# NVIDIA/nvalchemi-toolkit-ops

Measured on AMD Instinct MI355X. Metric: atom-steps/sec (nlist+D3+PME) on 100k-atom PBC box, higher is better.
Workload: dtype f64 (PME) + f32 (D3)

## Files before the change

include/nvalchemiops_hip.h:

```cpp
#ifndef NVALCHEMIOPS_HIP_H
#define NVALCHEMIOPS_HIP_H

#include <stddef.h>
#include <stdint.h>

#ifdef __cplusplus
extern "C" {
#endif

#define MI_OK 0
#define MI_EINVAL (-1)
#define MI_EHIP (-2)
#define MI_EWORKSPACE (-3)
#define MI_ECOMM (-4)

#define MI_F32 0
#define MI_F64 1

int mi_version(void);
const char* mi_last_error(void);
int mi_timing_enable(int on);
int mi_timing_select(const char* name );
int mi_timing_report(char* buf , int cap);
int mi_timing_report_stats(char* buf , int cap);
int mi_calibrate_copy(const void* src, void* dst, size_t bytes, void* stream);
int mi_calibrate_fill(void* dst, size_t bytes, float value, void* stream);
int mi_calibrate_read(const void* src, size_t bytes, float* sink , void* stream);

#define MI_NL_MODE_MATRIX 0
#define MI_NL_MODE_COUNT 1
#define MI_NL_MODE_CSR 2

#define MI_NL_HALF_FILL 1
#define MI_NL_NAIVE_EXPR 2
#define MI_NL_REUSE_GRID 4
#define MI_NL_NO_SHIFTS 8
#define MI_NL_NO_PAD 16

size_t mi_nl_workspace_bytes(int n_atoms, int n_systems, int dtype);

int mi_nl_neighbors(const void* positions,
                    int n_atoms,
                    const void* cell,
                    const uint8_t* pbc,
                    const int32_t* batch_idx,
                    int n_systems, double cutoff, int dtype, int mode, int flags,
                    int32_t* neighbor_matrix,
                    int32_t* neighbor_matrix_shifts,
                    int32_t* num_neighbors,
                    int max_neighbors, int fill_value,
                    const int32_t* neighbor_ptr,
                    int32_t* list_ij,
                    int32_t* list_shifts,
                    long long n_pairs,
                    const void* bin_origin,
                    void* workspace, size_t workspace_bytes, void* stream);

size_t mi_nl_packed_bytes(int n_atoms, int max_neighbors);
int mi_nl_neighbors_packed(const void* positions, int n_atoms, const void* cell, const uint8_t* pbc, const int32_t* batch_idx, int n_systems,
                           double cutoff, int dtype, int flags, int32_t* neighbor_matrix, int32_t* neighbor_matrix_shifts,
                           int32_t* num_neighbors, int max_neighbors, int fill_value, const void* bin_origin, void* workspace,
                           size_t workspace_bytes, void* packed_out, size_t packed_bytes, void* stream);

typedef struct mi_nl_cn_request {
  const int32_t* numbers;
  const float* covalent_radii;
  int nz;
  float k1;
} mi_nl_cn_request;
size_t mi_nl_cn_bytes(int n_atoms);
int mi_nl_neighbors_packed_cn(const void* positions, int n_atoms, const void* cell, const uint8_t* pbc, const int32_t* batch_idx, int n_systems,
                              double cutoff, int dtype, int flags, int32_t* neighbor_matrix, int32_t* neighbor_matrix_shifts,
                              int32_t* num_neighbors, int max_neighbors, int fill_value, const void* bin_origin, void* workspace,
                              size_t workspace_bytes, void* packed_out, size_t packed_bytes, const mi_nl_cn_request* request ,
                              void* cn_out, size_t cn_bytes, void* stream);

int mi_nl_neighbors_dual(const void* positions, int n_atoms, const void* cell, const uint8_t* pbc, const int32_t* batch_idx, int n_systems,
                         double cutoff_short, double cutoff_long, int dtype, int flags,
                         int32_t* neighbor_matrix_short, int32_t* neighbor_matrix_shifts_short, int32_t* num_neighbors_short,
                         int max_neighbors_short,
                         int32_t* neighbor_matrix_long, int32_t* neighbor_matrix_shifts_long, int32_t* num_neighbors_long,
                         int max_neighbors_long, int fill_value, const void* bin_origin, void* workspace, size_t workspace_bytes,
                         void* stream);

int mi_nl_matrix_to_coo(const int32_t* neighbor_matrix, const int32_t* neighbor_matrix_shifts,
                        const int32_t* neighbor_ptr, int n_atoms, int max_neighbors, int fill_value,
                        int32_t* list_ij, int32_t* list_shifts, long long n_pairs, void* stream);

int mi_nl_build_cell_cache(const void* positions, int n_atoms, const void* cell, const uint8_t* pbc,
                           const int32_t* batch_idx, int n_systems, double cutoff, int dtype,
                           int max_total_cells, int32_t* cells_per_dimension, int32_t* atom_periodic_shifts,
                           int32_t* atom_to_cell_mapping, int32_t* atoms_per_cell_count,
                           int32_t* cell_atom_start_indices, int32_t* cell_atom_list, void* workspace,
                           size_t workspace_bytes, void* stream);

int mi_nl_estimate_sizes(const void* cell, const uint8_t* pbc, int n_systems, double cutoff, int max_nbins,
                         int dtype, int32_t* number_of_cells ,
                         int32_t* neighbor_search_radius , void* stream);

int mi_nl_bounding_cells(const void* positions, const int32_t* batch_idx, int n_atoms, int n_systems, int dtype, void* cell_out,
                         void* origin_out, void* scratch, void* stream);

int mi_nl_cells_changed(const void* positions, const void* cell , const int32_t* atom_to_cell_mapping,
                        const int32_t* cells_per_dimension , const uint8_t* pbc , int n_atoms, int dtype,
                        uint8_t* flag, void* stream);
int mi_nl_moved_beyond_skin(const void* reference_positions, const void* current_positions, double threshold, int n_atoms, int dtype,
                            uint8_t* flag, void* stream);

typedef struct {
  const float* rcov;
  const float* r4r2;
  const float* c6ab;
  const float* cn_ref;
  int nz;
  float a1, a2, s6, s8, k1, k3, s5_on, s5_off;
} mi_d3_params;

size_t mi_d3_workspace_bytes(int n_atoms, int n_systems, int nz);
size_t mi_d3_workspace_bytes_packed(int n_atoms, int n_systems, int nz, int max_neighbors);
size_t mi_d3_workspace_bytes_entries(int n_atoms, int n_systems, int nz, long long n_entries);

int mi_d3(const void* positions, const int32_t* numbers, int n_atoms, int dtype,
          const int32_t* idx_j,
          const int32_t* unit_shifts,
          const int32_t* neighbor_ptr,
          int max_neighbors,
          long long n_list_entries,
          int fill_value,
          const void* cell,
          const int32_t* batch_idx,
          int n_systems, const mi_d3_params* params , int compute_virial,
          float* energy , float* forces , float* coord_num ,
          float* virial , void* workspace, size_t workspace_bytes, void* stream);

int mi_d3_packed(const void* positions, const int32_t* numbers, int n_atoms, int dtype, const int32_t* neighbor_matrix,
                 const int32_t* neighbor_matrix_shifts, int max_neighbors, int fill_value, const void* cell, const int32_t* batch_idx,
                 int n_systems, const mi_d3_params* params, int compute_virial, float* energy, float* forces, float* coord_num, float* virial,
                 void* workspace, size_t workspace_bytes, const void* packed_list, size_t packed_bytes ,
                 void* stream);

int mi_d3_packed_cn(const void* positions, const int32_t* numbers, int n_atoms, int dtype, const int32_t* neighbor_matrix,
                    const int32_t* neighbor_matrix_shifts, int max_neighbors, int fill_value, const void* cell, const int32_t* batch_idx,
                    int n_systems, const mi_d3_params* params, int compute_virial, float* energy, float* forces, float* coord_num, float* virial,
                    void* workspace, size_t workspace_bytes, const void* packed_list, size_t packed_bytes, const void* cn_block, size_t cn_bytes,
                    int verify_stride, int verify_phase, void* stream);

typedef struct {
  float rs6, rs8, alpha, beta;
  const float* r0ab;
} mi_d3_zero_params;

int mi_d3_zero(const void* positions, const int32_t* numbers, int n_atoms, int dtype, const int32_t* idx_j, const int32_t* unit_shifts,
               const int32_t* neighbor_ptr, int max_neighbors, long long n_list_entries, int fill_value, const void* cell,
               const int32_t* batch_idx, int n_systems, const mi_d3_params* params , const mi_d3_zero_params* zero ,
               int compute_virial, float* energy, float* forces, float* coord_num, float* virial, void* workspace, size_t workspace_bytes,
               void* stream);

int mi_d3_zero_packed_cn(const void* positions, const int32_t* numbers, int n_atoms, int dtype, const int32_t* neighbor_matrix,
                         const int32_t* neighbor_matrix_shifts, int max_neighbors, int fill_value, const void* cell, const int32_t* batch_idx,
                         int n_systems, const mi_d3_params* params, const mi_d3_zero_params* zero, int compute_virial, float* energy,
                         float* forces, float* coord_num, float* virial, void* workspace, size_t workspace_bytes, const void* packed_list,
                         size_t packed_bytes, const void* cn_block, size_t cn_bytes, int verify_stride, int verify_phase, void* stream);

size_t mi_d3_atm_workspace_bytes(int n_atoms, int n_systems, int nz);
size_t mi_d3_atm_visits_offset(int n_atoms, int n_systems, int nz);
int mi_d3_atm_tile(void);
int mi_d3_atm(const void* positions, const int32_t* numbers, int n_atoms, int dtype,
              const int32_t* idx_j, const int32_t* unit_shifts, const int32_t* neighbor_ptr ,
              int max_neighbors, int fill_value, const void* cell, const int32_t* batch_idx, int n_systems,
              const mi_d3_params* params , float s9, float alpha, float three_body_cutoff, int compute_virial,
              float* energy , float* forces , float* virial ,
              void* workspace, size_t workspace_bytes, void* stream);

int mi_d3_zero_atm(const void* positions, const int32_t* numbers, int n_atoms, int dtype,
                   const int32_t* idx_j, const int32_t* unit_shifts, const int32_t* neighbor_ptr ,
                   int max_neighbors, int fill_value, const void* cell, const int32_t* batch_idx, int n_systems,
                   const mi_d3_params* params , float s9, float alpha, float three_body_cutoff, float rs9,
                   const float* r0ab , int compute_virial, float* energy, float* forces, float* virial,
                   void* workspace, size_t workspace_bytes, void* stream);

typedef struct {
  const float* rcov;
  const float* en;
  const float* r4r2;
  const float* zeff;
  const float* gam;
  const int32_t* n_ref;
  const int32_t* ngw;
  const float* cn_ref;
  const float* q_ref;
  const float* c6_ref;
  int nz;
  float a1, a2, s6, s8, k_cn, k4, k5, k6, wf, ga, gc;
  float cn_cutoff;
} mi_d4_params;
size_t mi_d4_workspace_bytes(int n_atoms, int n_systems, int nz);
int mi_d4_species_slots(void);
int mi_d4_fold_blocks(void);
int mi_d4(const void* positions, const int32_t* numbers, int n_atoms, int dtype, const int32_t* idx_j, const int32_t* unit_shifts,
          const int32_t* neighbor_ptr , int max_neighbors, long long n_list_entries, int fill_value,
          const void* cell, const int32_t* batch_idx, int n_systems, const mi_d4_params* params ,
          const float* charges , int compute_virial, float* energy , float* forces ,
          float* coord_num , float* charge_grad , float* virial ,
          void* workspace, size_t workspace_bytes, void* stream);

size_t mi_d4_atm_workspace_bytes(int n_atoms, int n_systems, int nz);
size_t mi_d4_atm_visits_offset(int n_atoms, int n_systems, int nz);
int mi_d4_atm_tile(void);
int mi_d4_atm(const void* positions, const int32_t* numbers, int n_atoms, int dtype, const int32_t* idx_j, const int32_t* unit_shifts,
              const int32_t* neighbor_ptr , int max_neighbors, int fill_value, const void* cell,
              const int32_t* batch_idx, int n_systems, const mi_d4_params* params , float s9, float alpha,
              float three_body_cutoff, int compute_virial, float* energy , float* forces ,
              float* virial , void* workspace, size_t workspace_bytes, void* stream);

#define MI_EW_FORCES 1
#define MI_EW_CHARGE_GRAD 2
size_t mi_ewald_symmetry_scratch_bytes(void);
size_t mi_ewald_real_scratch_bytes(int n_atoms, int dtype);
int mi_ewald_real(const void* positions, const void* charges, const void* cell, const void* alpha ,
                  const int32_t* batch_idx, int n_atoms, int dtype, const int32_t* idx_j,
                  const int32_t* unit_shifts, const int32_t* neighbor_ptr, int max_neighbors, int mask_value,
                  int flags, double* energies , void* forces ,
                  double* charge_grads , void* scratch , size_t scratch_bytes, void* stream);
int mi_ewald_real_listed(const void* positions, const void* charges, const void* cell, const void* alpha, const int32_t* batch_idx, int n_atoms,
                         int dtype, const int32_t* idx_j, const int32_t* unit_shifts, const int32_t* neighbor_ptr, int max_neighbors,
                         int mask_value, int flags, double* energies, void* forces, double* charge_grads, void* scratch, size_t scratch_bytes,
                         const int32_t* search_num_neighbors, int verify_stride, int verify_phase, void* stream);
int mi_ewald_real_virial(const void* positions, const void* charges, const void* cell, const void* alpha, const int32_t* batch_idx, int n_atoms,
                         int n_systems, int dtype, const int32_t* idx_j, const int32_t* unit_shifts, const int32_t* neighbor_ptr, int max_neighbors,
                         int mask_value, int flags, double* energies, void* forces, double* charge_grads, void* scratch, size_t scratch_bytes,
                         const int32_t* search_num_neighbors, int verify_stride, int verify_phase, double* row_virial, double* virial_partial,
                         void* stream);
int mi_ewald_virial_blocks(void);

#define MI_GC_FORCES 1
#define MI_GC_CHARGE_GRAD 2
#define MI_GC_SIGMA_GRAD 4
#define MI_GC_VIRIAL 8
#define MI_GC_CELL_GRAD 16
size_t mi_gaussian_charges_scratch_bytes(int n_atoms, int dtype);
int mi_gaussian_charges_blocks(void);
int mi_gaussian_charges_row_words(void);
int mi_gaussian_charges_system_sums(const void* charges, const void* sigma, const double* weights, const int32_t* batch_idx, int n_atoms,
                                    int n_systems, int dtype, double* partial, void* stream);
int mi_gaussian_charges(const void* positions, const void* charges, const void* sigma, const void* cell ,
                        const int32_t* batch_idx, const double* weights, int n_atoms, int n_systems, int dtype, const int32_t* idx_j,
                        const int32_t* unit_shifts, const int32_t* neighbor_ptr, int max_neighbors, int mask_value, int flags, double* energies,
                        void* forces, double* charge_grads, double* sigma_grads, double* system_partial, void* scratch, size_t scratch_bytes,
                        void* stream);

#define MI_DP_FORCES 1
#define MI_DP_CHARGE_GRAD 2
#define MI_DP_DIPOLE_GRAD 4
#define MI_DP_VIRIAL 8
size_t mi_ewald_dipole_real_scratch_bytes(int n_atoms, int dtype);
int mi_ewald_dipole_blocks(void);
int mi_ewald_dipole_real(const void* positions, const void* charges, const void* dipoles, const void* cell ,
                         const void* alpha , const int32_t* batch_idx, const double* weights, int n_atoms, int n_systems, int dtype,
                         const int32_t* idx_j, const int32_t* unit_shifts, const int32_t* neighbor_ptr, int max_neighbors, int mask_value, int flags,
                         double* energies, void* forces, double* charge_grads, double* dipole_grads, double* virial_partial, void* scratch,
                         size_t scratch_bytes, void* stream);
int mi_ewald_dipole_structure_factors(const void* positions, const void* charges, const void* dipoles, const double* weights, const void* k_vectors,
                                      const int32_t* system_ptr, int n_atoms, int n_systems, int n_k, int dtype, double* table, void* stream);
int mi_ewald_dipole_recip_gather(const void* positions, const void* charges, const void* dipoles, const void* k_vectors, const void* cell,
                                 const void* alpha, const int32_t* batch_idx, const double* table, const double* table_g, const double* weights,
                                 int n_atoms, int n_systems, int n_k, int dtype, double* energies, void* forces, double* charge_grads,
                                 double* dipole_grads, void* stream);
int mi_ewald_dipole_recip_virial(const double* table, const void* k_vectors, const void* cell, const void* alpha, int n_systems, int n_k, int dtype,
                                 double* virial, void* stream);

#define MI_QD_FORCES 1
#define MI_QD_CHARGE_GRAD 2
#define MI_QD_DIPOLE_GRAD 4
#define MI_QD_VIRIAL 8
#define MI_QD_QUADRUPOLE_GRAD 16
size_t mi_ewald_quadrupole_real_scratch_bytes(int n_atoms, int dtype);
int mi_ewald_quadrupole_blocks(void);
int mi_ewald_quadrupole_real(const void* positions, const void* charges, const void* dipoles, const void* quadrupoles,
                             const void* cell , const void* alpha , const int32_t* batch_idx,
                             const double* weights, int n_atoms, int n_systems, int dtype, const int32_t* idx_j, const int32_t* unit_shifts,
                             const int32_t* neighbor_ptr, int max_neighbors, int mask_value, int flags, double* energies, void* forces,
                             double* charge_grads, double* dipole_grads, double* quadrupole_grads, double* virial_partial, void* scratch,
                             size_t scratch_bytes, void* stream);
int mi_ewald_quadrupole_structure_factors(const void* positions, const void* charges, const void* dipoles, const void* quadrupoles,
                                          const double* weights, const void* k_vectors, const int32_t* system_ptr, int n_atoms, int n_systems,
                                          int n_k, int dtype, double* table, double* table_v, void* stream);
int mi_ewald_quadrupole_recip_gather(const void* positions, const void* charges, const void* dipoles, const void* quadrupoles,
                                     const void* k_vectors, const void* cell, const void* alpha, const int32_t* batch_idx, const double* table,
                                     const double* table_g, const double* weights, int n_atoms, int n_systems, int n_k, int dtype,
                                     double* energies, void* forces, double* charge_grads, double* dipole_grads, double* quadrupole_grads,
                                     void* stream);
int mi_ewald_quadrupole_recip_virial(const double* table, const double* table_v, const void* k_vectors, const void* cell, const void* alpha,
                                     int n_systems, int n_k, int dtype, double* virial, void* stream);

#define MI_DP_POLAR_GRAD 16
size_t mi_thole_dipole_scratch_bytes(int n_atoms, int dtype);
int mi_thole_dipole_blocks(void);
int mi_thole_dipole(const void* positions, const void* charges, const void* dipoles, const void* cell ,
                    const void* polarizability , double thole_a, const int32_t* batch_idx, const double* weights, int n_atoms,
                    int n_systems, int dtype, const int32_t* idx_j, const int32_t* unit_shifts, const int32_t* neighbor_ptr, int max_neighbors,
                    int mask_value, int flags, double* energies, void* forces, double* charge_grads, double* dipole_grads,
                    double* polarizability_grads, double* virial_partial, void* scratch, size_t scratch_bytes, void* stream);

size_t mi_coulomb_dipole_scratch_bytes(int n_atoms, int dtype);
int mi_coulomb_dipole_blocks(void);
int mi_coulomb_dipole(const void* positions, const void* charges, const void* dipoles, const void* cell ,
                      const int32_t* batch_idx, const double* weights, int n_atoms, int n_systems, int dtype, const int32_t* idx_j,
                      const int32_t* unit_shifts, const int32_t* neighbor_ptr, int max_neighbors, int mask_value, int flags, double* energies,
                      void* forces, double* charge_grads, double* dipole_grads, double* virial_partial, void* scratch, size_t scratch_bytes,
                      void* stream);
size_t mi_coulomb_quadrupole_scratch_bytes(int n_atoms, int dtype);
int mi_coulomb_quadrupole_blocks(void);
int mi_coulomb_quadrupole(const void* positions, const void* charges, const void* dipoles, const void* quadrupoles,
                          const void* cell , const int32_t* batch_idx, const double* weights, int n_atoms,
                          int n_systems, int dtype, const int32_t* idx_j, const int32_t* unit_shifts, const int32_t* neighbor_ptr,
                          int max_neighbors, int mask_value, int flags, double* energies, void* forces, double* charge_grads,
                          double* dipole_grads, double* quadrupole_grads, double* virial_partial, void* scratch, size_t scratch_bytes,
                          void* stream);

int mi_qeq_blocks(void);
int mi_qeq_state_words(void);
int mi_qeq_pair_coefficients(const void* positions, const void* sigma, const double* hardness, const void* cell ,
                             const void* alpha , const int32_t* batch_idx, int n_atoms, int n_systems, int dtype,
                             const int32_t* idx_j, const int32_t* unit_shifts, const int32_t* neighbor_ptr, int max_neighbors, int mask_value,
                             double* coefficients, int32_t* neighbors, double* diagonal, void* stream);
int mi_qeq_apply(const double* coefficients, const int32_t* neighbors, const double* diagonal, const double* x, const double* y_in,
                 const int32_t* batch_idx, int n_atoms, int n_systems, const int32_t* neighbor_ptr, int max_neighbors, double* y, double* partial,
                 void* stream);
int mi_qeq_cg_update(const double* y, const double* partial_y, const double* counts, const int32_t* batch_idx, int n_atoms, int n_systems, int mode,
                     double* q, double* r, const double* p, const double* state_in, double* state_out, double* partial_rr, void* stream);
int mi_qeq_cg_direction(const double* partial_rr, const int32_t* batch_idx, int n_atoms, int n_systems, int mode, double tolerance, const double* r,
                        double* p, const double* state_in, double* state_out, void* stream);

int mi_induced_blocks(void);
int mi_induced_state_words(void);
int mi_induced_tensor_words(void);
int mi_induced_unroll_depth(void);
int mi_induced_pair_tensors(const void* positions, const void* polarizability, const void* cell , const void* alpha ,
                            const int32_t* batch_idx, int n_atoms, int n_systems, int dtype, const int32_t* idx_j, const int32_t* unit_shifts,
                            const int32_t* neighbor_ptr, int max_neighbors, int mask_value, long long n_slots, double* tensors, int32_t* neighbors,
                            double* diagonal, double* preconditioner, void* stream);
int mi_thole_induced_pair_tensors(const void* positions, const void* polarizability, const void* cell ,
                                  const void* alpha , const int32_t* batch_idx, int n_atoms, int n_systems, int dtype,
                                  const int32_t* idx_j, const int32_t* unit_shifts, const int32_t* neighbor_ptr, int max_neighbors, int mask_value,
                                  long long n_slots, double* tensors, int32_t* neighbors, double* diagonal, double* preconditioner,
                                  double thole_a, void* stream);
int mi_cluster_induced_pair_tensors(const void* positions, const void* polarizability, int n_atoms, int dtype, const int32_t* idx_j,
                                    const int32_t* neighbor_ptr, int max_neighbors, int mask_value, long long n_slots, double* tensors,
                                    int32_t* neighbors, double* diagonal, double* preconditioner, double thole_a, void* stream);
int mi_induced_apply(const double* tensors, const int32_t* neighbors, const double* diagonal, const double* x, const double* y_in,
                     const int32_t* batch_idx, int n_atoms, int n_systems, const int32_t* neighbor_ptr, int max_neighbors, long long n_slots,
                     double* y, double* partial, void* stream);
int mi_induced_dot(const double* x, const double* y, const int32_t* batch_idx, int n_atoms, int n_systems, double* partial, void* stream);
int mi_induced_cg_update(const double* y, const double* partial_y, const double* preconditioner, const int32_t* batch_idx, int n_atoms,
                         int n_systems, int mode, double* x, double* r, const double* p, const double* state_in,
                         double* state_out, double* partial_rr, void* stream);
int mi_induced_cg_direction(const double* partial_rr, const double* preconditioner, const int32_t* batch_idx, int n_atoms, int n_systems,
                            int mode, double tolerance, const double* r, double* p, const double* state_in, double* state_out,
                            void* stream);

int mi_ewald_recip_virial(const double* structure_factors, const void* k_vectors, const void* cell, const void* alpha, int n_systems, int n_k,
                          int dtype, double* partial, void* stream);
int mi_ewald_recip_virial_blocks(void);
int mi_ewald_structure_factors(const void* positions, const void* weights , const void* k_vectors, const void* cell,
                               const void* alpha, const int32_t* system_ptr, int n_atoms, int n_systems, int n_k,
                               int max_atoms_per_system, int dtype, double* structure_factors ,
                               double* total_charge , void* stream);
int mi_ewald_recip_gather(const void* positions, const void* charges, const void* k_vectors, const void* alpha, const int32_t* batch_idx,
                          const double* structure_factors, const double* total_charge, int n_atoms, int n_k, int dtype,
                          double* potential , double* kforce , double* energies ,
                          void* forces , double* charge_grads , void* stream);

int mi_ewald_recip_gather_kk(const void* positions, const void* k_vectors, const int32_t* batch_idx, const double* structure_factors,
                             const double* weights , int n_atoms, int n_k, int dtype, double* out , void* stream);

size_t mi_ewald_real_bwd_scratch_bytes(int n_systems);
int mi_ewald_real_bwd(const void* positions, const void* charges, const void* cell, const void* alpha, const int32_t* batch_idx,
                      int n_atoms, int n_systems, int dtype, const int32_t* idx_j, const int32_t* unit_shifts, const int32_t* neighbor_ptr,
                      int max_neighbors, int mask_value, const void* grad_energies ,
                      void* grad_positions , void* grad_charges ,
                      double* grad_cell, double* grad_alpha, void* symmetry_scratch ,
                      size_t scratch_bytes ,
                      void* stream);

int mi_ewald_real_forces_bwd(const void* positions, const void* charges, const void* cell, const void* alpha, const int32_t* batch_idx,
                             int n_atoms, int n_systems, int dtype, const int32_t* idx_j, const int32_t* unit_shifts,
                             const int32_t* neighbor_ptr, int max_neighbors, int mask_value, const void* grad_forces ,
                             const void* grad_charge_grads , double* grad_positions ,
                             double* grad_charges , double* grad_cell , double* grad_alpha ,
                             void* scratch , size_t scratch_bytes, void* stream);

int mi_coulomb(const double* positions, const double* charges, const double* cell , const int32_t* batch_idx,
               int n_atoms, const int32_t* idx_j, const int32_t* unit_shifts, const int32_t* neighbor_ptr, int max_neighbors,
               int fill_value, double cutoff, double alpha, double energy_prefactor, double* energies ,
               double* forces , void* stream);
int mi_coulomb_bwd(const double* positions, const double* charges, const double* cell, const int32_t* batch_idx, int n_atoms,
                   int n_systems, const int32_t* idx_j, const int32_t* unit_shifts, const int32_t* neighbor_ptr, int max_neighbors,
                   int fill_value, double cutoff, double alpha, double energy_prefactor, const double* grad_energies ,
                   double* grad_positions , double* grad_charges , double* grad_cell ,
                   void* stream);

int mi_coulomb_forces_bwd(const double* positions, const double* charges, const double* cell, const int32_t* batch_idx, int n_atoms,
                          int n_systems, const int32_t* idx_j, const int32_t* unit_shifts, const int32_t* neighbor_ptr, int max_neighbors,
                          int fill_value, double cutoff, double alpha, const double* grad_forces ,
                          double* grad_positions , double* grad_charges , double* grad_cell ,
                          void* stream);

#define MI_SPLINE_REFERENCE_ORDERS 0x100
int mi_cell_geometry(const void* cell, int n_systems, int dtype, void* cell_inv_t, void* reciprocal_cell, void* volume, void* stream);
int mi_pme_prepare(const void* cell, const void* charges, const int32_t* batch_idx, int n_atoms, int n_systems, int dtype,
                   void* cell_inv_t, void* reciprocal_cell, void* volume, void* total_charge , void* stream);
int mi_spline_spread_is_tiled(int n_systems, int nx, int ny, int nz, int order);
int mi_spline_spread_prefers_tiles(int n_atoms, int n_systems, int nx, int ny, int nz, int order);
int mi_spline_spread(const void* positions, const void* values, const int32_t* batch_idx,
                     const void* cell_inv_t , int n_atoms, int n_systems, int nx, int ny,
                     int nz, int order, int batched, int dtype, void* mesh ,
                     void* workspace , size_t workspace_bytes, void* stream);
size_t mi_spline_spread_workspace_bytes(int n_atoms, int n_systems, int nx, int ny, int nz);
size_t mi_spline_spread_workspace_bytes_for(int n_atoms, int n_systems, int nx, int ny, int nz, int order, int dtype);
long long mi_spline_spread_order_offset(int n_atoms, int n_systems, int nx, int ny, int nz, int order);
int mi_spline_gather(const void* positions, const void* mesh, const int32_t* batch_idx, const void* cell_inv_t,
                     int n_atoms, int n_systems, int nx, int ny, int nz, int order, int dtype,
                     void* out , void* stream);
int mi_spline_gather_vec3(const void* positions, const void* charges, const void* mesh_vec3 ,
                          const int32_t* batch_idx, const void* cell_inv_t, int n_atoms, int n_systems, int nx,
                          int ny, int nz, int order, int dtype, void* out , void* stream);

int mi_spline_gather_grad(const void* positions, const void* mesh, const int32_t* batch_idx, const void* cell_inv_t, int n_atoms,
                          int n_systems, int nx, int ny, int nz, int order, int dtype, void* out , void* stream);

int mi_spline_gather_hess_dot(const void* positions, const void* mesh, const int32_t* batch_idx, const void* cell_inv_t,
                              const void* vec , int n_atoms, int n_systems, int nx, int ny, int nz, int order, int dtype,
                              void* out , void* stream);
int mi_spline_spread_grad(const void* positions, const void* vec , const int32_t* batch_idx, const void* cell_inv_t,
                          int n_atoms, int n_systems, int nx, int ny, int nz, int order, int dtype, void* mesh ,
                          void* stream);

size_t mi_spline_spread_channels_workspace_bytes_for(int n_atoms, int n_systems, int nx, int ny, int nz, int order, int n_channels, int dtype);
int mi_spline_spread_channels(const void* positions, const void* values , const int32_t* batch_idx, const void* cell_inv_t,
                              int n_atoms, int n_systems, int n_channels, int nx, int ny, int nz, int order, int batched, int dtype,
                              void* mesh , void* workspace, size_t workspace_bytes, void* stream);
int mi_spline_gather_channels(const void* positions, const void* mesh , const int32_t* batch_idx,
                              const void* cell_inv_t, int n_atoms, int n_systems, int n_channels, int nx, int ny, int nz, int order, int dtype,
                              void* out , void* stream);
int mi_spline_gather_channels_frac_grad(const void* positions, const void* mesh , const void* coef ,
                                        const int32_t* batch_idx, const void* cell_inv_t, int n_atoms, int n_systems, int n_channels, int nx,
                                        int ny, int nz, int order, int dtype, void* out , void* stream);

int mi_sph_harm(const double* positions , int n, int l_max, double* out, void* stream);
int mi_sph_harm_grad(const double* positions , int n, int l_max, double* out, void* stream);
int mi_gto_density(const double* positions , int n, double sigma, int l_max, double* out, void* stream);
int mi_gto_fourier(const double* k_vectors , int n, double sigma, int l_max, double* out_real, double* out_imag, void* stream);

int mi_fft_plan_create(int nx, int ny, int nz, int batch, int dtype, int inverse, void** plan_out);
size_t mi_fft_plan_work_bytes(const void* plan);
int mi_fft_plan_exec(void* plan, void* in, void* out, void* stream);
int mi_fft_plan_destroy(void* plan);

int mi_fft_library_versions(int* compiled, int* loaded);

#define MI_DFT_MAX_N 1024
int mi_dft3d(void* in, void* out, int nx, int ny, int nz, int batch, int dtype, int inverse, void* stream);

int mi_pme_green_sf(const void* k_squared , const void* alpha , const void* volume ,
                    int n_systems, int nx, int ny, int nz, int sf_exponent, int dtype, void* green ,
                    void* sf_sq , void* stream);
int mi_pme_convolve(const void* spec , const void* recip_cell ,
                    const void* alpha , const void* volume , int n_systems, int nx, int ny, int nz,
                    int sf_exponent, int with_field, int dtype,
                    const void* k_vectors , const void* k_squared ,
                    int k_batched , void* out , void* stream);
int mi_pme_solve_supported(int n_systems, int nx, int ny, int nz, int dtype);
int mi_pme_solve_preferred(int n_systems, int nx, int ny, int nz, int dtype);
size_t mi_pme_solve_scratch_bytes(int n_systems, int nx, int ny, int nz, int n_channels , int dtype);
int mi_pme_solve(const void* mesh, const void* recip_cell , const void* alpha ,
                 const void* volume , int n_systems, int nx, int ny, int nz, int order ,
                 int with_field, int dtype, void* scratch, size_t scratch_bytes, void* real_out, void* stream);
int mi_pme_solve_keep(const void* mesh, const void* recip_cell, const void* alpha, const void* volume, int n_systems, int nx, int ny, int nz,
                      int order, int with_field, int dtype, void* scratch, size_t scratch_bytes, void* real_out, void* spectrum_out,
                      void* stream);
int mi_fft_lds_supported(int batch, int nx, int ny, int nz, int dtype);
size_t mi_fft_lds_scratch_bytes(int batch, int nx, int ny, int nz, int dtype);
int mi_fft_lds(const void* in, void* out, int batch, int nx, int ny, int nz, int dtype, int inverse, void* scratch, size_t scratch_bytes,
               const void* tables , void* stream);
size_t mi_fft_lds_tables_bytes(int nx, int ny, int nz, int dtype);
int mi_fft_lds_tables(int nx, int ny, int nz, int dtype, void* tables, void* stream);
int mi_pme_solve_tabled(const void* mesh, const void* recip_cell, const void* alpha, const void* volume, int n_systems, int nx, int ny, int nz,
                        int order, int with_field, int dtype, void* scratch, size_t scratch_bytes, void* real_out, void* spectrum_out,
                        const void* tables, void* stream);
int mi_pme_convolve_bwd(const void* spec, const void* weight_spec, int n_channels, const void* recip_cell, const void* alpha, const void* volume,
                        int n_systems, int nx, int ny, int nz, int order, int dtype, void* conv_out, double* partial, void* stream);
int mi_pme_convolve_bwd_blocks(void);
int mi_pme_virial(const void* spec, const void* recip_cell, const void* alpha, const void* volume, int n_systems, int nx, int ny, int nz, int order,
                  int dtype, const void* k_vectors, const void* k_squared, int k_batched, const void* total_charge, double* partial, void* stream);
int mi_pme_virial_blocks(void);

int mi_pme_dipole_spread(const void* positions, const void* charges, const void* dipoles, const double* weights, const int32_t* batch_idx,
                         const void* cell_inv_t, int n_atoms, int n_systems, int nx, int ny, int nz, int order, int dtype, void* meshes, void* stream);
int mi_pme_dipole_gather(const void* positions, const void* charges, const void* dipoles, const double* weights, const int32_t* batch_idx,
                         const void* cell_inv_t, const void* mesh_a, const void* mesh_b, const void* alpha , int n_atoms, int n_systems,
                         int nx, int ny, int nz, int order, int dtype, int accumulate, double* energies, void* forces, double* charge_grads,
                         double* dipole_grads, void* stream);
int mi_pme_dipole_virial(const void* spec_q, const void* spec_mu, const void* recip_cell, const void* alpha, const void* volume, int n_systems, int nx,
                         int ny, int nz, int order, int dtype, double* partial, void* stream);
int mi_pme_dipole_virial_blocks(void);

int mi_pme_quadrupole_spread(const void* positions, const void* charges, const void* dipoles, const void* quadrupoles, const double* weights,
                             const int32_t* batch_idx, const void* cell_inv_t, int n_atoms, int n_systems, int nx, int ny, int nz, int order, int dtype,
                             void* meshes, void* stream);
int mi_pme_quadrupole_gather(const void* positions, const void* charges, const void* dipoles, const void* quadrupoles, const double* weights,
                             const int32_t* batch_idx, const void* cell_inv_t, const void* mesh_a, const void* mesh_b, const void* alpha ,
                             int n_atoms, int n_systems, int nx, int ny, int nz, int order, int dtype, int accumulate, double* energies, void* forces,
                             double* charge_grads, double* dipole_grads, double* quadrupole_grads, void* stream);
int mi_pme_quadrupole_virial(const void* spec_l, const void* spec_t, const void* recip_cell, const void* alpha, const void* volume, int n_systems,
                             int nx, int ny, int nz, int order, int dtype, double* partial, void* stream);
int mi_pme_quadrupole_virial_blocks(void);

int mi_pme_gather_finish(const void* positions, const void* charges, const int32_t* batch_idx, const void* cell_inv_t,
                         const void* meshes , const void* alpha, const void* volume,
                         const void* total_charge , int n_atoms, int n_systems, int nx, int ny, int nz,
                         int order, int with_field, int dtype, void* energies ,
                         void* forces , void* charge_grads ,
                         const double* add_energies, const void* add_forces, const double* add_charge_grads,
                         const void* spread_workspace ,
                         void* stream);
int mi_pme_corrections(const void* raw, const void* charges, const int32_t* batch_idx, const void* volume,
                       const void* alpha, const void* total_charge, int n_atoms, int dtype, void* energies,
                       void* charge_grads , void* stream);
int mi_segment_sum(const void* values, const int32_t* batch_idx, int n_atoms, int dtype, void* out , void* stream);

int mi_frame_rotate(const void* positions, const void* local_dipoles, const void* local_quadrupoles, const int32_t* frame_atoms,
                    const int32_t* frame_kinds, const void* cell, const int32_t* batch_idx, int n_atoms, int n_systems, int dtype, void* dipoles,
                    void* quadrupoles, void* stream);
int mi_frame_adjoint(const void* positions, const void* local_dipoles, const void* local_quadrupoles, const int32_t* frame_atoms,
                     const int32_t* frame_kinds, const void* cell, const int32_t* batch_idx, const void* dipole_grads,
                     const void* quadrupole_grads, int n_atoms, int n_systems, int dtype, double* records, double* local_dipole_grads,
                     double* local_quadrupole_grads, double* virial_rows, void* stream);
int mi_frame_gather(const double* records, const int32_t* inverse_ptr, const int32_t* inverse_slots, long long n_entries,
                    const double* virial_rows, const int32_t* batch_idx, int n_atoms, int n_systems, int dtype, double sign, void* out,
                    double* virial_partial, void* stream);
int mi_frame_blocks(void);
int mi_frame_block_threads(void);

#define MI_COMM_ID_BYTES 128
int mi_comm_library_version(int* version );
int mi_comm_unique_id(void* id_out , size_t bytes);
int mi_comm_init(const void* id , size_t bytes, int n_ranks, int rank, void** comm_out);
int mi_comm_size(const void* comm, int* n_ranks , int* rank );
int mi_comm_allgather_f32(void* comm, const float* send, float* recv , size_t count_per_rank, void* stream);
int mi_comm_allgather_f64(void* comm, const double* send, double* recv, size_t count_per_rank, void* stream);
int mi_comm_destroy(void* comm);

#ifdef __cplusplus
}
#endif
#endif
```

nvalchemi-toolkit-ops_amd/csrc/nlist.hip:

```cpp
#include <stdlib.h>

#include "binsort.h"
#include "common.h"

namespace {

#define NL_PRUNE_R 8
#ifndef NL_TILE
#define NL_TILE 1024
#endif
#ifndef NL_TILE_F64
#define NL_TILE_F64 768
#endif
#ifndef NL_TILED_WAVES
#define NL_TILED_WAVES 0
#endif
#ifndef NL_CCHUNK
#define NL_CCHUNK 64
#endif
#define NL_MAXROWS 96
#define NL_MIXED 0x7fffffff
#define NL_TILED_GRID 1536
static int nl_tiled_grid() {
  static const int g = [] { const char* e = getenv("NVALCHEMIOPS_NL_TILED_GRID"); const int v = e ? atoi(e) : 0; return v > 0 ? v : NL_TILED_GRID; }();
  return g;
}
template <class T> struct NlSys {
  T cell[9];
  T inv[9];
  T origin[3];
  int cpd[3];
  int R[3];
  int pbc[3];
  int nrange[3];
  int cell_off;
  int ncells;
  int tiled;
  int prune;
  signed char dxlim[NL_PRUNE_R + 1][NL_PRUNE_R + 1];
};
struct NlGlobal {
  int total_cells; int any_wrap; int use_tiled; int pad1;
  int work[4];
  int done[4];
};

struct NlLayout {
  size_t sys, glob, natoms, keys_in, keys_out, vals_in, vals_out, wrap, swrap, spos, srk, cell_start, bins, total;
  long long cell_cap;
};

inline long long nl_cell_cap(int N, int B) { return 4ll * N + 8ll * B; }

inline int nl_key_bits(long long cap) {
  int bits = 1;
  while ((1ll << bits) <= cap && bits < 31) ++bits;
  return bits;
}

NlLayout nl_layout(int N, int B, int dtype) {
  NlLayout L;
  size_t o = 0;
  const size_t sysz = dtype == MI_F32 ? sizeof(NlSys<float>) : sizeof(NlSys<double>);
  const size_t esz = dtype == MI_F32 ? 4 : 8;
  L.cell_cap = nl_cell_cap(N, B);
  auto take = [&](size_t bytes) { size_t at = o; o += mi_align(bytes); return at; };
  L.sys = take(sysz * (size_t)B);
  L.glob = take(sizeof(NlGlobal));
  L.natoms = take(sizeof(int) * (size_t)B);
  L.keys_in = take(sizeof(int) * (size_t)N);
  L.keys_out = take(sizeof(int) * (size_t)N);
  L.vals_in = take(sizeof(int) * (size_t)N);
  L.vals_out = take(sizeof(int) * (size_t)N);
  L.wrap = take(8 * (size_t)N);
  L.swrap = take(8 * (size_t)N);
  L.spos = take(4 * esz * (size_t)N);
  L.srk = take(sizeof(float) * (size_t)N);
  L.cell_start = take(sizeof(int) * (size_t)(L.cell_cap + 2));
  L.bins = take(sizeof(int) * bs_scratch_ints(L.cell_cap + 2));
  L.total = o;
  return L;
}

__device__ __forceinline__ float4 pack4(float x, float y, float z, int idx) { return make_float4(x, y, z, __int_as_float(idx)); }
__device__ __forceinline__ double4 pack4(double x, double y, double z, int idx) { return make_double4(x, y, z, (double)idx); }
__device__ __forceinline__ int idx_of(const float4& v) { return __float_as_int(v.w); }
__device__ __forceinline__ int idx_of(const double4& v) { return (int)v.w; }

__global__ void nl_count_atoms_kernel(const int* __restrict__ batch_idx, int N, int* __restrict__ natoms) {
  const int i = blockIdx.x * blockDim.x + threadIdx.x;
  const bool in = i < N;
  const int s = in ? batch_idx[i] : -1;
  const int s0 = __shfl(s, 0, MI_WAVE);
  const unsigned long long same = __ballot(in && s == s0);
  if ((threadIdx.x & (MI_WAVE - 1)) == 0 && s0 >= 0) atomicAdd(&natoms[s0], __popcll(same));
  if (in && s != s0) atomicAdd(&natoms[s], 1);
}

template <class T>
__device__ void nl_describe_system(const T* __restrict__ cell, const uint8_t* __restrict__ pbc, const int* __restrict__ natoms, int N, T cutoff,
                                   const T* __restrict__ origin, int s, NlSys<T>& S) {
  for (int k = 0; k < 9; ++k) S.cell[k] = cell[9 * (size_t)s + k];
  for (int k = 0; k < 3; ++k) S.origin[k] = origin ? origin[3 * (size_t)s + k] : T(0);
  inverse3(S.cell, S.inv);
  const T* a = S.cell;
  double det = (double)a[0] * ((double)a[4] * a[8] - (double)a[5] * a[7]) - (double)a[1] * ((double)a[3] * a[8] - (double)a[5] * a[6]) +
               (double)a[2] * ((double)a[3] * a[7] - (double)a[4] * a[6]);
  double vol = fabs(det);
  int ns = natoms ? natoms[s] : N;
  double rc = (double)cutoff;
  double apc = vol > 0 ? (double)ns / vol * rc * rc * rc : 0.0;
#ifndef NL_K2_APC
#define NL_K2_APC 64.0
#endif
  int k = apc < NL_K2_APC ? 1 : (apc < 512.0 ? 2 : 3);
  long long cap = 4ll * ns + 8;
  double face[3];
  for (int d = 0; d < 3; ++d) {
    T col[3] = {S.inv[d], S.inv[3 + d], S.inv[6 + d]};
    T ln = sqrt(col[0] * col[0] + col[1] * col[1] + col[2] * col[2]);
    face[d] = 1.0 / (double)ln;
    S.pbc[d] = pbc[3 * (size_t)s + d] ? 1 : 0;
    double want = face[d] * k / (rc * (1.0 + 2e-6));
    S.cpd[d] = want >= 1048576.0 ? 1048576 : (want >= 1.0 ? (int)want : 1);
    S.nrange[d] = S.pbc[d] ? (int)ceil(ln * cutoff) : 0;
  }
  long long tot = (long long)S.cpd[0] * S.cpd[1] * S.cpd[2];
  while (tot > cap) {
    for (int d = 0; d < 3; ++d) S.cpd[d] = S.cpd[d] / 2 > 1 ? S.cpd[d] / 2 : 1;
    tot = (long long)S.cpd[0] * S.cpd[1] * S.cpd[2];
  }
  for (int d = 0; d < 3; ++d) {
    if (S.cpd[d] == 1 && !S.pbc[d]) S.R[d] = 0;
    else S.R[d] = (int)ceil(rc * S.cpd[d] / face[d] * (1.0 + 1e-6));
  }
  S.ncells = (int)tot;
  S.cell_off = 0;
  S.tiled = ((k >= 2 || apc >= 32.0) && (2 * S.R[1] + 1) * (2 * S.R[2] + 1) <= NL_MAXROWS && (!S.pbc[0] || S.R[0] <= S.cpd[0])) ? 1 : 0;
  const bool ortho = a[1] == T(0) && a[2] == T(0) && a[3] == T(0) && a[5] == T(0) && a[6] == T(0) && a[7] == T(0);
  S.prune = (ortho && S.R[0] <= NL_PRUNE_R && S.R[1] <= NL_PRUNE_R && S.R[2] <= NL_PRUNE_R) ? 1 : 0;
}

template <class T>
__global__ __launch_bounds__(256) void nl_setup_kernel(const T* __restrict__ cell, const uint8_t* __restrict__ pbc, const int* __restrict__ natoms, int N,
                                int B, T cutoff, const T* __restrict__ origin, NlSys<T>* __restrict__ sys, NlGlobal* __restrict__ glob,
                                int table_blocks, int4* __restrict__ zero, long long zero_words, int* __restrict__ pk_flag,
                                int* __restrict__ cn_hdr, float cn_scale) {
  constexpr int NE = (NL_PRUNE_R + 1) * (NL_PRUNE_R + 1);
  if (pk_flag && blockIdx.x == 0 && threadIdx.x == 0) *pk_flag = 0;
  if (cn_hdr && blockIdx.x == 0) {
    if (threadIdx.x == 0) { cn_hdr[0] = 0; cn_hdr[1] = 0; cn_hdr[2] = __float_as_int((float)cutoff); cn_hdr[3] = __float_as_int(cn_scale); }
    if (threadIdx.x < MI_CN_SLOTS) reinterpret_cast<unsigned long long*>(cn_hdr)[MI_CN_SLOT_OFFSET_U64 + threadIdx.x] = 0ull;
  }
  if ((int)blockIdx.x > table_blocks) {
    const long long zb = (long long)blockIdx.x - table_blocks - 1, nzb = (long long)gridDim.x - table_blocks - 1;
    for (long long k = zb * blockDim.x + threadIdx.x; k < zero_words; k += nzb * blockDim.x) zero[k] = make_int4(0, 0, 0, 0);
    return;
  }
  if (blockIdx.x > 0) {
    const int t = ((int)blockIdx.x - 1) * blockDim.x + threadIdx.x;
    if (t >= B * NE) return;
    const int s = t / NE, az = (t - s * NE) / (NL_PRUNE_R + 1), ay = t - s * NE - az * (NL_PRUNE_R + 1);
    NlSys<T> S;
    nl_describe_system<T>(cell, pbc, natoms, N, cutoff, origin, s, S);
    if (!S.prune) return;
    const double rc = (double)cutoff;
    double w[3];
    for (int d = 0; d < 3; ++d) {
      const double ln = fabs((double)S.inv[4 * d]);
      w[d] = (S.pbc[d] && ln > 0.0) ? (1.0 / ln) / S.cpd[d] : 0.0;
    }
    const double gz = (az > 1 ? az - 1 : 0) * w[2], gy = (ay > 1 ? ay - 1 : 0) * w[1];
    const double rem = rc * rc - gz * gz - gy * gy;
    int lim;
    if (rem < -1e-6 * rc * rc) lim = -1;
    else if (w[0] > 0.0) { lim = (int)(sqrt(rem > 0.0 ? rem : 0.0) / w[0] * (1.0 + 1e-6)) + 1; if (lim > S.R[0]) lim = S.R[0]; }
    else lim = S.R[0];
    sys[s].dxlim[az][ay] = (signed char)lim;
    return;
  }
  for (int s = threadIdx.x; s < B; s += blockDim.x) {
    NlSys<T> S;
    nl_describe_system<T>(cell, pbc, natoms, N, cutoff, origin, s, S);
    NlSys<T>* dst = sys + s;
    for (int k = 0; k < 9; ++k) { dst->cell[k] = S.cell[k]; dst->inv[k] = S.inv[k]; }
    for (int k = 0; k < 3; ++k) { dst->origin[k] = S.origin[k]; dst->cpd[k] = S.cpd[k]; dst->R[k] = S.R[k]; dst->pbc[k] = S.pbc[k]; dst->nrange[k] = S.nrange[k]; }
    dst->cell_off = 0; dst->ncells = S.ncells; dst->tiled = S.tiled; dst->prune = S.prune;
  }
  __syncthreads();
  __shared__ int wave_tot[4];
  __shared__ int carry_sh, tiled_sh;
  if (threadIdx.x == 0) { carry_sh = 0; tiled_sh = 1; }
  __syncthreads();
  const int lane = threadIdx.x & (MI_WAVE - 1), wave = threadIdx.x / MI_WAVE;
  for (int s0 = 0; s0 < B; s0 += blockDim.x) {
    const int s = s0 + threadIdx.x;
    const int x = s < B ? sys[s].ncells : 0;
    if (s < B && !sys[s].tiled) tiled_sh = 0;
    int inc = x;
#pragma unroll
    for (int o = 1; o < MI_WAVE; o <<= 1) { const int up = __shfl_up(inc, o, MI_WAVE); if (lane >= o) inc += up; }
    if (lane == MI_WAVE - 1) wave_tot[wave] = inc;
    __syncthreads();
    int woff = carry_sh;
    for (int w = 0; w < 4; ++w) woff += (w < wave) ? wave_tot[w] : 0;
    if (s < B) sys[s].cell_off = woff + inc - x;
    __syncthreads();
    if (threadIdx.x == blockDim.x - 1) carry_sh = woff + inc;
    __syncthreads();
  }
  if (threadIdx.x == 0) {
    glob->total_cells = carry_sh;
    glob->any_wrap = 0;
    glob->use_tiled = tiled_sh;
    for (int k = 0; k < 4; ++k) { glob->work[k] = 0; glob->done[k] = 0; }
  }
}

template <class T>
__global__ void nl_assign_kernel(const T* __restrict__ pos, const int* __restrict__ batch_idx, int N, const NlSys<T>* __restrict__ sys,
                                 int* __restrict__ keys, int* __restrict__ count, short4* __restrict__ wrap, NlGlobal* __restrict__ glob) {
  int i = blockIdx.x * blockDim.x + threadIdx.x;
  const bool in = i < N;
  int key = 0;
  if (in) {
    const int s = batch_idx ? batch_idx[i] : 0;
    const NlSys<T>& S = sys[s];
    T p[3] = {pos[3 * (size_t)i] - S.origin[0], pos[3 * (size_t)i + 1] - S.origin[1], pos[3 * (size_t)i + 2] - S.origin[2]}, frac[3];
    rowvec_mat3(p, S.inv, frac);
    int c[3], w[3];
#pragma unroll
    for (int d = 0; d < 3; ++d) {
      int v = (int)floor(frac[d] * (T)S.cpd[d]);
      if (S.pbc[d]) floor_divmod(v, S.cpd[d], w[d], c[d]);
      else { w[d] = 0; c[d] = v < 0 ? 0 : (v >= S.cpd[d] ? S.cpd[d] - 1 : v); }
    }
    key = S.cell_off + c[0] + S.cpd[0] * (c[1] + S.cpd[1] * c[2]);
    keys[i] = key;
    wrap[i] = make_short4((short)w[0], (short)w[1], (short)w[2], 0);
    if (w[0] | w[1] | w[2]) glob->any_wrap = 1;
  }
  bs_wave_add<false>(count, key, in);
}

struct NlCnBuild { const int* numbers; const float* rcov; int nz; float K; float* srk; unsigned long long* slots; const void* cell; int n_cell; const int* batch_idx; };
template <class T>
__global__ void nl_rank_gather_kernel(const T* __restrict__ pos, const int* __restrict__ ids, const int* __restrict__ keys,
                                      const int* __restrict__ cell_start, const short4* __restrict__ wrap, int N,
                                      typename Vec4<T>::type* __restrict__ spos, short4* __restrict__ swrap, int* __restrict__ keys_sorted,
                                      NlCnBuild C) {
  int p = blockIdx.x * blockDim.x + threadIdx.x;
  unsigned long long h = 0;
  if (p < N) {
    const int i = ids[p];
    const int key = keys[i];
    const int b = cell_start[key], e = cell_start[key + 1];
    int rank = 0;
    for (int q = b; q < e; ++q) rank += ids[q] < i ? 1 : 0;
    const int dst = b + rank;
    const T x = pos[3 * (size_t)i], y = pos[3 * (size_t)i + 1], z = pos[3 * (size_t)i + 2];
    spos[dst] = pack4(x, y, z, i);
    swrap[dst] = wrap[i];
    keys_sorted[dst] = key;
    if (C.srk) {
      const float rk = mi_cn_rk(C.numbers[i], C.nz, C.rcov, C.K);
      C.srk[dst] = rk;
      h = mi_cn_atom_hash<T>(i, C.batch_idx ? C.batch_idx[i] : 0, x, y, z, rk);
    }
  }
  if (C.srk) {
    if (p < C.n_cell) h += mi_cn_cell_hash<T>(p, reinterpret_cast<const T*>(C.cell)[p]);
    if (p == 0) h += mi_cn_scale_hash(C.K);
    mi_cn_slot_add(C.slots, p / MI_WAVE, h);
  }
}

struct NlInt3 { int a, b, c; };

template <bool NT = true>
__device__ __forceinline__ void wave_fill(int* __restrict__ dst, long long begin, long long end, int value, int lane) {
  long long n = end - begin;
  if (n <= 0) return;
  int* p = dst + begin;
  int head = (int)(((16 - ((uintptr_t)p & 15)) & 15) >> 2);
  if (head > n) head = (int)n;
  if (lane < head) p[lane] = value;
  long long body = (n - head) >> 2;
  int4* p4 = reinterpret_cast<int4*>(p + head);
  typedef int nl_i4 __attribute__((ext_vector_type(4)));
  const nl_i4 w4 = {value, value, value, value};
  for (long long t = lane; t < body; t += MI_WAVE) {
    if constexpr (NT) __builtin_nontemporal_store(w4, reinterpret_cast<nl_i4*>(p4 + t));
    else *reinterpret_cast<nl_i4*>(p4 + t) = w4;
  }
  long long done = head + (body << 2);
  if (done + lane < n) p[done + lane] = value;
}

__device__ __noinline__ void nl_prefix_runs(int* run_pre, int n, int lane) {
  int carry = 0;
  if (lane == 0) run_pre[0] = 0;
  for (int r0 = 0; r0 < n; r0 += MI_WAVE) {
    const int r = r0 + lane;
    int inc = r < n ? run_pre[r + 1] : 0;
#pragma unroll
    for (int o = 1; o < MI_WAVE; o <<= 1) { const int up = __shfl_up(inc, o, MI_WAVE); if (lane >= o) inc += up; }
    if (r < n) run_pre[r + 1] = carry + inc;
    carry += __shfl(inc, MI_WAVE - 1, MI_WAVE);
  }
}

__device__ __forceinline__ long long nl_uniform64(long long v) {
  const unsigned lo = __builtin_amdgcn_readfirstlane((unsigned)v), hi = __builtin_amdgcn_readfirstlane((unsigned)((unsigned long long)v >> 32));
  return (long long)(((unsigned long long)hi << 32) | lo);
}

__device__ __forceinline__ float nl_uni(float x) { return __int_as_float(__builtin_amdgcn_readfirstlane(__float_as_int(x))); }
__device__ __forceinline__ double nl_uni(double x) { return __longlong_as_double(nl_uniform64(__double_as_longlong(x))); }

template <class T> struct NlSecond { T rc2; int* nm; int* nsh; int* num; int M; };
struct NlPacked { unsigned* words; int* flag; };
struct NlCn { const float* rk; float* cn; int* flag; float K; };
__device__ __forceinline__ float nl_cn_term(float d2, float rki, float rkj, float K) {
  const float rinv = __builtin_amdgcn_rsqf(d2);
  const float t = fmaf(-(rki + rkj), rinv, K);
  return __builtin_amdgcn_rcpf(1.0f + __builtin_amdgcn_exp2f(t));
}
#define NL_PK_PAD 0xffffffffu
#ifndef NL_PREZERO_SHIFTS
#define NL_PREZERO_SHIFTS 1
#endif
#ifndef NL_PREZERO_NT
#define NL_PREZERO_NT 1
#endif
#define NL_PK_ZERO_SHIFT 0x54000000u
__device__ __forceinline__ unsigned nl_pk_code(int Sx, int Sy, int Sz, bool& bad) {
  const unsigned cx = (unsigned)(Sx + 1), cy = (unsigned)(Sy + 1), cz = (unsigned)(Sz + 1);
  bad = (cx > 2u) | (cy > 2u) | (cz > 2u);
  return ((cx & 3u) << 26) | ((cy & 3u) << 28) | (cz << 30);
}

template <class T>
__device__ __forceinline__ bool nl_pair_hit(T pix, T piy, T piz, int i, T cjx, T cjy, T cjz, int j, int Sx, int Sy, int Sz, const T* cart,
                                            T rc2, bool naive, bool half, int nr0, int nr1, int nr2, T* d2_out = nullptr) {
  T dr0, dr1, dr2;
  bool ok = true;
  if (!naive) {
    dr0 = (cjx - pix) + cart[0];
    dr1 = (cjy - piy) + cart[1];
    dr2 = (cjz - piz) + cart[2];
  } else {
    const bool upper = Sx > 0 || (Sx == 0 && Sy > 0) || (Sx == 0 && Sy == 0 && Sz >= 0);
    if (upper) { dr0 = (cart[0] + cjx) - pix; dr1 = (cart[1] + cjy) - piy; dr2 = (cart[2] + cjz) - piz; }
    else { dr0 = ((-cart[0]) + pix) - cjx; dr1 = ((-cart[1]) + piy) - cjy; dr2 = ((-cart[2]) + piz) - cjz; }
    ok = (Sx <= nr0 && -Sx <= nr0) && (Sy <= nr1 && -Sy <= nr1) && (Sz <= nr2 && -Sz <= nr2);
  }
  const T d2 = dr0 * dr0 + dr1 * dr1 + dr2 * dr2;
  if (d2_out) *d2_out = d2;
  const bool zeroS = (Sx | Sy | Sz) == 0;
  bool hit = ok && (d2 < rc2) && !(j == i && zeroS);
  if (half && hit) {
    const bool pos_shift = Sx > 0 || (Sx == 0 && Sy > 0) || (Sx == 0 && Sy == 0 && Sz > 0);
    hit = pos_shift || (zeroS && j > i);
  }
  return hit;
}

template <class T, int MODE, bool FAST, bool DUAL = false, bool CNF = false>
#if NL_TILED_WAVES > 0
__global__ __launch_bounds__(256) __attribute__((amdgpu_waves_per_eu(NL_TILED_WAVES, NL_TILED_WAVES))) void nl_query_tiled_kernel(
#else
__global__ __launch_bounds__(256) __attribute__((amdgpu_waves_per_eu((CNF && sizeof(T) == 4) ? 5 : 1, (CNF && sizeof(T) == 4) ? 5 : 8))) void nl_query_tiled_kernel(
#endif
    const typename Vec4<T>::type* __restrict__ spos, const short4* __restrict__ swrap, const int* __restrict__ cell_start,
    const NlSys<T>* __restrict__ sys, const NlGlobal* __restrict__ glob, int B, T rc2, int flags, int* __restrict__ nm,
    int* __restrict__ nsh, int* __restrict__ num, int M, int fill_value, const int* __restrict__ ptr, int* __restrict__ list_ij,
    int* __restrict__ list_sh, long long P, NlSecond<T> D, NlPacked K, NlCn CN = NlCn{nullptr, nullptr, nullptr, 0.0f}) {
  static_assert(!DUAL || (MODE == MI_NL_MODE_MATRIX && !FAST), "the dual-cutoff sweep is instantiated for the general matrix kernel only");
  static_assert(!CNF || (MODE == MI_NL_MODE_MATRIX && FAST && !DUAL), "coordination numbers ride with the plain full-list matrix search");
  constexpr int TILE = sizeof(T) == 8 ? NL_TILE_F64 : NL_TILE;
  if (!glob->use_tiled) return;
  if (!DUAL && FAST != ((flags & (MI_NL_HALF_FILL | MI_NL_NAIVE_EXPR)) == 0)) return;
  __shared__ float trk[CNF ? TILE : 1], cen_rk[CNF ? NL_CCHUNK : 1];
  __shared__ double ccn[CNF ? NL_CCHUNK : 1];
  __shared__ int ccnt2[DUAL ? NL_CCHUNK : 1];
  __shared__ T tx[TILE], ty[TILE], tz[TILE];
  __shared__ int tj[TILE];
  __shared__ short tsx[CNF ? 1 : TILE], tsy[CNF ? 1 : TILE], tsz[CNF ? 1 : TILE];
  __shared__ int tsp[CNF ? TILE : 1];
  __shared__ int run_beg[3 * NL_MAXROWS], run_pre[3 * NL_MAXROWS + 1], run_cs[3 * NL_MAXROWS];
  __shared__ int ccnt[NL_CCHUNK];
  __shared__ T cen_x[NL_CCHUNK], cen_y[NL_CCHUNK], cen_z[NL_CCHUNK];
  __shared__ int cen_i[NL_CCHUNK];
  __shared__ short4 cen_w[NL_CCHUNK];
  __shared__ int grp_run[TILE / MI_WAVE];
  __shared__ int grp_shift[TILE / MI_WAVE];
  __shared__ int u_store[CNF ? 1 : 9 * NL_MAXROWS];
  static_assert(sizeof(T) * TILE >= sizeof(int) * 9 * NL_MAXROWS, "the run table must fit the x array of a tile");
  int* const u_beg = CNF ? reinterpret_cast<int*>(tx) : u_store;
  int* const u_len = u_beg + 3 * NL_MAXROWS;
  int* const u_cs = u_beg + 6 * NL_MAXROWS;
  const int tid = threadIdx.x, lane = tid & (MI_WAVE - 1), wave = tid / MI_WAVE;
  const int total_cells = glob->total_cells;
  const bool anyw = glob->any_wrap != 0;
  const bool half = (flags & MI_NL_HALF_FILL) != 0, naive = (flags & MI_NL_NAIVE_EXPR) != 0;
  const unsigned long long lt = (1ull << lane) - 1ull;
  __shared__ int next_cell;
  NlGlobal* gw = const_cast<NlGlobal*>(glob);
  for (;;) {
    __syncthreads();
    if (tid == 0) next_cell = atomicAdd(&gw->work[MODE], 1);
    __syncthreads();
    const int c = next_cell;
    if (c >= total_cells) break;
    const int c_beg = cell_start[c], n_c = cell_start[c + 1] - c_beg;
    if (n_c == 0) continue;
    int s = 0;
    {
      int lo = 0, hi = B - 1;
      while (lo < hi) { const int mid = (lo + hi + 1) >> 1; if (sys[mid].cell_off <= c) lo = mid; else hi = mid - 1; }
      s = lo;
    }
    const NlSys<T>* S = sys + s;
    const int nx = S->cpd[0], ny = S->cpd[1], nz = S->cpd[2];
    const int Rx = S->R[0], Ry = S->R[1], Rz = S->R[2];
    const bool pbx = S->pbc[0] != 0, pby = S->pbc[1] != 0, pbz = S->pbc[2] != 0;
    const int coff = S->cell_off;
    const int nr0 = S->nrange[0], nr1 = S->nrange[1], nr2 = S->nrange[2];
    T cm[9];
#pragma unroll
    for (int k = 0; k < 9; ++k) cm[k] = S->cell[k];
    const int local = c - coff;
    const int cx = local % nx, cyz = local / nx, cy = cyz % ny, cz = cyz / ny;
    const int nyr = 2 * Ry + 1, nrows = (2 * Rz + 1) * nyr;
    __syncthreads();
    if (tid < nrows) {
      const int dzr = tid / nyr, dz = dzr - Rz, dy = tid - dzr * nyr - Ry;
      const int tzc = cz + dz, tyc = cy + dy;
      bool ok = (pbz || (tzc >= 0 && tzc < nz)) && (pby || (tyc >= 0 && tyc < ny));
      int csz = 0, wz = tzc, csy = 0, wy = tyc;
      if (ok) {
        while (wz < 0) { wz += nz; --csz; }
        while (wz >= nz) { wz -= nz; ++csz; }
        while (wy < 0) { wy += ny; --csy; }
        while (wy >= ny) { wy -= ny; ++csy; }
      }
      int dxm = Rx;
      if (S->prune) { dxm = S->dxlim[dz < 0 ? -dz : dz][dy < 0 ? -dy : dy]; ok = ok && dxm >= 0; }
      int xlo = cx - dxm, xhi = cx + dxm;
      if (!pbx) { xlo = xlo < 0 ? 0 : xlo; xhi = xhi > nx - 1 ? nx - 1 : xhi; }
      const int rowbase = coff + nx * (wy + ny * wz);
      for (int g = 0; g < 3; ++g) {
        const int img0 = (g - 1) * nx;
        const int xa = (xlo > img0 ? xlo : img0), xb = (xhi < img0 + nx - 1 ? xhi : img0 + nx - 1);
        int b = 0, len = 0;
        if (ok && xa <= xb && (pbx || g == 1)) { b = cell_start[rowbase + xa - img0]; len = cell_start[rowbase + xb - img0 + 1] - b; }
        u_beg[3 * tid + g] = b;
        u_len[3 * tid + g] = len;
        u_cs[3 * tid + g] = ((g - 1) & 0x3ff) | ((csy & 0x3ff) << 10) | ((csz & 0x3ff) << 20);
      }
    }
    __syncthreads();
    for (int r = tid; r < 3 * nrows; r += 256) {
      const int key = u_cs[r];
      int rank = 0;
      for (int q = 0; q < 3 * nrows; ++q) {
        const int kq = u_cs[q];
        rank += ((unsigned)kq < (unsigned)key) || (kq == key && q < r);
      }
      run_beg[rank] = u_beg[r];
      run_pre[rank + 1] = u_len[r];
      run_cs[rank] = key;
    }
    __syncthreads();
    if (wave == 0) nl_prefix_runs(run_pre, 3 * nrows, lane);
    __syncthreads();
    const int nruns = 3 * nrows, total = run_pre[nruns];
    for (int cbase = 0; cbase < n_c; cbase += NL_CCHUNK) {
      const int cend = (cbase + NL_CCHUNK < n_c) ? cbase + NL_CCHUNK : n_c;
      if (tid < NL_CCHUNK) {
        ccnt[tid] = 0;
        if (DUAL) ccnt2[tid] = 0;
        if (cbase + tid < cend) {
          const auto cr = spos[c_beg + cbase + tid];
          cen_x[tid] = cr.x; cen_y[tid] = cr.y; cen_z[tid] = cr.z;
          cen_i[tid] = idx_of(cr);
          cen_w[tid] = anyw ? swrap[c_beg + cbase + tid] : make_short4(0, 0, 0, 0);
          if (CNF) { cen_rk[tid] = CN.rk[c_beg + cbase + tid]; ccn[tid] = 0.0; }
        }
      }
      for (int tile0 = 0; tile0 < total; tile0 += TILE) {
        const int tile_n = (total - tile0 < TILE) ? total - tile0 : TILE;
        __syncthreads();
        if (tid < TILE / MI_WAVE && tile0 + tid * MI_WAVE < total) {
          const int v = tile0 + tid * MI_WAVE;
          int lo = 0, hi = nruns - 1;
          while (lo < hi) { const int mid = (lo + hi + 1) >> 1; if (run_pre[mid] <= v) lo = mid; else hi = mid - 1; }
          grp_run[tid] = lo;
        }
        __syncthreads();
        for (int t = tid; t < tile_n; t += 256) {
          const int v = tile0 + t;
          int lo = grp_run[t / MI_WAVE];
          while (lo + 1 < nruns && run_pre[lo + 1] <= v) ++lo;
          const int q = run_beg[lo] + (v - run_pre[lo]);
          const auto rec = spos[q];
          tx[t] = rec.x; ty[t] = rec.y; tz[t] = rec.z;
          tj[t] = idx_of(rec);
          if (CNF) trk[t] = CN.rk[q];
          const int cs = run_cs[lo];
          int sx = (cs << 22) >> 22, sy = (cs << 12) >> 22, sz = (cs << 2) >> 22;
          if (anyw) {
            const short4 wj = swrap[q];
            if (pbx) sx -= wj.x;
            if (pby) sy -= wj.y;
            if (pbz) sz -= wj.z;
          }
          if (CNF) tsp[t] = (sx & 0x3ff) | ((sy & 0x3ff) << 10) | ((sz & 0x3ff) << 20);
          else { tsx[t] = (short)sx; tsy[t] = (short)sy; tsz[t] = (short)sz; }
          const int cs0 = __builtin_amdgcn_readfirstlane(cs);
          const bool same = __all(cs == cs0) && !anyw;
          if (lane == 0) grp_shift[t / MI_WAVE] = same ? cs0 : NL_MIXED;
        }
        __syncthreads();
        constexpr int NC = 2;
        for (int ci0 = cbase + wave; ci0 < cend; ci0 += 4 * NC) {
          T ccx[NC], ccy[NC], ccz[NC];
          int ii[NC], cap_row[NC], cnt[NC], cnt2[NC];
          float rki[NC], cnp[NC];
          long long out_base[NC];
          short4 wi[NC];
          const int nc = (cend - ci0 + 3) / 4 < NC ? (cend - ci0 + 3) / 4 : NC;
#pragma unroll
          for (int u = 0; u < NC; ++u) {
            const bool live = u < nc;
            const int ci = live ? ci0 + 4 * u : ci0;
            ccx[u] = live ? cen_x[ci - cbase] : (T)NAN; ccy[u] = cen_y[ci - cbase]; ccz[u] = cen_z[ci - cbase];
            if (CNF) { ccx[u] = nl_uni(ccx[u]); ccy[u] = nl_uni(ccy[u]); ccz[u] = nl_uni(ccz[u]); }
            ii[u] = __builtin_amdgcn_readfirstlane(cen_i[ci - cbase]);
            wi[u] = cen_w[ci - cbase];
            if (MODE == MI_NL_MODE_CSR) { out_base[u] = ptr[ii[u]]; cap_row[u] = ptr[ii[u] + 1] - ptr[ii[u]]; }
            else { out_base[u] = (long long)ii[u] * M; cap_row[u] = M; }
            cnt[u] = ccnt[ci - cbase];
            cnt2[u] = DUAL ? ccnt2[ci - cbase] : 0;
            if (CNF) { rki[u] = nl_uni(cen_rk[ci - cbase]); cnp[u] = 0.0f; }
          }
          const bool ortho = S->prune != 0;
          int* row_j[NC];
          NlInt3* row_s[NC];
          unsigned* row_p[NC];
#pragma unroll
          for (int u = 0; u < NC; ++u) {
            const long long ob = nl_uniform64(out_base[u]);
            row_p[u] = (MODE == MI_NL_MODE_MATRIX && !DUAL && K.words) ? K.words + ob : nullptr;
            if (MODE == MI_NL_MODE_MATRIX) { row_j[u] = nm + ob; row_s[u] = nsh ? reinterpret_cast<NlInt3*>(nsh) + ob : nullptr; }
            else if (MODE == MI_NL_MODE_CSR) { row_j[u] = list_ij + P + ob; row_s[u] = list_sh ? reinterpret_cast<NlInt3*>(list_sh) + ob : nullptr; }
            else { row_j[u] = nullptr; row_s[u] = nullptr; }
          }
          constexpr bool PREZERO = NL_PREZERO_SHIFTS && MODE == MI_NL_MODE_MATRIX && !DUAL;
          const bool prezero = PREZERO && nsh && !(flags & MI_NL_NO_PAD);
          if (PREZERO && prezero && tile0 == 0) {
#pragma unroll
            for (int u = 0; u < NC; ++u)
              if (u < nc) wave_fill<NL_PREZERO_NT != 0>(nsh, out_base[u] * 3, (out_base[u] + M) * 3, 0, lane);
            asm volatile("s_waitcnt vmcnt(0)" ::: "memory");
          }
          auto emit_m = [&](int u, unsigned long long mask, bool hit, int j, int Sx, int Sy, int Sz, unsigned code, bool zero_shift = false) {
            if (MODE == MI_NL_MODE_COUNT) { cnt[u] += __popcll(mask); return; }
            if (mask) {
              const unsigned slot = __builtin_amdgcn_mbcnt_hi((unsigned)(mask >> 32), __builtin_amdgcn_mbcnt_lo((unsigned)mask, (unsigned)cnt[u]));
              if (hit && slot < (unsigned)cap_row[u]) {
                *reinterpret_cast<int*>(reinterpret_cast<char*>(row_j[u]) + slot * 4u) = j;
                if (row_s[u] && !(PREZERO && prezero && zero_shift))
                  *reinterpret_cast<NlInt3*>(reinterpret_cast<char*>(row_s[u]) + __umul24(slot, 12u)) = NlInt3{Sx, Sy, Sz};
                if (MODE == MI_NL_MODE_MATRIX && !DUAL && row_p[u]) *reinterpret_cast<unsigned*>(reinterpret_cast<char*>(row_p[u]) + slot * 4u) = (unsigned)j | code;
              }
              cnt[u] += __popcll(mask);
            }
          };
          auto emit = [&](int u, bool hit, int j, int Sx, int Sy, int Sz, unsigned code) { emit_m(u, __builtin_amdgcn_ballot_w64(hit), hit, j, Sx, Sy, Sz, code); };
          struct Cand { int j, tt, zg; T x, y, z; };
          auto fetch = [&](int t0) {
            Cand c;
            const int t = t0 + lane;
            const bool in = t < tile_n;
            c.tt = in ? t : 0;
            c.j = tj[c.tt];
            c.x = in ? tx[c.tt] : (T)NAN;
            c.y = ty[c.tt]; c.z = tz[c.tt];
            c.zg = grp_shift[(t0 < tile_n ? t0 : 0) / MI_WAVE];
            return c;
          };
          Cand nxt = fetch(0);
          for (int t0 = 0; t0 < tile_n; t0 += MI_WAVE) {
            const Cand cur = nxt;
            nxt = fetch(t0 + MI_WAVE);
            const int j = cur.j, tt = cur.tt;
            const float rkj = CNF ? trk[tt] : 0.0f;
            const T cjx = cur.x, cjy = cur.y, cjz = cur.z;
            const int gs = __builtin_amdgcn_readfirstlane(cur.zg);
            if (FAST && gs == 0) {
#pragma unroll
              for (int u = 0; u < NC; ++u) {
                const T dr0 = cjx - ccx[u], dr1 = cjy - ccy[u], dr2 = cjz - ccz[u];
                const T d2 = dr0 * dr0 + dr1 * dr1 + dr2 * dr2;
                const bool in = d2 < rc2, other = j != ii[u];
                if (CNF) cnp[u] += (in & other & ((float)d2 >= 1e-24f)) ? nl_cn_term((float)d2, rki[u], rkj, CN.K) : 0.0f;
                emit_m(u, __builtin_amdgcn_ballot_w64(in) & __builtin_amdgcn_ballot_w64(other), in & other, j, 0, 0, 0, NL_PK_ZERO_SHIFT, true);
              }
            } else if (FAST && gs != NL_MIXED) {
              const int Sx = (gs << 22) >> 22, Sy = (gs << 12) >> 22, Sz = (gs << 2) >> 22;
              T cart[3];
              if (ortho) { cart[0] = cm[0] * (T)Sx; cart[1] = cm[4] * (T)Sy; cart[2] = cm[8] * (T)Sz; }
              else { const T fs[3] = {(T)Sx, (T)Sy, (T)Sz}; rowvec_mat3(fs, cm, cart); }
              bool bad;
              const unsigned code = nl_pk_code(Sx, Sy, Sz, bad);
#pragma unroll
              for (int u = 0; u < NC; ++u) {
                const T dr0 = (cjx - ccx[u]) + cart[0], dr1 = (cjy - ccy[u]) + cart[1], dr2 = (cjz - ccz[u]) + cart[2];
                const T d2 = dr0 * dr0 + dr1 * dr1 + dr2 * dr2;
                const bool h = d2 < rc2;
                if (CNF) cnp[u] += (h & ((float)d2 >= 1e-24f)) ? nl_cn_term((float)d2, rki[u], rkj, CN.K) : 0.0f;
                if (MODE == MI_NL_MODE_MATRIX && bad && row_p[u] && h) *K.flag = 1;
                emit(u, h, j, Sx, Sy, Sz, code);
              }
            } else {
              int Sx0, Sy0, Sz0;
              if (CNF) { const int w = tsp[tt]; Sx0 = (w << 22) >> 22; Sy0 = (w << 12) >> 22; Sz0 = (w << 2) >> 22; }
              else { Sx0 = tsx[tt]; Sy0 = tsy[tt]; Sz0 = tsz[tt]; }
#pragma unroll
              for (int u = 0; u < NC; ++u) {
                int Sx = Sx0, Sy = Sy0, Sz = Sz0;
                if (anyw) { if (pbx) Sx += wi[u].x; if (pby) Sy += wi[u].y; if (pbz) Sz += wi[u].z; }
                T cart[3];
                if (ortho) { cart[0] = cm[0] * (T)Sx; cart[1] = cm[4] * (T)Sy; cart[2] = cm[8] * (T)Sz; }
                else { const T fs[3] = {(T)Sx, (T)Sy, (T)Sz}; rowvec_mat3(fs, cm, cart); }
                bool h;
                if (FAST) {
                  const T dr0 = (cjx - ccx[u]) + cart[0], dr1 = (cjy - ccy[u]) + cart[1], dr2 = (cjz - ccz[u]) + cart[2];
                  const T d2 = dr0 * dr0 + dr1 * dr1 + dr2 * dr2;
                  h = (d2 < rc2) & !((j == ii[u]) & ((Sx | Sy | Sz) == 0));
                  if (CNF) cnp[u] += (h & ((float)d2 >= 1e-24f)) ? nl_cn_term((float)d2, rki[u], rkj, CN.K) : 0.0f;
                } else {
                  T d2;
                  h = nl_pair_hit<T>(ccx[u], ccy[u], ccz[u], ii[u], cjx, cjy, cjz, j, Sx, Sy, Sz, cart, rc2, naive, half, nr0, nr1, nr2, &d2);
                  if (DUAL) {
                    const bool h2 = h && (d2 < D.rc2);
                    const unsigned long long m2 = __ballot(h2);
                    if (m2) {
                      const int slot = cnt2[u] + __popcll(m2 & lt);
                      if (h2 && slot < D.M) {
                        const long long o = (long long)ii[u] * D.M + slot;
                        D.nm[o] = j;
                        if (D.nsh) reinterpret_cast<NlInt3*>(D.nsh)[o] = NlInt3{Sx, Sy, Sz};
                      }
                      cnt2[u] += __popcll(m2);
                    }
                  }
                }
                bool bad;
                const unsigned code = nl_pk_code(Sx, Sy, Sz, bad);
                if (MODE == MI_NL_MODE_MATRIX && !DUAL && bad && row_p[u] && h) *K.flag = 1;
                emit(u, h, j, Sx, Sy, Sz, code);
              }
            }
          }
          if (CNF) {
#pragma unroll
            for (int u = 0; u < NC; ++u) {
              const double part = wave_sum((double)cnp[u]);
              if (lane == 0 && u < nc) ccn[ci0 + 4 * u - cbase] += part;
            }
          }
          if (lane == 0) {
#pragma unroll
            for (int u = 0; u < NC; ++u) if (u < nc) { ccnt[ci0 + 4 * u - cbase] = cnt[u]; if (DUAL) ccnt2[ci0 + 4 * u - cbase] = cnt2[u]; }
          }
        }
      }
      __syncthreads();
      for (int ci = cbase + wave; ci < cend; ci += 4) {
        const int i = __builtin_amdgcn_readfirstlane(cen_i[ci - cbase]);
        const int cnt = ccnt[ci - cbase];
        if (MODE != MI_NL_MODE_CSR) { if (lane == 0) num[i] = cnt; }
        if (CNF && lane == 0) {
          CN.cn[i] = (float)ccn[ci - cbase];
          if (cnt > M) *CN.flag = 1;
        }
        if (MODE == MI_NL_MODE_CSR) {
          const long long rb = ptr[i];
          const int room = ptr[i + 1] - ptr[i];
          wave_fill(list_ij, rb, rb + (cnt < room ? cnt : room), i, lane);
        }
        if (MODE == MI_NL_MODE_MATRIX && !(flags & MI_NL_NO_PAD)) {
          const long long out_base = (long long)i * M;
          const int used = cnt < M ? cnt : M;
          wave_fill(nm, out_base + used, out_base + M, fill_value, lane);
          if (nsh && !(NL_PREZERO_SHIFTS && !DUAL)) wave_fill(nsh, (out_base + used) * 3, (out_base + M) * 3, 0, lane);
          if (!DUAL && K.words) wave_fill(reinterpret_cast<int*>(K.words), out_base + used, out_base + M, (int)NL_PK_PAD, lane);
        }
        if (DUAL) {
          const int c2 = ccnt2[ci - cbase];
          if (lane == 0) D.num[i] = c2;
          if (!(flags & MI_NL_NO_PAD)) {
            const long long ob = (long long)i * D.M;
            const int used = c2 < D.M ? c2 : D.M;
            wave_fill(D.nm, ob + used, ob + D.M, fill_value, lane);
            if (D.nsh) wave_fill(D.nsh, (ob + used) * 3, (ob + D.M) * 3, 0, lane);
          }
        }
      }
      __syncthreads();
    }
  }
  if (tid == 0 && atomicAdd(&gw->done[MODE], 1) == (int)gridDim.x - 1) {
    gw->work[MODE] = 0;
    gw->done[MODE] = 0;
  }
}

template <class T, int MODE, bool DUAL = false, bool CNF = false>
__global__ __launch_bounds__(256) void nl_query_kernel(
    const typename Vec4<T>::type* __restrict__ spos, const short4* __restrict__ swrap, const int* __restrict__ keys_sorted,
    const int* __restrict__ cell_start, const int* __restrict__ batch_idx, const NlSys<T>* __restrict__ sys,
    const NlGlobal* __restrict__ glob, int N, T rc2, int flags, int* __restrict__ nm, int* __restrict__ nsh, int* __restrict__ num,
    int M, int fill_value, const int* __restrict__ ptr, int* __restrict__ list_ij, int* __restrict__ list_sh, long long P, NlSecond<T> D,
    NlPacked K, NlCn CN = NlCn{nullptr, nullptr, nullptr, 0.0f}) {
  static_assert(!DUAL || MODE == MI_NL_MODE_MATRIX, "the dual-cutoff sweep fills two padded matrices");
  static_assert(!CNF || (MODE == MI_NL_MODE_MATRIX && !DUAL), "coordination numbers ride with the plain matrix search");
  if (glob->use_tiled) return;
  const int lane = threadIdx.x & (MI_WAVE - 1);
  const int p = __builtin_amdgcn_readfirstlane(blockIdx.x * (blockDim.x / MI_WAVE) + (threadIdx.x / MI_WAVE));
  if (p >= N) return;
  const auto ci = spos[p];
  const int i = __builtin_amdgcn_readfirstlane(idx_of(ci));
  const T pix = ci.x, piy = ci.y, piz = ci.z;
  const int s = batch_idx ? __builtin_amdgcn_readfirstlane(batch_idx[i]) : 0;
  const NlSys<T>* S = sys + s;
  const int nx = S->cpd[0], ny = S->cpd[1], nz = S->cpd[2];
  const int Rx = S->R[0], Ry = S->R[1], Rz = S->R[2];
  const bool pbx = S->pbc[0] != 0, pby = S->pbc[1] != 0, pbz = S->pbc[2] != 0;
  const int coff = S->cell_off;
  T cm[9];
#pragma unroll
  for (int k = 0; k < 9; ++k) cm[k] = S->cell[k];
  const int local = __builtin_amdgcn_readfirstlane(keys_sorted[p]) - coff;
  const int cx = local % nx, cyz = local / nx, cy = cyz % ny, cz = cyz / ny;
  const bool anyw = glob->any_wrap != 0;
  short4 wi = make_short4(0, 0, 0, 0);
  if (anyw) wi = swrap[p];
  const bool half = (flags & MI_NL_HALF_FILL) != 0;
  const bool naive = (flags & MI_NL_NAIVE_EXPR) != 0;
  const int nr0 = S->nrange[0], nr1 = S->nrange[1], nr2 = S->nrange[2];
  const unsigned long long lt = (1ull << lane) - 1ull;
  long long out_base;
  int cap_row;
  if (MODE == MI_NL_MODE_CSR) { out_base = ptr[i]; cap_row = ptr[i + 1] - ptr[i]; }
  else { out_base = (long long)i * M; cap_row = M; }
  int cnt = 0, cnt2 = 0;
  const float rki = CNF ? __int_as_float(__builtin_amdgcn_readfirstlane(__float_as_int(CN.rk[p]))) : 0.0f;
  double cnacc = 0.0;

  const bool prune = S->prune != 0;

  auto scan_run = [&](int beg, int end, int sx, int csy, int csz) {
    T cart_u[3];
    {
      const T fsu[3] = {(T)sx, (T)csy, (T)csz};
      rowvec_mat3(fsu, cm, cart_u);
    }
    for (int q0 = beg; q0 < end; q0 += MI_WAVE) {
      const int q = q0 + lane;
      bool hit = false, hit2 = false;
      int j = 0, Sx = sx, Sy = csy, Sz = csz;
      if (q < end) {
        const auto cj = spos[q];
        j = idx_of(cj);
        if (anyw) {
          const short4 wj = swrap[q];
          if (pbx) Sx += (int)wi.x - (int)wj.x;
          if (pby) Sy += (int)wi.y - (int)wj.y;
          if (pbz) Sz += (int)wi.z - (int)wj.z;
        }
        T cart[3] = {cart_u[0], cart_u[1], cart_u[2]};
        if (anyw) {
          const T fs[3] = {(T)Sx, (T)Sy, (T)Sz};
          rowvec_mat3(fs, cm, cart);
        }
        T d2;
        hit = nl_pair_hit<T>(pix, piy, piz, i, cj.x, cj.y, cj.z, j, Sx, Sy, Sz, cart, rc2, naive, half, nr0, nr1, nr2, &d2);
        hit2 = DUAL && hit && (d2 < D.rc2);
        if (CNF) cnacc += (hit && (float)d2 >= 1e-24f) ? (double)nl_cn_term((float)d2, rki, CN.rk[q], CN.K) : 0.0;
      }
      if (DUAL) {
        const unsigned long long m2 = __ballot(hit2);
        if (m2) {
          const int slot = cnt2 + __popcll(m2 & lt);
          if (hit2 && slot < D.M) {
            const long long o = (long long)i * D.M + slot;
            D.nm[o] = j;
            if (D.nsh) reinterpret_cast<NlInt3*>(D.nsh)[o] = NlInt3{Sx, Sy, Sz};
          }
          cnt2 += __popcll(m2);
        }
      }
      const unsigned long long mask = __ballot(hit);
      if (mask) {
        const int slot = cnt + __popcll(mask & lt);
        if (MODE == MI_NL_MODE_MATRIX) {
          if (hit && slot < cap_row) {
            nm[out_base + slot] = j;
            if (nsh) reinterpret_cast<NlInt3*>(nsh)[out_base + slot] = NlInt3{Sx, Sy, Sz};
            if (K.words) {
              bool bad;
              const unsigned code = nl_pk_code(Sx, Sy, Sz, bad);
              if (bad) *K.flag = 1;
              K.words[out_base + slot] = (unsigned)j | code;
            }
          }
        } else if (MODE == MI_NL_MODE_CSR) {
          if (hit && slot < cap_row) {
            list_ij[P + out_base + slot] = j;
            if (list_sh) reinterpret_cast<NlInt3*>(list_sh)[out_base + slot] = NlInt3{Sx, Sy, Sz};
          }
        }
        cnt += __popcll(mask);
      }
    }
  };

  if (!pbx || Rx <= nx) {
    const int nyr = 2 * Ry + 1, nrows = (2 * Rz + 1) * nyr;
    for (int rbase = 0; rbase < nrows; rbase += MI_WAVE) {
      const int row = rbase + lane;
      int rb[3] = {0, 0, 0}, re[3] = {0, 0, 0}, cs = 0;
      if (row < nrows) {
        const int dzr = row / nyr, dz = dzr - Rz, dy = row - dzr * nyr - Ry;
        const int tz = cz + dz, ty = cy + dy;
        bool ok = (pbz || (tz >= 0 && tz < nz)) && (pby || (ty >= 0 && ty < ny));
        int csz = 0, wz = tz, csy = 0, wy = ty;
        if (ok) {
          while (wz < 0) { wz += nz; --csz; }
          while (wz >= nz) { wz -= nz; ++csz; }
          while (wy < 0) { wy += ny; --csy; }
          while (wy >= ny) { wy -= ny; ++csy; }
        }
        int dxm = Rx;
        if (prune) { dxm = S->dxlim[dz < 0 ? -dz : dz][dy < 0 ? -dy : dy]; ok = ok && dxm >= 0; }
        if (ok) {
          int xlo = cx - dxm, xhi = cx + dxm;
          if (!pbx) { xlo = xlo < 0 ? 0 : xlo; xhi = xhi > nx - 1 ? nx - 1 : xhi; }
          const int rowbase = coff + nx * (wy + ny * wz);
#pragma unroll
          for (int g = 0; g < 3; ++g) {
            const int img0 = (g - 1) * nx;
            const int xa = (xlo > img0 ? xlo : img0), xb = (xhi < img0 + nx - 1 ? xhi : img0 + nx - 1);
            if (xa <= xb && (pbx || g == 1)) { rb[g] = cell_start[rowbase + xa - img0]; re[g] = cell_start[rowbase + xb - img0 + 1]; }
          }
          cs = (csy & 0xffff) | (csz << 16);
        }
      }
      const int rmax = nrows - rbase < MI_WAVE ? nrows - rbase : MI_WAVE;
      for (int r = 0; r < rmax; ++r) {
        const int csr = __builtin_amdgcn_readlane(cs, r);
        const int csy = (int)(short)(csr & 0xffff), csz = csr >> 16;
#pragma unroll
        for (int g = 0; g < 3; ++g) {
          const int beg = __builtin_amdgcn_readlane(rb[g], r), end = __builtin_amdgcn_readlane(re[g], r);
          if (beg < end) scan_run(beg, end, g - 1, csy, csz);
        }
      }
    }
  } else {
    for (int dz = -Rz; dz <= Rz; ++dz) {
      const int tz = cz + dz;
      if (!pbz && (tz < 0 || tz >= nz)) continue;
      int csz = 0, wz = tz;
      while (wz < 0) { wz += nz; --csz; }
      while (wz >= nz) { wz -= nz; ++csz; }
      for (int dy = -Ry; dy <= Ry; ++dy) {
        const int ty = cy + dy;
        if (!pby && (ty < 0 || ty >= ny)) continue;
        int csy = 0, wy = ty;
        while (wy < 0) { wy += ny; --csy; }
        while (wy >= ny) { wy -= ny; ++csy; }
        int dxm = Rx;
        if (prune) {
          dxm = S->dxlim[dz < 0 ? -dz : dz][dy < 0 ? -dy : dy];
          if (dxm < 0) continue;
        }
        int xlo = cx - dxm, xhi = cx + dxm, sx_lo = 0, sx_hi = 0;
        for (int t = xlo; t < 0; t += nx) --sx_lo;
        for (int t = xhi; t >= nx; t -= nx) ++sx_hi;
        const int rowbase = coff + nx * (wy + ny * wz);
        for (int sx = sx_lo; sx <= sx_hi; ++sx) {
          const int img0 = sx * nx;
          const int xa = (xlo > img0 ? xlo : img0) - img0;
          const int xb = (xhi < img0 + nx - 1 ? xhi : img0 + nx - 1) - img0;
          scan_run(cell_start[rowbase + xa], cell_start[rowbase + xb + 1], sx, csy, csz);
        }
      }
    }
  }
  if (MODE != MI_NL_MODE_CSR) {
    if (lane == 0) num[i] = cnt;
  } else {
    wave_fill(list_ij, out_base, out_base + (cnt < cap_row ? cnt : cap_row), i, lane);
  }
  if (CNF) {
    cnacc = wave_sum(cnacc);
    if (lane == 0) {
      CN.cn[i] = (float)cnacc;
      if (cnt > M || half) *CN.flag = 1;
    }
  }
  if (MODE == MI_NL_MODE_MATRIX && !(flags & MI_NL_NO_PAD)) {
    const int used = cnt < M ? cnt : M;
    wave_fill(nm, out_base + used, out_base + M, fill_value, lane);
    if (nsh) wave_fill(nsh, (out_base + used) * 3, (out_base + M) * 3, 0, lane);
    if (K.words) wave_fill(reinterpret_cast<int*>(K.words), out_base + used, out_base + M, (int)NL_PK_PAD, lane);
  }
  if (DUAL) {
    if (lane == 0) D.num[i] = cnt2;
    if (!(flags & MI_NL_NO_PAD)) {
      const long long ob = (long long)i * D.M;
      const int used = cnt2 < D.M ? cnt2 : D.M;
      wave_fill(D.nm, ob + used, ob + D.M, fill_value, lane);
      if (D.nsh) wave_fill(D.nsh, (ob + used) * 3, (ob + D.M) * 3, 0, lane);
    }
  }
}

__global__ __launch_bounds__(256) void nl_matrix_to_coo_kernel(const int* __restrict__ nm, const int* __restrict__ nsh,
                                                               const int* __restrict__ ptr, int N, int M, int fill_value,
                                                               int* __restrict__ ij, int* __restrict__ sh, long long P) {
  const int lane = threadIdx.x & (MI_WAVE - 1);
  const int i = __builtin_amdgcn_readfirstlane(blockIdx.x * (blockDim.x / MI_WAVE) + (threadIdx.x / MI_WAVE));
  if (i >= N) return;
  const long long base = ptr[i];
  const int room = ptr[i + 1] - ptr[i];
  const unsigned long long lt = (1ull << lane) - 1ull;
  int cnt = 0;
  for (int t0 = 0; t0 < M; t0 += MI_WAVE) {
    const int t = t0 + lane;
    int j = fill_value;
    if (t < M) j = nm[(long long)i * M + t];
    const bool keep = (t < M) && (j != fill_value);
    const unsigned long long mask = __ballot(keep);
    const int slot = cnt + __popcll(mask & lt);
    if (keep && slot < room) {
      ij[base + slot] = i;
      ij[P + base + slot] = j;
      if (sh) {
        const int* sp = nsh + ((long long)i * M + t) * 3;
        int* dp = sh + (base + slot) * 3;
        dp[0] = sp[0]; dp[1] = sp[1]; dp[2] = sp[2];
      }
    }
    cnt += __popcll(mask);
  }
}

template <class T>
__device__ void ref_cells_per_dim(const T* cell9, const uint8_t* pbc3, T cutoff, int cpd[3], int* radius) {
  T inv[9];
  inverse3(cell9, inv);
  for (int d = 0; d < 3; ++d) {
    T col[3] = {inv[d], inv[3 + d], inv[6 + d]};
    T face = T(1) / sqrt(col[0] * col[0] + col[1] * col[1] + col[2] * col[2]);
    int c = (int)(face / cutoff);
    cpd[d] = c > 1 ? c : 1;
    if (radius) radius[d] = (cpd[d] == 1 && !pbc3[d]) ? 0 : (int)ceil(cutoff * (T)cpd[d] / face);
  }
}
template <class T>
__global__ void nl_estimate_sizes_kernel(const T* __restrict__ cell, const uint8_t* __restrict__ pbc, int B, T cutoff, int max_nbins,
                                         int* __restrict__ ncells, int* __restrict__ radius) {
  int s = blockIdx.x * blockDim.x + threadIdx.x;
  if (s >= B) return;
  int cpd[3];
  ref_cells_per_dim(cell + 9 * (size_t)s, pbc + 3 * (size_t)s, cutoff, cpd, radius + 3 * (size_t)s);
  long long tot = (long long)cpd[0] * cpd[1] * cpd[2];
  while (tot > max_nbins) {
    for (int d = 0; d < 3; ++d) cpd[d] = cpd[d] / 2 > 1 ? cpd[d] / 2 : 1;
    tot = (long long)cpd[0] * cpd[1] * cpd[2];
  }
  ncells[s] = (int)tot;
}

template <class T>
__global__ void nl_cache_binsize_kernel(const T* __restrict__ cell, const uint8_t* __restrict__ pbc, int B, T cutoff, int max_total_cells,
                                        int batched, int* __restrict__ cpd_out, int* __restrict__ cell_off ) {
  for (int s = threadIdx.x; s < B; s += blockDim.x) {
    int cpd[3];
    ref_cells_per_dim<T>(cell + 9 * (size_t)s, pbc + 3 * (size_t)s, cutoff, cpd, nullptr);
    long long tot = (long long)cpd[0] * cpd[1] * cpd[2];
    const long long mult = batched ? B : 1;
    while (tot * mult > max_total_cells) {
      for (int d = 0; d < 3; ++d) cpd[d] = cpd[d] / 2 > 1 ? cpd[d] / 2 : 1;
      tot = (long long)cpd[0] * cpd[1] * cpd[2];
    }
    for (int d = 0; d < 3; ++d) cpd_out[3 * (size_t)s + d] = cpd[d];
  }
  __syncthreads();
  if (threadIdx.x == 0) {
    int off = 0;
    for (int s = 0; s < B; ++s) { cell_off[s] = off; off += cpd_out[3 * s] * cpd_out[3 * s + 1] * cpd_out[3 * s + 2]; }
    cell_off[B] = off;
  }
}
template <class T>
__global__ void nl_cache_assign_kernel(const T* __restrict__ pos, const T* __restrict__ cell, const uint8_t* __restrict__ pbc,
                                       const int* __restrict__ batch_idx, int N, const int* __restrict__ cpd, const int* __restrict__ cell_off,
                                       int* __restrict__ keys, int* __restrict__ counts, int* __restrict__ atom_shift, int* __restrict__ atom_cell) {
  int i = blockIdx.x * blockDim.x + threadIdx.x;
  const bool in = i < N;
  int key = 0;
  if (in) {
    const int s = batch_idx ? batch_idx[i] : 0;
    T inv[9];
    inverse3(cell + 9 * (size_t)s, inv);
    T p[3] = {pos[3 * (size_t)i], pos[3 * (size_t)i + 1], pos[3 * (size_t)i + 2]}, frac[3];
    rowvec_mat3(p, inv, frac);
    int c[3];
    for (int d = 0; d < 3; ++d) {
      const int n = cpd[3 * s + d];
      int v = (int)floor(frac[d] * (T)n), w = 0;
      if (pbc[3 * s + d]) floor_divmod(v, n, w, c[d]);
      else c[d] = v < 0 ? 0 : (v >= n ? n - 1 : v);
      atom_shift[3 * (size_t)i + d] = w;
      atom_cell[3 * (size_t)i + d] = c[d];
    }
    key = cell_off[s] + c[0] + cpd[3 * s] * (c[1] + cpd[3 * s + 1] * c[2]);
    keys[i] = key;
  }
  bs_wave_add<false>(counts, key, in);
}
__global__ void nl_cache_add_offsets_kernel(int* __restrict__ starts, const int* __restrict__ block_off, int C) {
  const int c = blockIdx.x * blockDim.x + threadIdx.x;
  if (c < C) starts[c] += block_off[c / BS_CHUNK];
}
__global__ void nl_cache_scatter_kernel(const int* __restrict__ keys, int N, int* __restrict__ cursor, int* __restrict__ ids) {
  const int i = blockIdx.x * blockDim.x + threadIdx.x;
  const bool in = i < N;
  const int slot = bs_wave_add<true>(cursor, in ? keys[i] : 0, in);
  if (in) ids[slot] = i;
}
__global__ void nl_cache_rank_kernel(const int* __restrict__ ids, const int* __restrict__ keys, const int* __restrict__ cursor_end,
                                     const int* __restrict__ counts, int N, int* __restrict__ cell_atoms) {
  const int p = blockIdx.x * blockDim.x + threadIdx.x;
  if (p >= N) return;
  const int i = ids[p], key = keys[i];
  const int e = cursor_end[key], b = e - counts[key];
  int rank = 0;
  for (int q = b; q < e; ++q) rank += ids[q] < i ? 1 : 0;
  cell_atoms[b + rank] = i;
}
__global__ void nl_cache_rewind_kernel(int* __restrict__ starts, const int* __restrict__ counts, int C) {
  const int c = blockIdx.x * blockDim.x + threadIdx.x;
  if (c < C) starts[c] -= counts[c];
}

__device__ __forceinline__ unsigned long long nl_key(double v) {
  const unsigned long long b = (unsigned long long)__double_as_longlong(v);
  return (b >> 63) ? ~b : (b | 0x8000000000000000ull);
}
__device__ __forceinline__ double nl_unkey(unsigned long long k) {
  const unsigned long long b = (k >> 63) ? (k & 0x7fffffffffffffffull) : ~k;
  return __longlong_as_double((long long)b);
}
template <class T>
__global__ void nl_bbox_kernel(const T* __restrict__ pos, const int* __restrict__ batch_idx, int N, unsigned long long* __restrict__ box ) {
  const int i = blockIdx.x * blockDim.x + threadIdx.x;
  const bool in = i < N;
  const int s = in ? (batch_idx ? batch_idx[i] : 0) : -1;
  double v[3] = {0, 0, 0};
  if (in) { v[0] = pos[3 * (size_t)i]; v[1] = pos[3 * (size_t)i + 1]; v[2] = pos[3 * (size_t)i + 2]; }
  const int s0 = __shfl(s, 0, MI_WAVE);
  if (__all(!in || s == s0) && s0 >= 0) {
#pragma unroll
    for (int d = 0; d < 3; ++d) {
      double lo = in ? v[d] : INFINITY, hi = in ? v[d] : -INFINITY;
      for (int o = MI_WAVE / 2; o; o >>= 1) { lo = fmin(lo, __shfl_xor(lo, o, MI_WAVE)); hi = fmax(hi, __shfl_xor(hi, o, MI_WAVE)); }
      if ((threadIdx.x & (MI_WAVE - 1)) == 0) { atomicMin(&box[6 * (size_t)s0 + d], nl_key(lo)); atomicMax(&box[6 * (size_t)s0 + 3 + d], nl_key(hi)); }
    }
  } else if (in) {
#pragma unroll
    for (int d = 0; d < 3; ++d) { atomicMin(&box[6 * (size_t)s + d], nl_key(v[d])); atomicMax(&box[6 * (size_t)s + 3 + d], nl_key(v[d])); }
  }
}
template <class T>
__global__ void nl_bbox_finish_kernel(const unsigned long long* __restrict__ box, int B, T* __restrict__ cell, T* __restrict__ origin) {
  const int s = blockIdx.x * blockDim.x + threadIdx.x;
  if (s >= B) return;
  for (int k = 0; k < 9; ++k) cell[9 * (size_t)s + k] = T(0);
  for (int d = 0; d < 3; ++d) {
    const unsigned long long klo = box[6 * (size_t)s + d], khi = box[6 * (size_t)s + 3 + d];
    const bool empty = klo == ~0ull;
    const double lo = empty ? 0.0 : nl_unkey(klo), hi = empty ? 0.0 : nl_unkey(khi);
    const T span = (T)lo == (T)lo ? (T)(hi - lo) : T(0);
    cell[9 * (size_t)s + 4 * d] = (span > T(1) ? span : T(1)) * (T)1.001;
    origin[3 * (size_t)s + d] = (T)lo;
  }
}

template <class T>
__global__ void nl_cells_changed_kernel(const T* __restrict__ pos, const T* __restrict__ cell, const int* __restrict__ atom_cell,
                                        const int* __restrict__ cpd, const uint8_t* __restrict__ pbc, int N, uint8_t* __restrict__ flag) {
  const int i = blockIdx.x * blockDim.x + threadIdx.x;
  if (i >= N) return;
  T inv[9];
  inverse3(cell, inv);
  const T p[3] = {pos[3 * (size_t)i], pos[3 * (size_t)i + 1], pos[3 * (size_t)i + 2]};
  T frac[3];
  rowvec_mat3(p, inv, frac);
  bool changed = false;
#pragma unroll
  for (int d = 0; d < 3; ++d) {
    const int n = cpd[d];
    int c = (int)floor(frac[d] * (T)n);
    if (pbc[d]) { c = c % n; if (c < 0) c += n; }
    else c = c < 0 ? 0 : (c >= n ? n - 1 : c);
    changed = changed || (c != atom_cell[3 * (size_t)i + d]);
  }
  if (changed) *flag = 1;
}
template <class T>
__global__ void nl_moved_kernel(const T* __restrict__ ref, const T* __restrict__ cur, T threshold, int N, uint8_t* __restrict__ flag) {
  const int i = blockIdx.x * blockDim.x + threadIdx.x;
  if (i >= N) return;
  const T dx = cur[3 * (size_t)i] - ref[3 * (size_t)i], dy = cur[3 * (size_t)i + 1] - ref[3 * (size_t)i + 1], dz = cur[3 * (size_t)i + 2] - ref[3 * (size_t)i + 2];
  if (sqrt(dx * dx + dy * dy + dz * dz) > threshold) *flag = 1;
}

template <class T>
int nl_neighbors_impl(const T* pos, int N, const T* cell, const uint8_t* pbc, const int* batch_idx, int B, double cutoff, int mode, int flags,
                      int* nm, int* nsh, int* num, int M, int fill_value, const int* ptr, int* list_ij, int* list_sh, long long P,
                      const T* origin, char* ws, const NlLayout& L, hipStream_t st, const NlSecond<T>* second = nullptr,
                      NlPacked K = NlPacked{nullptr, nullptr}, const mi_nl_cn_request* cnreq = nullptr, void* cn_block = nullptr) {
  auto* sys = reinterpret_cast<NlSys<T>*>(ws + L.sys);
  auto* glob = reinterpret_cast<NlGlobal*>(ws + L.glob);
  int* natoms = reinterpret_cast<int*>(ws + L.natoms);
  int* keys_in = reinterpret_cast<int*>(ws + L.keys_in);
  int* keys_out = reinterpret_cast<int*>(ws + L.keys_out);
  int* vals_in = reinterpret_cast<int*>(ws + L.vals_in);
  int* vals_out = reinterpret_cast<int*>(ws + L.vals_out);
  auto* wrap = reinterpret_cast<short4*>(ws + L.wrap);
  auto* swrap = reinterpret_cast<short4*>(ws + L.swrap);
  auto* spos = reinterpret_cast<typename Vec4<T>::type*>(ws + L.spos);
  int* cell_start = reinterpret_cast<int*>(ws + L.cell_start);
  const T rc = (T)cutoff;
  NlCn CN{nullptr, nullptr, nullptr, 0.0f};
  NlCnBuild CB{nullptr, nullptr, 0, 0.0f, nullptr, nullptr, nullptr, 0, nullptr};
  if (cnreq && cn_block) {
    const float K1 = mi_cn_scale(cnreq->k1);
    int* hdr = reinterpret_cast<int*>(cn_block);
    CN = NlCn{reinterpret_cast<const float*>(ws + L.srk), reinterpret_cast<float*>((char*)cn_block + MI_CN_HEADER_BYTES), hdr, K1};
    CB = NlCnBuild{cnreq->numbers, cnreq->covalent_radii, cnreq->nz, K1, reinterpret_cast<float*>(ws + L.srk),
                   reinterpret_cast<unsigned long long*>(cn_block) + MI_CN_SLOT_OFFSET_U64, cell, 9 * B, batch_idx};
    MI_REQUIRE(!(flags & MI_NL_REUSE_GRID), "a search that sums coordination numbers bins its atoms itself (no MI_NL_REUSE_GRID)");
  }
  const T rc2 = (flags & MI_NL_NAIVE_EXPR) ? (T)(cutoff * cutoff) : rc * rc;

  if (!(flags & MI_NL_REUSE_GRID)) {
    mi_timing_begin("nl_build(setup+assign+binsort+gather)", (void*)st);
    const int* nat = nullptr;
    if (batch_idx && B > 1) {
      MI_HIP_CHECK(hipMemsetAsync(natoms, 0, sizeof(int) * (size_t)B, st));
      nl_count_atoms_kernel<<<mi_blocks(N, 256), 256, 0, st>>>(batch_idx, N, natoms);
      MI_LAUNCH_CHECK();
      nat = natoms;
    }
    const BsScratch bins = bs_carve(reinterpret_cast<int*>(ws + L.bins), L.cell_cap + 2);
    const long long zero_words = (2 * bins.cap + 3) / 4;
    const int zero_blocks = (int)(zero_words / 2048 < 1 ? 1 : (zero_words / 2048 > 255 ? 255 : zero_words / 2048));
    const int table_blocks = mi_blocks((long long)B * (NL_PRUNE_R + 1) * (NL_PRUNE_R + 1), 256);
    nl_setup_kernel<T><<<1 + table_blocks + zero_blocks, 256, 0, st>>>(cell, pbc, nat, N, B, rc, origin, sys, glob, table_blocks,
                                                                       reinterpret_cast<int4*>(bins.count), zero_words, K.words ? K.flag : nullptr,
                                                                       CN.flag, CN.K);
    MI_LAUNCH_CHECK();
    nl_assign_kernel<T><<<mi_blocks(N, 256), 256, 0, st>>>(pos, batch_idx, N, sys, keys_in, bins.count, wrap, glob);
    MI_LAUNCH_CHECK();
    MI_HIP_CHECK(bs_sort(bins, keys_in, N, &glob->total_cells, vals_out, cell_start, st));
    nl_rank_gather_kernel<T><<<mi_blocks(CB.srk && 9 * B > N ? 9 * B : N, 256), 256, 0, st>>>(pos, vals_out, keys_in, cell_start, wrap, N, spos, swrap, keys_out, CB);
    MI_LAUNCH_CHECK();
    mi_timing_end((void*)st);
  }
  const int blocks = mi_blocks(N, 4);
  const NlSecond<T> none{T(0), nullptr, nullptr, nullptr, 0};
  const NlPacked nopk{nullptr, nullptr};
  if (K.words && (flags & MI_NL_REUSE_GRID)) MI_HIP_CHECK(hipMemsetAsync(K.flag, 0, sizeof(int), st));
  if (second) {
    MI_TIMED("nl_query_dual", st,
             (nl_query_kernel<T, MI_NL_MODE_MATRIX, true><<<blocks, 256, 0, st>>>(spos, swrap, keys_out, cell_start, batch_idx, sys, glob, N, rc2, flags, nm, nsh,
                                                                                 num, M, fill_value, ptr, list_ij, list_sh, P, *second, nopk),
              nl_query_tiled_kernel<T, MI_NL_MODE_MATRIX, false, true><<<nl_tiled_grid(), 256, 0, st>>>(spos, swrap, cell_start, sys, glob, B, rc2, flags, nm, nsh,
                                                                                                       num, M, fill_value, ptr, list_ij, list_sh, P, *second, nopk)));
    MI_LAUNCH_CHECK();
    return MI_OK;
  }
#define MI_NLQ(MODE_)                                                                                                              \
  nl_query_kernel<T, MODE_><<<blocks, 256, 0, st>>>(spos, swrap, keys_out, cell_start, batch_idx, sys, glob, N, rc2, flags, nm, nsh, num, M, \
                                                    fill_value, ptr, list_ij, list_sh, P, none, K)
#define MI_NLT(MODE_)                                                                                                                    \
  do {                                                                                                                                   \
    if ((flags & (MI_NL_HALF_FILL | MI_NL_NAIVE_EXPR)) == 0)                                                                             \
      nl_query_tiled_kernel<T, MODE_, true><<<nl_tiled_grid(), 256, 0, st>>>(spos, swrap, cell_start, sys, glob, B, rc2, flags, nm, nsh, num, \
                                                                          M, fill_value, ptr, list_ij, list_sh, P, none, K);             \
    else                                                                                                                                 \
      nl_query_tiled_kernel<T, MODE_, false><<<nl_tiled_grid(), 256, 0, st>>>(spos, swrap, cell_start, sys, glob, B, rc2, flags, nm, nsh, num, \
                                                                           M, fill_value, ptr, list_ij, list_sh, P, none, K);            \
  } while (0)
  if (mode == MI_NL_MODE_MATRIX && CN.cn) {
    MI_TIMED(sizeof(T) == 4 ? "nl_query_matrix_f32" : "nl_query_matrix_f64", st,
             (nl_query_kernel<T, MI_NL_MODE_MATRIX, false, true><<<blocks, 256, 0, st>>>(spos, swrap, keys_out, cell_start, batch_idx, sys, glob, N, rc2, flags, nm,
                                                                                        nsh, num, M, fill_value, ptr, list_ij, list_sh, P, none, K, CN),
              nl_query_tiled_kernel<T, MI_NL_MODE_MATRIX, true, false, true><<<nl_tiled_grid(), 256, 0, st>>>(
                  spos, swrap, cell_start, sys, glob, B, rc2, flags, nm, nsh, num, M, fill_value, ptr, list_ij, list_sh, P, none, K, CN)));
  } else if (mode == MI_NL_MODE_MATRIX) MI_TIMED(sizeof(T) == 4 ? "nl_query_matrix_f32" : "nl_query_matrix_f64", st, MI_NLQ(MI_NL_MODE_MATRIX); MI_NLT(MI_NL_MODE_MATRIX));
  else if (mode == MI_NL_MODE_COUNT) MI_TIMED("nl_query_count", st, MI_NLQ(MI_NL_MODE_COUNT); MI_NLT(MI_NL_MODE_COUNT));
  else MI_TIMED("nl_query_csr", st, MI_NLQ(MI_NL_MODE_CSR); MI_NLT(MI_NL_MODE_CSR));
#undef MI_NLT
#undef MI_NLQ
  MI_LAUNCH_CHECK();
  return MI_OK;
}

template <class T>
int nl_cache_impl(const T* pos, int N, const T* cell, const uint8_t* pbc, const int* batch_idx, int B, double cutoff, int C, int* cpd,
                  int* atom_shift, int* atom_cell, int* counts, int* starts, int* cell_atoms, char* ws, const NlLayout& L, hipStream_t st) {
  int* keys_in = reinterpret_cast<int*>(ws + L.keys_in);
  int* ids = reinterpret_cast<int*>(ws + L.keys_out);
  int* cell_off = reinterpret_cast<int*>(ws + L.cell_start);
  int* block_sum = reinterpret_cast<int*>(ws + L.bins);
  const int nblocks = (C + BS_CHUNK - 1) / BS_CHUNK;
  MI_REQUIRE((size_t)(2 * nblocks + 8) <= bs_scratch_ints(L.cell_cap + 2), "max_total_cells too large for this workspace");
  int* block_off = block_sum + nblocks + 4;
  nl_cache_binsize_kernel<T><<<1, 256, 0, st>>>(cell, pbc, B, (T)cutoff, C, batch_idx != nullptr, cpd, cell_off);
  MI_LAUNCH_CHECK();
  MI_HIP_CHECK(hipMemsetAsync(counts, 0, sizeof(int) * (size_t)C, st));
  nl_cache_assign_kernel<T><<<mi_blocks(N, 256), 256, 0, st>>>(pos, cell, pbc, batch_idx, N, cpd, cell_off, keys_in, counts, atom_shift, atom_cell);
  MI_LAUNCH_CHECK();
  MI_HIP_CHECK(hipMemcpyAsync(starts, counts, sizeof(int) * (size_t)C, hipMemcpyDeviceToDevice, st));
  bs_scan_partial_kernel<<<nblocks, 256, 0, st>>>(starts, nullptr, C, block_sum);
  bs_scan_blocks_kernel<<<1, 256, 0, st>>>(block_sum, nblocks, block_off);
  nl_cache_add_offsets_kernel<<<mi_blocks(C, 256), 256, 0, st>>>(starts, block_off, C);
  nl_cache_scatter_kernel<<<mi_blocks(N, 256), 256, 0, st>>>(keys_in, N, starts, ids);
  nl_cache_rank_kernel<<<mi_blocks(N, 256), 256, 0, st>>>(ids, keys_in, starts, counts, N, cell_atoms);
  nl_cache_rewind_kernel<<<mi_blocks(C, 256), 256, 0, st>>>(starts, counts, C);
  MI_LAUNCH_CHECK();
  return MI_OK;
}

}

extern "C" {

size_t mi_nl_workspace_bytes(int n_atoms, int n_systems, int dtype) {
  if (n_atoms < 0 || n_systems < 1) return 0;
  return nl_layout(n_atoms, n_systems, dtype).total;
}

}
static int nl_neighbors_entry(const void* positions, int n_atoms, const void* cell, const uint8_t* pbc, const int32_t* batch_idx, int n_systems,
                    double cutoff, int dtype, int mode, int flags, int32_t* neighbor_matrix, int32_t* neighbor_matrix_shifts,
                    int32_t* num_neighbors, int max_neighbors, int fill_value, const int32_t* neighbor_ptr, int32_t* list_ij,
                    int32_t* list_shifts, long long n_pairs, const void* bin_origin, void* workspace, size_t workspace_bytes, void* stream, void* packed_out,
                    const mi_nl_cn_request* cnreq = nullptr, void* cn_block = nullptr) {
  MI_REQUIRE(dtype == MI_F32 || dtype == MI_F64, "dtype must be MI_F32 or MI_F64");
  MI_REQUIRE(n_atoms >= 0 && n_systems >= 1, "n_atoms >= 0 and n_systems >= 1");
  MI_REQUIRE(cutoff > 0, "cutoff must be positive");
  MI_REQUIRE(mode >= 0 && mode <= 2, "mode");
  if (n_atoms == 0) return MI_OK;
  MI_REQUIRE(positions && cell && pbc && workspace, "null pointer");
  if (mode == MI_NL_MODE_MATRIX) MI_REQUIRE(neighbor_matrix && num_neighbors && max_neighbors >= 0, "matrix outputs");
  if (mode == MI_NL_MODE_COUNT) MI_REQUIRE(num_neighbors != nullptr, "num_neighbors");
  if (mode == MI_NL_MODE_CSR) MI_REQUIRE(neighbor_ptr && list_ij, "csr outputs");
  if (flags & MI_NL_NO_SHIFTS) neighbor_matrix_shifts = nullptr;
  NlLayout L = nl_layout(n_atoms, n_systems, dtype);
  if (workspace_bytes < L.total) { mi_set_error("workspace too small: %zu < %zu", workspace_bytes, L.total); return MI_EWORKSPACE; }
  hipStream_t st = (hipStream_t)stream;
  NlPacked K{nullptr, nullptr};
  if (packed_out) {
    MI_REQUIRE(mode == MI_NL_MODE_MATRIX && neighbor_matrix_shifts && !(flags & (MI_NL_NO_PAD | MI_NL_HALF_FILL)) && n_atoms < (1 << 26),
               "packed companion: full (not half-filled) padded matrix with shifts, n_atoms < 2^26");
    K.flag = reinterpret_cast<int*>(packed_out);
    K.words = reinterpret_cast<unsigned*>(packed_out) + 64;
  }
  if (cnreq) MI_REQUIRE(packed_out && cn_block && cnreq->numbers && cnreq->covalent_radii && cnreq->nz >= 2, "coordination numbers: companion, output block, numbers and radii");
  if (dtype == MI_F32)
    return nl_neighbors_impl<float>((const float*)positions, n_atoms, (const float*)cell, pbc, batch_idx, n_systems, cutoff, mode, flags,
                                    neighbor_matrix, neighbor_matrix_shifts, num_neighbors, max_neighbors, fill_value, neighbor_ptr, list_ij,
                                    list_shifts, n_pairs, (const float*)bin_origin, (char*)workspace, L, st, nullptr, K, cnreq, cn_block);
  return nl_neighbors_impl<double>((const double*)positions, n_atoms, (const double*)cell, pbc, batch_idx, n_systems, cutoff, mode, flags,
                                   neighbor_matrix, neighbor_matrix_shifts, num_neighbors, max_neighbors, fill_value, neighbor_ptr, list_ij,
                                   list_shifts, n_pairs, (const double*)bin_origin, (char*)workspace, L, st, nullptr, K, cnreq, cn_block);
}

extern "C" {
int mi_nl_neighbors(const void* positions, int n_atoms, const void* cell, const uint8_t* pbc, const int32_t* batch_idx, int n_systems,
                    double cutoff, int dtype, int mode, int flags, int32_t* neighbor_matrix, int32_t* neighbor_matrix_shifts,
                    int32_t* num_neighbors, int max_neighbors, int fill_value, const int32_t* neighbor_ptr, int32_t* list_ij,
                    int32_t* list_shifts, long long n_pairs, const void* bin_origin, void* workspace, size_t workspace_bytes, void* stream) {
  return nl_neighbors_entry(positions, n_atoms, cell, pbc, batch_idx, n_systems, cutoff, dtype, mode, flags, neighbor_matrix, neighbor_matrix_shifts,
                            num_neighbors, max_neighbors, fill_value, neighbor_ptr, list_ij, list_shifts, n_pairs, bin_origin, workspace,
                            workspace_bytes, stream, nullptr);
}

size_t mi_nl_packed_bytes(int n_atoms, int max_neighbors) {
  if (n_atoms <= 0 || max_neighbors <= 0 || n_atoms >= (1 << 26)) return 0;
  return 256 + sizeof(unsigned) * (size_t)n_atoms * (size_t)max_neighbors;
}

int mi_nl_neighbors_packed(const void* positions, int n_atoms, const void* cell, const uint8_t* pbc, const int32_t* batch_idx, int n_systems,
                           double cutoff, int dtype, int flags, int32_t* neighbor_matrix, int32_t* neighbor_matrix_shifts,
                           int32_t* num_neighbors, int max_neighbors, int fill_value, const void* bin_origin, void* workspace,
                           size_t workspace_bytes, void* packed_out, size_t packed_bytes, void* stream) {
  MI_REQUIRE(packed_out != nullptr && packed_bytes >= mi_nl_packed_bytes(n_atoms, max_neighbors) && mi_nl_packed_bytes(n_atoms, max_neighbors) > 0,
             "packed_out: mi_nl_packed_bytes(n_atoms, max_neighbors) bytes");
  return nl_neighbors_entry(positions, n_atoms, cell, pbc, batch_idx, n_systems, cutoff, dtype, MI_NL_MODE_MATRIX, flags, neighbor_matrix,
                            neighbor_matrix_shifts, num_neighbors, max_neighbors, fill_value, nullptr, nullptr, nullptr, 0, bin_origin, workspace,
                            workspace_bytes, stream, packed_out);
}

size_t mi_nl_cn_bytes(int n_atoms) { return n_atoms > 0 ? MI_CN_HEADER_BYTES + sizeof(float) * (size_t)n_atoms : 0; }

int mi_nl_neighbors_packed_cn(const void* positions, int n_atoms, const void* cell, const uint8_t* pbc, const int32_t* batch_idx, int n_systems,
                              double cutoff, int dtype, int flags, int32_t* neighbor_matrix, int32_t* neighbor_matrix_shifts,
                              int32_t* num_neighbors, int max_neighbors, int fill_value, const void* bin_origin, void* workspace,
                              size_t workspace_bytes, void* packed_out, size_t packed_bytes, const mi_nl_cn_request* request, void* cn_out,
                              size_t cn_bytes, void* stream) {
  MI_REQUIRE(packed_out != nullptr && packed_bytes >= mi_nl_packed_bytes(n_atoms, max_neighbors) && mi_nl_packed_bytes(n_atoms, max_neighbors) > 0,
             "packed_out: mi_nl_packed_bytes(n_atoms, max_neighbors) bytes");
  MI_REQUIRE(request != nullptr && cn_out != nullptr && cn_bytes >= mi_nl_cn_bytes(n_atoms), "cn_out: mi_nl_cn_bytes(n_atoms) bytes and a request");
  return nl_neighbors_entry(positions, n_atoms, cell, pbc, batch_idx, n_systems, cutoff, dtype, MI_NL_MODE_MATRIX, flags, neighbor_matrix,
                            neighbor_matrix_shifts, num_neighbors, max_neighbors, fill_value, nullptr, nullptr, nullptr, 0, bin_origin, workspace,
                            workspace_bytes, stream, packed_out, request, cn_out);
}

int mi_nl_neighbors_dual(const void* positions, int n_atoms, const void* cell, const uint8_t* pbc, const int32_t* batch_idx, int n_systems,
                         double cutoff_short, double cutoff_long, int dtype, int flags, int32_t* neighbor_matrix_short,
                         int32_t* neighbor_matrix_shifts_short, int32_t* num_neighbors_short, int max_neighbors_short,
                         int32_t* neighbor_matrix_long, int32_t* neighbor_matrix_shifts_long, int32_t* num_neighbors_long, int max_neighbors_long,
                         int fill_value, const void* bin_origin, void* workspace, size_t workspace_bytes, void* stream) {
  MI_REQUIRE(dtype == MI_F32 || dtype == MI_F64, "dtype must be MI_F32 or MI_F64");
  MI_REQUIRE(n_atoms >= 0 && n_systems >= 1, "n_atoms >= 0 and n_systems >= 1");
  MI_REQUIRE(cutoff_short > 0 && cutoff_long >= cutoff_short, "0 < cutoff_short <= cutoff_long");
  if (n_atoms == 0) return MI_OK;
  MI_REQUIRE(positions && cell && pbc && workspace, "null pointer");
  MI_REQUIRE(neighbor_matrix_short && num_neighbors_short && max_neighbors_short >= 0 && neighbor_matrix_long && num_neighbors_long &&
                 max_neighbors_long >= 0, "matrix outputs");
  if (flags & MI_NL_NO_SHIFTS) neighbor_matrix_shifts_short = neighbor_matrix_shifts_long = nullptr;
  NlLayout L = nl_layout(n_atoms, n_systems, dtype);
  if (workspace_bytes < L.total) { mi_set_error("workspace too small: %zu < %zu", workspace_bytes, L.total); return MI_EWORKSPACE; }
  hipStream_t st = (hipStream_t)stream;
  if (dtype == MI_F32) {
    const float r1 = (float)cutoff_short;
    const NlSecond<float> sec{(flags & MI_NL_NAIVE_EXPR) ? (float)(cutoff_short * cutoff_short) : r1 * r1, neighbor_matrix_short,
                              neighbor_matrix_shifts_short, num_neighbors_short, max_neighbors_short};
    return nl_neighbors_impl<float>((const float*)positions, n_atoms, (const float*)cell, pbc, batch_idx, n_systems, cutoff_long, MI_NL_MODE_MATRIX,
                                    flags, neighbor_matrix_long, neighbor_matrix_shifts_long, num_neighbors_long, max_neighbors_long, fill_value,
                                    nullptr, nullptr, nullptr, 0, (const float*)bin_origin, (char*)workspace, L, st, &sec);
  }
  const double r1 = cutoff_short;
  const NlSecond<double> sec{(flags & MI_NL_NAIVE_EXPR) ? cutoff_short * cutoff_short : r1 * r1, neighbor_matrix_short, neighbor_matrix_shifts_short,
                             num_neighbors_short, max_neighbors_short};
  return nl_neighbors_impl<double>((const double*)positions, n_atoms, (const double*)cell, pbc, batch_idx, n_systems, cutoff_long, MI_NL_MODE_MATRIX,
                                   flags, neighbor_matrix_long, neighbor_matrix_shifts_long, num_neighbors_long, max_neighbors_long, fill_value,
                                   nullptr, nullptr, nullptr, 0, (const double*)bin_origin, (char*)workspace, L, st, &sec);
}

int mi_nl_matrix_to_coo(const int32_t* neighbor_matrix, const int32_t* neighbor_matrix_shifts, const int32_t* neighbor_ptr, int n_atoms,
                             int max_neighbors, int fill_value, int32_t* list_ij, int32_t* list_shifts, long long n_pairs, void* stream) {
  if (n_atoms == 0 || n_pairs == 0) return MI_OK;
  MI_REQUIRE(neighbor_matrix && neighbor_ptr && list_ij, "null pointer");
  nl_matrix_to_coo_kernel<<<mi_blocks(n_atoms, 4), 256, 0, (hipStream_t)stream>>>(neighbor_matrix, neighbor_matrix_shifts, neighbor_ptr, n_atoms,
                                                                                  max_neighbors, fill_value, list_ij,
                                                                                  neighbor_matrix_shifts ? list_shifts : nullptr, n_pairs);
  MI_LAUNCH_CHECK();
  return MI_OK;
}

int mi_nl_bounding_cells(const void* positions, const int32_t* batch_idx, int n_atoms, int n_systems, int dtype, void* cell_out,
                         void* origin_out, void* scratch, void* stream) {
  MI_REQUIRE(dtype == MI_F32 || dtype == MI_F64, "dtype");
  MI_REQUIRE(n_systems >= 1 && cell_out && origin_out && scratch, "null pointer");
  MI_REQUIRE(n_atoms == 0 || positions, "positions");
  hipStream_t st = (hipStream_t)stream;
  unsigned long long* box = (unsigned long long*)scratch;
  MI_HIP_CHECK(hipMemsetAsync(box, 0xff, sizeof(unsigned long long) * 6 * (size_t)n_systems, st));
  MI_HIP_CHECK(hipMemset2DAsync(box + 3, sizeof(unsigned long long) * 6, 0, sizeof(unsigned long long) * 3, (size_t)n_systems, st));
  if (n_atoms > 0) {
    if (dtype == MI_F32) nl_bbox_kernel<float><<<mi_blocks(n_atoms, 256), 256, 0, st>>>((const float*)positions, batch_idx, n_atoms, box);
    else nl_bbox_kernel<double><<<mi_blocks(n_atoms, 256), 256, 0, st>>>((const double*)positions, batch_idx, n_atoms, box);
    MI_LAUNCH_CHECK();
  }
  if (dtype == MI_F32) nl_bbox_finish_kernel<float><<<mi_blocks(n_systems, 256), 256, 0, st>>>(box, n_systems, (float*)cell_out, (float*)origin_out);
  else nl_bbox_finish_kernel<double><<<mi_blocks(n_systems, 256), 256, 0, st>>>(box, n_systems, (double*)cell_out, (double*)origin_out);
  MI_LAUNCH_CHECK();
  return MI_OK;
}

int mi_nl_cells_changed(const void* positions, const void* cell, const int32_t* atom_to_cell_mapping, const int32_t* cells_per_dimension,
                        const uint8_t* pbc, int n_atoms, int dtype, uint8_t* flag, void* stream) {
  MI_REQUIRE(dtype == MI_F32 || dtype == MI_F64, "dtype");
  if (n_atoms <= 0) return MI_OK;
  MI_REQUIRE(positions && cell && atom_to_cell_mapping && cells_per_dimension && pbc && flag, "null pointer");
  hipStream_t st = (hipStream_t)stream;
  if (dtype == MI_F32)
    nl_cells_changed_kernel<float><<<mi_blocks(n_atoms, 256), 256, 0, st>>>((const float*)positions, (const float*)cell, atom_to_cell_mapping,
                                                                           cells_per_dimension, pbc, n_atoms, flag);
  else
    nl_cells_changed_kernel<double><<<mi_blocks(n_atoms, 256), 256, 0, st>>>((const double*)positions, (const double*)cell, atom_to_cell_mapping,
                                                                            cells_per_dimension, pbc, n_atoms, flag);
  MI_LAUNCH_CHECK();
  return MI_OK;
}

int mi_nl_moved_beyond_skin(const void* reference_positions, const void* current_positions, double threshold, int n_atoms, int dtype,
                            uint8_t* flag, void* stream) {
  MI_REQUIRE(dtype == MI_F32 || dtype == MI_F64, "dtype");
  if (n_atoms <= 0) return MI_OK;
  MI_REQUIRE(reference_positions && current_positions && flag, "null pointer");
  hipStream_t st = (hipStream_t)stream;
  if (dtype == MI_F32)
    nl_moved_kernel<float><<<mi_blocks(n_atoms, 256), 256, 0, st>>>((const float*)reference_positions, (const float*)current_positions,
                                                                   (float)threshold, n_atoms, flag);
  else
    nl_moved_kernel<double><<<mi_blocks(n_atoms, 256), 256, 0, st>>>((const double*)reference_positions, (const double*)current_positions,
                                                                    threshold, n_atoms, flag);
  MI_LAUNCH_CHECK();
  return MI_OK;
}

int mi_nl_estimate_sizes(const void* cell, const uint8_t* pbc, int n_systems, double cutoff, int max_nbins, int dtype, int32_t* number_of_cells,
                         int32_t* neighbor_search_radius, void* stream) {
  MI_REQUIRE(dtype == MI_F32 || dtype == MI_F64, "dtype");
  MI_REQUIRE(cell && pbc && number_of_cells && neighbor_search_radius && n_systems >= 1, "null pointer");
  hipStream_t st = (hipStream_t)stream;
  if (dtype == MI_F32)
    nl_estimate_sizes_kernel<float><<<mi_blocks(n_systems, 128), 128, 0, st>>>((const float*)cell, pbc, n_systems, (float)cutoff, max_nbins,
                                                                               number_of_cells, neighbor_search_radius);
  else
    nl_estimate_sizes_kernel<double><<<mi_blocks(n_systems, 128), 128, 0, st>>>((const double*)cell, pbc, n_systems, cutoff, max_nbins,
                                                                                number_of_cells, neighbor_search_radius);
  MI_LAUNCH_CHECK();
  return MI_OK;
}

int mi_nl_build_cell_cache(const void* positions, int n_atoms, const void* cell, const uint8_t* pbc, const int32_t* batch_idx, int n_systems,
                           double cutoff, int dtype, int max_total_cells, int32_t* cells_per_dimension, int32_t* atom_periodic_shifts,
                           int32_t* atom_to_cell_mapping, int32_t* atoms_per_cell_count, int32_t* cell_atom_start_indices,
                           int32_t* cell_atom_list, void* workspace, size_t workspace_bytes, void* stream) {
  MI_REQUIRE(dtype == MI_F32 || dtype == MI_F64, "dtype");
  if (n_atoms == 0) return MI_OK;
  MI_REQUIRE(positions && cell && pbc && workspace && cells_per_dimension && atom_periodic_shifts && atom_to_cell_mapping &&
                 atoms_per_cell_count && cell_atom_start_indices && cell_atom_list,
             "null pointer");
  MI_REQUIRE(max_total_cells >= n_systems, "max_total_cells");
  NlLayout L = nl_layout(n_atoms, n_systems, dtype);
  if (workspace_bytes < L.total) { mi_set_error("workspace too small: %zu < %zu", workspace_bytes, L.total); return MI_EWORKSPACE; }
  hipStream_t st = (hipStream_t)stream;
  if (dtype == MI_F32)
    return nl_cache_impl<float>((const float*)positions, n_atoms, (const float*)cell, pbc, batch_idx, n_systems, cutoff, max_total_cells,
                                cells_per_dimension, atom_periodic_shifts, atom_to_cell_mapping, atoms_per_cell_count, cell_atom_start_indices,
                                cell_atom_list, (char*)workspace, L, st);
  return nl_cache_impl<double>((const double*)positions, n_atoms, (const double*)cell, pbc, batch_idx, n_systems, cutoff, max_total_cells,
                               cells_per_dimension, atom_periodic_shifts, atom_to_cell_mapping, atoms_per_cell_count, cell_atom_start_indices,
                               cell_atom_list, (char*)workspace, L, st);
}

}
```

nvalchemi-toolkit-ops_amd/nvalchemiops/_capi.py:

```python
from __future__ import annotations

import contextvars
import ctypes
import functools
import os

import torch

_LIB_PATH = os.path.join(os.path.dirname(os.path.abspath(__file__)), "lib", "libnvalchemiops_hip.so")
_LIB = None

MI_F32, MI_F64 = 0, 1
NL_MATRIX, NL_COUNT, NL_CSR = 0, 1, 2
NL_HALF_FILL, NL_NAIVE_EXPR, NL_REUSE_GRID, NL_NO_SHIFTS, NL_NO_PAD = 1, 2, 4, 8, 16
EW_FORCES, EW_CHARGE_GRAD = 1, 2


class NativeLibraryError(RuntimeError):
    """The HIP library is missing or failed: there is deliberately no fallback path."""


class MiD3Params(ctypes.Structure):
    _fields_ = [("rcov", ctypes.c_void_p), ("r4r2", ctypes.c_void_p), ("c6ab", ctypes.c_void_p), ("cn_ref", ctypes.c_void_p),
                ("nz", ctypes.c_int), ("a1", ctypes.c_float), ("a2", ctypes.c_float), ("s6", ctypes.c_float), ("s8", ctypes.c_float),
                ("k1", ctypes.c_float), ("k3", ctypes.c_float), ("s5_on", ctypes.c_float), ("s5_off", ctypes.c_float)]


class MiD3ZeroParams(ctypes.Structure):
    _fields_ = [("rs6", ctypes.c_float), ("rs8", ctypes.c_float), ("alpha", ctypes.c_float), ("beta", ctypes.c_float), ("r0ab", ctypes.c_void_p)]


class MiD4Params(ctypes.Structure):
    _fields_ = ([(name, ctypes.c_void_p) for name in ("rcov", "en", "r4r2", "zeff", "gam", "n_ref", "ngw", "cn_ref", "q_ref", "c6_ref")]
                + [("nz", ctypes.c_int)]
                + [(name, ctypes.c_float) for name in ("a1", "a2", "s6", "s8", "k_cn", "k4", "k5", "k6", "wf", "ga", "gc", "cn_cutoff")])


class MiNlCnRequest(ctypes.Structure):
    _fields_ = [("numbers", ctypes.c_void_p), ("covalent_radii", ctypes.c_void_p), ("nz", ctypes.c_int), ("k1", ctypes.c_float)]


def lib() -> ctypes.CDLL:
    global _LIB
    if _LIB is None:
        if not os.path.exists(_LIB_PATH):
            raise NativeLibraryError(
                f"{_LIB_PATH} not found: build it with `python nvalchemi-toolkit-ops_amd/build_native.py` "
                "(hipcc --offload-arch=gfx950). This package has no CPU or PyTorch fallback.")
        L = ctypes.CDLL(_LIB_PATH)
        L.mi_last_error.restype = ctypes.c_char_p
        L.mi_nl_workspace_bytes.restype = ctypes.c_size_t
        L.mi_nl_workspace_bytes.argtypes = [ctypes.c_int, ctypes.c_int, ctypes.c_int]
        L.mi_spline_spread_workspace_bytes.restype = ctypes.c_size_t
        L.mi_pme_solve_scratch_bytes.restype = ctypes.c_size_t
        L.mi_pme_solve_scratch_bytes.argtypes = [ctypes.c_int] * 6
        L.mi_fft_lds_scratch_bytes.restype = ctypes.c_size_t
        L.mi_fft_lds_scratch_bytes.argtypes = [ctypes.c_int] * 5
        L.mi_spline_spread_workspace_bytes.argtypes = [ctypes.c_int] * 5
        L.mi_spline_spread_workspace_bytes_for.restype = ctypes.c_size_t
        L.mi_spline_spread_workspace_bytes_for.argtypes = [ctypes.c_int] * 7
        L.mi_spline_spread_order_offset.restype = ctypes.c_longlong
        L.mi_spline_spread_order_offset.argtypes = [ctypes.c_int] * 6
        L.mi_nl_packed_bytes.restype = ctypes.c_size_t
        L.mi_nl_packed_bytes.argtypes = [ctypes.c_int, ctypes.c_int]
        L.mi_nl_cn_bytes.restype = ctypes.c_size_t
        L.mi_nl_cn_bytes.argtypes = [ctypes.c_int]
        if hasattr(L, "mi_d3_workspace_bytes"):
            L.mi_d3_workspace_bytes.restype = ctypes.c_size_t
            L.mi_d3_workspace_bytes.argtypes = [ctypes.c_int, ctypes.c_int, ctypes.c_int]
            L.mi_d3_workspace_bytes_packed.restype = ctypes.c_size_t
            L.mi_d3_workspace_bytes_packed.argtypes = [ctypes.c_int] * 4
            L.mi_d3_workspace_bytes_entries.restype = ctypes.c_size_t
            L.mi_d3_workspace_bytes_entries.argtypes = [ctypes.c_int, ctypes.c_int, ctypes.c_int, ctypes.c_longlong]
        if hasattr(L, "mi_d3_atm"):
            for name in ("mi_d3_atm_workspace_bytes", "mi_d3_atm_visits_offset"):
                getattr(L, name).restype = ctypes.c_size_t
                getattr(L, name).argtypes = [ctypes.c_int, ctypes.c_int, ctypes.c_int]
            L.mi_d3_atm_tile.restype = ctypes.c_int
            L.mi_d3_atm_tile.argtypes = []
            L.mi_d3_atm.restype = ctypes.c_int
            L.mi_d3_atm.argtypes = ([ctypes.c_void_p, ctypes.c_void_p, ctypes.c_int, ctypes.c_int, ctypes.c_void_p, ctypes.c_void_p, ctypes.c_void_p,
                                     ctypes.c_int, ctypes.c_int, ctypes.c_void_p, ctypes.c_void_p, ctypes.c_int, ctypes.c_void_p, ctypes.c_float,
                                     ctypes.c_float, ctypes.c_float, ctypes.c_int] + [ctypes.c_void_p] * 4 + [ctypes.c_size_t, ctypes.c_void_p])
        if hasattr(L, "mi_d3_zero_atm"):
            L.mi_d3_zero_atm.restype = ctypes.c_int
            L.mi_d3_zero_atm.argtypes = ([ctypes.c_void_p, ctypes.c_void_p, ctypes.c_int, ctypes.c_int, ctypes.c_void_p, ctypes.c_void_p, ctypes.c_void_p,
                                          ctypes.c_int, ctypes.c_int, ctypes.c_void_p, ctypes.c_void_p, ctypes.c_int, ctypes.c_void_p, ctypes.c_float,
                                          ctypes.c_float, ctypes.c_float, ctypes.c_float, ctypes.c_void_p, ctypes.c_int] + [ctypes.c_void_p] * 4
                                         + [ctypes.c_size_t, ctypes.c_void_p])
        vp, i, sz = ctypes.c_void_p, ctypes.c_int, ctypes.c_size_t
        if hasattr(L, "mi_d4"):
            L.mi_d4_workspace_bytes.restype = sz
            L.mi_d4_workspace_bytes.argtypes = [i, i, i]
            L.mi_d4_species_slots.restype = i
            L.mi_d4_species_slots.argtypes = []
            L.mi_d4_fold_blocks.restype = i
            L.mi_d4_fold_blocks.argtypes = []
            L.mi_d4.restype = i
            L.mi_d4.argtypes = [vp, vp, i, i, vp, vp, vp, i, ctypes.c_longlong, i, vp, vp, i, vp, vp, i] + [vp] * 6 + [sz, vp]
        if hasattr(L, "mi_d4_atm"):
            for name in ("mi_d4_atm_workspace_bytes", "mi_d4_atm_visits_offset"):
                getattr(L, name).restype = sz
                getattr(L, name).argtypes = [i, i, i]
            L.mi_d4_atm_tile.restype = i
            L.mi_d4_atm_tile.argtypes = []
            L.mi_d4_atm.restype = i
            L.mi_d4_atm.argtypes = ([vp, vp, i, i, vp, vp, vp, i, i, vp, vp, i, vp, ctypes.c_float, ctypes.c_float, ctypes.c_float, i] + [vp] * 4
                                    + [sz, vp])
        L.mi_ewald_real_virial.restype = i
        L.mi_ewald_real_virial.argtypes = [vp, vp, vp, vp, vp, i, i, i, vp, vp, vp, i, i, i, vp, vp, vp, vp, sz, vp, i, i, vp, vp, vp]
        L.mi_ewald_recip_virial.restype = i
        L.mi_ewald_recip_virial.argtypes = [vp, vp, vp, vp, i, i, i, vp, vp]
        L.mi_pme_virial.restype = i
        L.mi_pme_virial.argtypes = [vp, vp, vp, vp, i, i, i, i, i, i, vp, vp, i, vp, vp, vp]
        for name in ("mi_ewald_virial_blocks", "mi_ewald_recip_virial_blocks", "mi_pme_virial_blocks"):
            getattr(L, name).restype = i
            getattr(L, name).argtypes = []
        L.mi_spline_spread_channels_workspace_bytes_for.restype = sz
        L.mi_spline_spread_channels_workspace_bytes_for.argtypes = [i] * 8
        L.mi_spline_spread_channels.restype = i
        L.mi_spline_spread_channels.argtypes = [vp, vp, vp, vp] + [i] * 9 + [vp, vp, sz, vp]
        L.mi_spline_gather_channels.restype = i
        L.mi_spline_gather_channels.argtypes = [vp, vp, vp, vp] + [i] * 8 + [vp, vp]
        L.mi_spline_gather_channels_frac_grad.restype = i
        L.mi_spline_gather_channels_frac_grad.argtypes = [vp, vp, vp, vp, vp] + [i] * 8 + [vp, vp]
        dbl = ctypes.c_double
        for name, args in (("mi_sph_harm", [vp, i, i, vp, vp]), ("mi_sph_harm_grad", [vp, i, i, vp, vp]), ("mi_gto_density", [vp, i, dbl, i, vp, vp]),
                           ("mi_gto_fourier", [vp, i, dbl, i, vp, vp, vp])):
            getattr(L, name).restype = i
            getattr(L, name).argtypes = args
        L.mi_gaussian_charges.restype = i
        L.mi_gaussian_charges.argtypes = [vp] * 6 + [i, i, i, vp, vp, vp, i, i, i] + [vp] * 6 + [sz, vp]
        L.mi_gaussian_charges_system_sums.restype = i
        L.mi_gaussian_charges_system_sums.argtypes = [vp, vp, vp, vp, i, i, i, vp, vp]
        L.mi_gaussian_charges_scratch_bytes.restype = sz
        L.mi_gaussian_charges_scratch_bytes.argtypes = [i, i]
        for name in ("mi_gaussian_charges_blocks", "mi_gaussian_charges_row_words"):
            getattr(L, name).restype = i
            getattr(L, name).argtypes = []
        L.mi_ewald_dipole_real.restype = i
        L.mi_ewald_dipole_real.argtypes = [vp] * 7 + [i, i, i, vp, vp, vp, i, i, i] + [vp] * 6 + [sz, vp]
        L.mi_ewald_dipole_structure_factors.restype = i
        L.mi_ewald_dipole_structure_factors.argtypes = [vp] * 6 + [i, i, i, i, vp, vp]
        L.mi_ewald_dipole_recip_gather.restype = i
        L.mi_ewald_dipole_recip_gather.argtypes = [vp] * 10 + [i, i, i, i] + [vp] * 5
        L.mi_ewald_dipole_recip_virial.restype = i
        L.mi_ewald_dipole_recip_virial.argtypes = [vp, vp, vp, vp, i, i, i, vp, vp]
        L.mi_ewald_dipole_real_scratch_bytes.restype = sz
        L.mi_ewald_dipole_real_scratch_bytes.argtypes = [i, i]
        L.mi_ewald_dipole_blocks.restype = i
        L.mi_ewald_dipole_blocks.argtypes = []
        L.mi_ewald_quadrupole_real.restype = i
        L.mi_ewald_quadrupole_real.argtypes = [vp] * 8 + [i, i, i, vp, vp, vp, i, i, i] + [vp] * 7 + [sz, vp]
        L.mi_ewald_quadrupole_structure_factors.restype = i
        L.mi_ewald_quadrupole_structure_factors.argtypes = [vp] * 7 + [i, i, i, i, vp, vp, vp]
        L.mi_ewald_quadrupole_recip_gather.restype = i
        L.mi_ewald_quadrupole_recip_gather.argtypes = [vp] * 11 + [i, i, i, i] + [vp] * 6
        L.mi_ewald_quadrupole_recip_virial.restype = i
        L.mi_ewald_quadrupole_recip_virial.argtypes = [vp, vp, vp, vp, vp, i, i, i, vp, vp]
        L.mi_ewald_quadrupole_real_scratch_bytes.restype = sz
        L.mi_ewald_quadrupole_real_scratch_bytes.argtypes = [i, i]
        L.mi_ewald_quadrupole_blocks.restype = i
        L.mi_ewald_quadrupole_blocks.argtypes = []
        L.mi_thole_dipole.restype = i
        L.mi_thole_dipole.argtypes = [vp] * 5 + [ctypes.c_double, vp, vp, i, i, i, vp, vp, vp, i, i, i] + [vp] * 7 + [sz, vp]
        L.mi_thole_dipole_scratch_bytes.restype = sz
        L.mi_thole_dipole_scratch_bytes.argtypes = [i, i]
        L.mi_thole_dipole_blocks.restype = i
        L.mi_thole_dipole_blocks.argtypes = []
        L.mi_coulomb_dipole.restype = i
        L.mi_coulomb_dipole.argtypes = [vp] * 6 + [i, i, i, vp, vp, vp, i, i, i] + [vp] * 6 + [sz, vp]
        L.mi_coulomb_quadrupole.restype = i
        L.mi_coulomb_quadrupole.argtypes = [vp] * 7 + [i, i, i, vp, vp, vp, i, i, i] + [vp] * 7 + [sz, vp]
        for name in ("mi_coulomb_dipole", "mi_coulomb_quadrupole"):
            getattr(L, name + "_scratch_bytes").restype = sz
            getattr(L, name + "_scratch_bytes").argtypes = [i, i]
            getattr(L, name + "_blocks").restype = i
            getattr(L, name + "_blocks").argtypes = []
        L.mi_pme_dipole_spread.restype = i
        L.mi_pme_dipole_spread.argtypes = [vp] * 6 + [i] * 7 + [vp, vp]
        L.mi_pme_dipole_gather.restype = i
        L.mi_pme_dipole_gather.argtypes = [vp] * 9 + [i] * 8 + [vp] * 5
        L.mi_pme_dipole_virial.restype = i
        L.mi_pme_dipole_virial.argtypes = [vp] * 5 + [i] * 6 + [vp, vp]
        L.mi_pme_dipole_virial_blocks.restype = i
        L.mi_pme_dipole_virial_blocks.argtypes = []
        L.mi_pme_quadrupole_spread.restype = i
        L.mi_pme_quadrupole_spread.argtypes = [vp] * 7 + [i] * 7 + [vp, vp]
        L.mi_pme_quadrupole_gather.restype = i
        L.mi_pme_quadrupole_gather.argtypes = [vp] * 10 + [i] * 8 + [vp] * 6
        L.mi_pme_quadrupole_virial.restype = i
        L.mi_pme_quadrupole_virial.argtypes = [vp] * 5 + [i] * 6 + [vp, vp]
        L.mi_pme_quadrupole_virial_blocks.restype = i
        L.mi_pme_quadrupole_virial_blocks.argtypes = []
        L.mi_qeq_pair_coefficients.restype = i
        L.mi_qeq_pair_coefficients.argtypes = [vp] * 6 + [i, i, i, vp, vp, vp, i, i, vp, vp, vp, vp]
        L.mi_qeq_apply.restype = i
        L.mi_qeq_apply.argtypes = [vp] * 6 + [i, i, vp, i, vp, vp, vp]
        L.mi_qeq_cg_update.restype = i
        L.mi_qeq_cg_update.argtypes = [vp] * 4 + [i, i, i] + [vp] * 7
        L.mi_qeq_cg_direction.restype = i
        L.mi_qeq_cg_direction.argtypes = [vp, vp, i, i, i, dbl, vp, vp, vp, vp, vp]
        for name in ("mi_qeq_blocks", "mi_qeq_state_words"):
            getattr(L, name).restype = i
            getattr(L, name).argtypes = []
        ll = ctypes.c_longlong
        L.mi_induced_pair_tensors.restype = i
        L.mi_induced_pair_tensors.argtypes = [vp] * 5 + [i, i, i, vp, vp, vp, i, i, ll, vp, vp, vp, vp, vp]
        L.mi_thole_induced_pair_tensors.restype = i
        L.mi_thole_induced_pair_tensors.argtypes = [vp] * 5 + [i, i, i, vp, vp, vp, i, i, ll, vp, vp, vp, vp, dbl, vp]
        L.mi_cluster_induced_pair_tensors.restype = i
        L.mi_cluster_induced_pair_tensors.argtypes = [vp, vp, i, i, vp, vp, i, i, ll, vp, vp, vp, vp, dbl, vp]
        L.mi_induced_apply.restype = i
        L.mi_induced_apply.argtypes = [vp] * 6 + [i, i, vp, i, ll, vp, vp, vp]
        L.mi_induced_dot.restype = i
        L.mi_induced_dot.argtypes = [vp, vp, vp, i, i, vp, vp]
        L.mi_induced_cg_update.restype = i
        L.mi_induced_cg_update.argtypes = [vp] * 4 + [i, i, i] + [vp] * 7
        L.mi_induced_cg_direction.restype = i
        L.mi_induced_cg_direction.argtypes = [vp, vp, vp, i, i, i, dbl, vp, vp, vp, vp, vp]
        for name in ("mi_induced_blocks", "mi_induced_state_words", "mi_induced_tensor_words", "mi_induced_unroll_depth"):
            getattr(L, name).restype = i
            getattr(L, name).argtypes = []
        L.mi_frame_rotate.restype = i
        L.mi_frame_rotate.argtypes = [vp] * 7 + [i, i, i, vp, vp, vp]
        L.mi_frame_adjoint.restype = i
        L.mi_frame_adjoint.argtypes = [vp] * 9 + [i, i, i] + [vp] * 5
        L.mi_frame_gather.restype = i
        L.mi_frame_gather.argtypes = [vp, vp, vp, ll, vp, vp, i, i, i, dbl, vp, vp, vp]
        for name in ("mi_frame_blocks", "mi_frame_block_threads"):
            getattr(L, name).restype = i
            getattr(L, name).argtypes = []
        _LIB = L
    return _LIB


def ewald_sym_words() -> int:
    L = lib()
    L.mi_ewald_symmetry_scratch_bytes.restype = ctypes.c_size_t
    return int(L.mi_ewald_symmetry_scratch_bytes()) // 8


def ewald_scratch_bytes(n_atoms: int, dtype: int) -> int:
    L = lib()
    L.mi_ewald_real_scratch_bytes.restype = ctypes.c_size_t
    return int(L.mi_ewald_real_scratch_bytes(int(n_atoms), int(dtype)))


def fold_virial(partial: torch.Tensor) -> torch.Tensor:
    xx, yy, zz, xy, xz, yz = partial.sum(1).unbind(-1)
    return torch.stack((xx, xy, xz, xy, yy, yz, xz, yz, zz), dim=-1).reshape(-1, 3, 3)


def fold_virial9(partial: torch.Tensor) -> torch.Tensor:
    return partial.sum(1).reshape(-1, 3, 3)


def check(rc: int, what: str) -> None:
    if rc != 0:
        raise NativeLibraryError(f"{what} failed (code {rc}): {lib().mi_last_error().decode()}")


def ptr(t: torch.Tensor | None):
    if t is None:
        return None
    return ctypes.c_void_p(t.data_ptr())


def stream_of(t: torch.Tensor):
    return ctypes.c_void_p(torch.cuda.current_stream(t.device).cuda_stream)


def dtype_code(dtype: torch.dtype) -> int:
    if dtype == torch.float32:
        return MI_F32
    if dtype == torch.float64:
        return MI_F64
    raise ValueError(f"Unsupported dtype: {dtype}")


def require_device(*tensors: torch.Tensor | None) -> torch.device:
    dev = None
    for t in tensors:
        if t is None:
            continue
        if not t.is_cuda:
            raise NativeLibraryError(
                "nvalchemiops (MI355X build) computes on ROCm devices only; got a tensor on "
                f"'{t.device}'. There is no CPU path in this package.")
        if dev is None:
            dev = t.device
        elif t.device != dev:
            raise ValueError(f"tensors on different devices: {dev} vs {t.device}")
    return dev


def check_per_atom(n: int, **named: torch.Tensor | None) -> None:
    for name, t in named.items():
        if t is not None and (t.dim() == 0 or t.shape[0] != n):
            raise ValueError(f"{name} must have one entry per atom: expected shape [{n}], got {tuple(t.shape)}")


def check_neighbor_data(n: int, *, neighbor_matrix=None, neighbor_matrix_shifts=None, neighbor_list=None, idx_j=None, neighbor_ptr=None,
                        neighbor_shifts=None, shifts_name: str = "neighbor_shifts", short_ptr_ok: bool = False, cell=None, num_systems=None,
                        alpha=None, **per_atom) -> None:
    check_per_atom(n, **per_atom)
    if neighbor_matrix is not None:
        if neighbor_matrix.dim() != 2 or neighbor_matrix.shape[0] != n:
            raise ValueError(f"neighbor_matrix must have shape [{n}, max_neighbors], got {tuple(neighbor_matrix.shape)}")
        want = (n, neighbor_matrix.shape[1], 3)
        if neighbor_matrix_shifts is not None and tuple(neighbor_matrix_shifts.shape) != want:
            raise ValueError(f"neighbor_matrix_shifts must have shape {list(want)} to match neighbor_matrix, got {tuple(neighbor_matrix_shifts.shape)}")
    if neighbor_list is not None:
        if neighbor_list.dim() != 2 or neighbor_list.shape[0] != 2:
            raise ValueError(f"neighbor_list must have shape [2, num_pairs], got {tuple(neighbor_list.shape)}")
        idx_j = neighbor_list[1]
    if idx_j is not None:
        if idx_j.dim() != 1:
            raise ValueError(f"idx_j must have shape [num_pairs], got {tuple(idx_j.shape)}")
        if neighbor_ptr is not None and (neighbor_ptr.dim() != 1 or (neighbor_ptr.shape[0] > n + 1 if short_ptr_ok else neighbor_ptr.shape[0] != n + 1)):
            raise ValueError(f"neighbor_ptr must have shape [{n + 1}] (num_atoms + 1), got {tuple(neighbor_ptr.shape)}")
        want = (idx_j.shape[0], 3)
        if neighbor_shifts is not None and tuple(neighbor_shifts.shape) != want:
            raise ValueError(f"{shifts_name} must have shape {list(want)} to match neighbor_list, got {tuple(neighbor_shifts.shape)}")
    if cell is not None:
        if cell.dim() not in (2, 3) or tuple(cell.shape[-2:]) != (3, 3):
            raise ValueError(f"cell must have shape [3, 3] or [num_systems, 3, 3], got {tuple(cell.shape)}")
        n_cells = cell.shape[0] if cell.dim() == 3 else 1
        if num_systems is not None and n_cells != int(num_systems):
            raise ValueError(f"cell must have shape [{int(num_systems)}, 3, 3] (one per system), got {tuple(cell.shape)}")
        if isinstance(alpha, torch.Tensor) and alpha.numel() > 1 and alpha.numel() != n_cells:
            raise ValueError(f"alpha has {alpha.numel()} values but there are {n_cells} systems")


SPLINE_REFERENCE_ORDERS = 0x100
_REFERENCE_SPLINE_ORDERS = os.environ.get("NVALCHEMIOPS_REFERENCE_SPLINE_ORDERS", "0") not in ("", "0")
_REFERENCE_SPLINE_ORDERS_CTX: contextvars.ContextVar = contextvars.ContextVar("nvalchemiops_reference_spline_orders", default=None)


def reference_spline_orders_active() -> bool:
    v = _REFERENCE_SPLINE_ORDERS_CTX.get()
    return _REFERENCE_SPLINE_ORDERS if v is None else bool(v)


SPLINE_RESOLVED = 0x200


def resolve_spline_order(order: int) -> int:
    order = int(order)
    if order & SPLINE_RESOLVED or torch.compiler.is_compiling():
        return order
    return (order & 0xff) | SPLINE_RESOLVED | (SPLINE_REFERENCE_ORDERS if reference_spline_orders_active() else 0)


def plain_spline_order(order: int) -> int:
    return int(order) & 0xff


def spline_order_arg(order: int) -> int:
    return resolve_spline_order(order) & (0xff | SPLINE_REFERENCE_ORDERS)


def cdouble(x: float):
    return ctypes.c_double(float(x))


def i32(t: torch.Tensor | None) -> torch.Tensor | None:
    if t is None:
        return None
    return t.to(torch.int32).contiguous()


def _on_device_of(args, kwargs):
    for a in (args if args else kwargs.values()):
        if isinstance(a, torch.Tensor):
            if a.is_cuda and a.device.index != torch.cuda.current_device():
                return a.device
            break
    return None


def eager(fn):
    inner = torch.compiler.disable(fn)

    @functools.wraps(fn)
    def entry(*args, **kwargs):
        dev = _on_device_of(args, kwargs)
        if dev is not None:
            with torch.cuda.device(dev):
                return inner(*args, **kwargs)
        return inner(*args, **kwargs)

    return entry


def hybrid(fn):
    inner = torch.compiler.disable(fn)

    @functools.wraps(fn)
    def entry(*args, **kwargs):
        if torch.compiler.is_compiling():
            return fn(*args, **kwargs)
        dev = _on_device_of(args, kwargs)
        if dev is not None:
            with torch.cuda.device(dev):
                return inner(*args, **kwargs)
        return inner(*args, **kwargs)

    return entry


def tracing() -> bool:
    return torch.compiler.is_compiling()


def traceable(fn):
    @functools.wraps(fn)
    def entry(*args, **kwargs):
        if torch.compiler.is_compiling():
            return fn(*args, **kwargs)
        dev = _on_device_of(args, kwargs)
        if dev is not None:
            with torch.cuda.device(dev):
                return fn(*args, **kwargs)
        return fn(*args, **kwargs)

    return entry
```

nvalchemi-toolkit-ops_amd/nvalchemiops/neighborlist/_engine.py:

```python
from __future__ import annotations

import ctypes
import os
import weakref

import torch

from nvalchemiops import _capi as C

_WS_BYTES: dict[tuple[int, int, int], int] = {}

_PACKED_POLICY = os.environ.get("NVALCHEMIOPS_NL_PACKED", "auto")
_PACKED_WANTED: set[tuple[int, int, int]] = set()
_PACKED_ATTR = "_nvalchemiops_packed"
_BUILT_ATTR = "_nvalchemiops_built"
_FULL_ATTR = "_nvalchemiops_full_list"
_D3CTX_ATTR = "_nvalchemiops_d3ctx"
_D3CTX_BY_SHAPE: dict = {}
_VERIFY_STRIDE = max(0, int(os.environ.get("NVALCHEMIOPS_NL_PACKED_VERIFY", "64") or 0))
_verify_calls = 0


def verify_args() -> tuple[int, int]:
    global _verify_calls
    _verify_calls += 1
    return _VERIFY_STRIDE, (_verify_calls - 1) & 0x3fffffff


class D3SearchContext:
    __slots__ = ("numbers", "rcov", "k1", "_src")

    def __init__(self, numbers: torch.Tensor, covalent_radii: torch.Tensor, k1: float = 16.0):
        self.numbers = numbers.detach().to(torch.int32).contiguous()
        self.rcov = covalent_radii.detach().to(device=numbers.device, dtype=torch.float32).contiguous()
        self.k1 = float(k1)
        self._src = (weakref.ref(numbers), numbers._version, weakref.ref(covalent_radii), covalent_radii._version)

    def describes(self, numbers: torch.Tensor, covalent_radii: torch.Tensor, k1: float) -> bool:
        n_ref, n_ver, r_ref, r_ver = self._src
        return (n_ref() is numbers and numbers._version == n_ver and r_ref() is covalent_radii and covalent_radii._version == r_ver
                and float(k1) == self.k1)


def attach_dftd3_context(neighbor_matrix: torch.Tensor, numbers: torch.Tensor, covalent_radii: torch.Tensor, k1: float = 16.0) -> None:
    setattr(neighbor_matrix, _D3CTX_ATTR, D3SearchContext(numbers, covalent_radii, k1))
    want_packed_companion(neighbor_matrix.device, int(neighbor_matrix.shape[0]), int(neighbor_matrix.shape[1]))


def learn_dftd3_context(neighbor_matrix: torch.Tensor, numbers: torch.Tensor, covalent_radii: torch.Tensor, k1: float) -> None:
    if _PACKED_POLICY != "auto" or not neighbor_matrix.is_cuda:
        return
    if getattr(neighbor_matrix, _PACKED_ATTR, None) is None and getattr(neighbor_matrix, _BUILT_ATTR, None) is None:
        return
    ctx = getattr(neighbor_matrix, _D3CTX_ATTR, None)
    try:
        if ctx is not None and ctx.describes(numbers, covalent_radii, k1):
            return
        if numbers.shape[0] != neighbor_matrix.shape[0]:
            return
        key = (neighbor_matrix.device.index, int(neighbor_matrix.shape[0]), int(neighbor_matrix.shape[1]))
        known = _D3CTX_BY_SHAPE.get(key)
        ctx = known if (known is not None and known.describes(numbers, covalent_radii, k1)) else D3SearchContext(numbers, covalent_radii, k1)
        setattr(neighbor_matrix, _D3CTX_ATTR, ctx)
        if len(_D3CTX_BY_SHAPE) > 64:
            _D3CTX_BY_SHAPE.clear()
        _D3CTX_BY_SHAPE[key] = ctx
    except Exception:
        pass


def invalidate(*tensors: torch.Tensor) -> None:
    for t in tensors:
        if t is None:
            continue
        for attr in (_PACKED_ATTR, _BUILT_ATTR, _FULL_ATTR):
            if hasattr(t, attr):
                delattr(t, attr)
        owner = getattr(t, "_nvalchemiops_owner", None)
        nm = owner() if owner is not None else None
        if nm is not None and nm is not t:
            for attr in (_PACKED_ATTR, _BUILT_ATTR, _FULL_ATTR):
                if hasattr(nm, attr):
                    delattr(nm, attr)


class PackedCompanion:
    __slots__ = ("words", "cn", "nm_version", "nsh_ref", "nsh_version", "n_atoms", "row_width", "fill_value")

    def __init__(self, words, nm, nsh, fill_value, cn=None):
        self.words = words
        self.cn = cn
        self.nm_version = nm._version
        self.nsh_ref = weakref.ref(nsh)
        self.nsh_version = nsh._version
        self.n_atoms, self.row_width = int(nm.shape[0]), int(nm.shape[1])
        self.fill_value = int(fill_value)

    def matches(self, nm: torch.Tensor, nsh: torch.Tensor | None, fill_value: int) -> bool:
        return (nsh is not None and self.nsh_ref() is nsh and nm._version == self.nm_version and nsh._version == self.nsh_version
                and tuple(nm.shape) == (self.n_atoms, self.row_width) and int(fill_value) == self.fill_value
                and nm.dtype == torch.int32 and nsh.dtype == torch.int32 and nm.is_contiguous() and nsh.is_contiguous())


class FullListRecord:
    __slots__ = ("nm_version", "nsh_ref", "nsh_version", "num_ref", "num_version", "n_atoms", "row_width", "fill_value")

    def __init__(self, nm, nsh, num, fill_value):
        self.nm_version = nm._version
        self.nsh_ref, self.nsh_version = weakref.ref(nsh), nsh._version
        self.num_ref, self.num_version = weakref.ref(num), num._version
        self.n_atoms, self.row_width = int(nm.shape[0]), int(nm.shape[1])
        self.fill_value = int(fill_value)

    def counts(self, nm: torch.Tensor, nsh: torch.Tensor | None):
        num = self.num_ref()
        ok = (nsh is not None and num is not None and self.nsh_ref() is nsh and nm._version == self.nm_version and nsh._version == self.nsh_version
              and num._version == self.num_version and tuple(nm.shape) == (self.n_atoms, self.row_width) and nm.dtype == torch.int32
              and nsh.dtype == torch.int32 and num.dtype == torch.int32 and nm.is_contiguous() and nsh.is_contiguous() and num.is_contiguous()
              and num.device == nm.device)
        return num if ok else None


def full_list_counts(nm: torch.Tensor | None, nsh: torch.Tensor | None):
    rec = getattr(nm, _FULL_ATTR, None) if nm is not None else None
    if rec is None:
        return None
    try:
        return rec.counts(nm, nsh)
    except Exception:
        return None


def _record_full_list(nm, nsh, num, fill_value, qualifies: bool) -> None:
    if not qualifies or num is None:
        return
    try:
        setattr(nm, _FULL_ATTR, FullListRecord(nm, nsh, num, fill_value))
        setattr(nsh, "_nvalchemiops_owner", weakref.ref(nm))
    except Exception:
        pass


def want_packed_companion(device: torch.device, n_atoms: int, row_width: int) -> None:
    if len(_PACKED_WANTED) > 64:
        _PACKED_WANTED.clear()
    _PACKED_WANTED.add((device.index, int(n_atoms), int(row_width)))


def _written(*tensors) -> None:
    for t in tensors:
        if t is None:
            continue
        for attr in (_PACKED_ATTR, _BUILT_ATTR, _FULL_ATTR):
            if hasattr(t, attr):
                delattr(t, attr)
        try:
            torch.autograd.graph.increment_version(t)
        except Exception:
            pass


def packed_companion(nm: torch.Tensor, nsh: torch.Tensor | None, fill_value: int):
    rec = getattr(nm, _PACKED_ATTR, None)
    if rec is not None:
        try:
            if rec.matches(nm, nsh, fill_value):
                return rec
        except Exception:
            pass
        return None
    if _PACKED_POLICY == "auto" and nsh is not None and getattr(nm, _BUILT_ATTR, None) == nm._version and nm.is_cuda:
        if len(_PACKED_WANTED) > 64:
            _PACKED_WANTED.clear()
        _PACKED_WANTED.add((nm.device.index, int(nm.shape[0]), int(nm.shape[1])))
    return None


def workspace(n_atoms: int, n_systems: int, dtype: torch.dtype, device: torch.device) -> torch.Tensor:
    key = (n_atoms, n_systems, C.dtype_code(dtype))
    nbytes = _WS_BYTES.get(key)
    if nbytes is None:
        nbytes = int(C.lib().mi_nl_workspace_bytes(*key))
        _WS_BYTES[key] = nbytes
    return torch.empty(nbytes, dtype=torch.uint8, device=device)


def canon_positions(positions: torch.Tensor) -> torch.Tensor:
    pos = positions.detach()
    if pos.dtype in (torch.float16, torch.bfloat16):
        pos = pos.float()
    return pos.contiguous()


def canon_geometry(positions: torch.Tensor, cell: torch.Tensor, pbc: torch.Tensor, n_systems: int | None = None):
    pos = canon_positions(positions)
    cell = cell.detach()
    cell = (cell if cell.ndim == 3 else cell.unsqueeze(0)).to(dtype=pos.dtype, device=pos.device).contiguous()
    pbc = pbc.reshape(-1, 3).to(device=pos.device, dtype=torch.bool)
    if pbc.shape[0] != cell.shape[0]:
        pbc = pbc.expand(cell.shape[0], 3)
    return pos, cell, pbc.contiguous()


def check_outputs(n, dev, nm, nsh, num, which="", width=None):
    m = (nm.shape[1] if nm.dim() == 2 else -1) if nm is not None else (-1 if width is None else int(width))
    for name, t, shape in ((f"neighbor_matrix{which}", nm, (n, m)), (f"num_neighbors{which}", num, (n,)),
                           (f"neighbor_matrix_shifts{which}", nsh, (n, m, 3))):
        if t is None:
            continue
        if t.dtype != torch.int32 or not t.is_contiguous() or t.device != dev or tuple(t.shape) != shape:
            raise ValueError(f"{name} must be a contiguous int32 tensor of shape {shape} on {dev}, got {t.dtype} {tuple(t.shape)} on {t.device}"
                             f"{'' if t.is_contiguous() else ' (non-contiguous)'}")


def check_cache(n, n_systems, dev, cells_per_dimension, atom_periodic_shifts, atom_to_cell_mapping, atoms_per_cell_count,
                cell_atom_start_indices, cell_atom_list):
    cap = atoms_per_cell_count.shape[0] if atoms_per_cell_count.dim() == 1 else -1
    for name, t, ok, want in (
            ("cells_per_dimension", cells_per_dimension, cells_per_dimension.numel() >= 3 * n_systems, f"[{n_systems}, 3] or [3]"),
            ("atom_periodic_shifts", atom_periodic_shifts, atom_periodic_shifts.dim() == 2 and atom_periodic_shifts.shape[0] >= n
             and atom_periodic_shifts.shape[1] == 3, f"[{n}, 3]"),
            ("atom_to_cell_mapping", atom_to_cell_mapping, atom_to_cell_mapping.dim() == 2 and atom_to_cell_mapping.shape[0] >= n
             and atom_to_cell_mapping.shape[1] == 3, f"[{n}, 3]"),
            ("atoms_per_cell_count", atoms_per_cell_count, cap >= n_systems, f"[max_total_cells >= {n_systems}]"),
            ("cell_atom_start_indices", cell_atom_start_indices, cell_atom_start_indices.dim() == 1 and cell_atom_start_indices.shape[0] >= cap,
             f"[{cap}] to match atoms_per_cell_count"),
            ("cell_atom_list", cell_atom_list, cell_atom_list.dim() == 1 and cell_atom_list.shape[0] >= n, f"[{n}]")):
        if t.dtype != torch.int32 or not t.is_contiguous() or t.device != dev or not ok:
            raise ValueError(f"{name} must be a contiguous int32 tensor of shape {want} (or longer) on {dev}, got {t.dtype} {tuple(t.shape)} "
                             f"on {t.device}{'' if t.is_contiguous() else ' (non-contiguous)'}")


def run(pos, cell, pbc, batch_idx, cutoff, mode, flags, *, nm=None, nsh=None, num=None, max_neighbors=0, fill_value=0,
        nptr=None, list_ij=None, list_sh=None, n_pairs=0, ws=None, origin=None):
    n = pos.shape[0]
    nsys = cell.shape[0]
    if ws is None:
        ws = workspace(n, nsys, pos.dtype, pos.device)
    if mode == C.NL_MATRIX:
        _written(nm, nsh, num)
    rc = C.lib().mi_nl_neighbors(
        C.ptr(pos), n, C.ptr(cell), C.ptr(pbc), C.ptr(batch_idx), nsys, C.cdouble(cutoff), C.dtype_code(pos.dtype), mode, flags,
        C.ptr(nm), C.ptr(nsh), C.ptr(num), int(max_neighbors), int(fill_value), C.ptr(nptr), C.ptr(list_ij), C.ptr(list_sh),
        ctypes.c_longlong(int(n_pairs)), C.ptr(origin), C.ptr(ws), ctypes.c_size_t(ws.numel()), C.stream_of(pos))
    C.check(rc, "mi_nl_neighbors")
    return ws


def neighbor_matrix(pos, cell, pbc, batch_idx, cutoff, max_neighbors, fill_value, half_fill, nm, nsh, num, *, naive=False,
                    want_shifts=True, pad=True, origin=None):
    flags = (C.NL_HALF_FILL if half_fill else 0) | (C.NL_NAIVE_EXPR if naive else 0)
    if not want_shifts:
        flags |= C.NL_NO_SHIFTS
    if not pad:
        flags |= C.NL_NO_PAD
    if C.tracing():
        torch.ops.nvalchemiops.neighbor_search(pos, cell, pbc, batch_idx, cutoff, flags, fill_value, nm, nsh if want_shifts else None, num,
                                               origin)
        return
    n = pos.shape[0]
    qualifies = (want_shifts and pad and not half_fill and nsh is not None and nm.is_contiguous() and nsh.is_contiguous() and int(fill_value) >= n
                 and int(max_neighbors) > 0)
    emit = qualifies and (_PACKED_POLICY == "1" or (_PACKED_POLICY == "auto" and (pos.device.index, n, int(max_neighbors)) in _PACKED_WANTED))
    nbytes = int(C.lib().mi_nl_packed_bytes(n, int(max_neighbors))) if emit else 0
    if nbytes == 0:
        run(pos, cell, pbc, batch_idx, cutoff, C.NL_MATRIX, flags, nm=nm, nsh=nsh if want_shifts else None, num=num,
            max_neighbors=max_neighbors, fill_value=fill_value, origin=origin)
        _record_full_list(nm, nsh, num, fill_value, qualifies)
        if qualifies and _PACKED_POLICY == "auto":
            try:
                setattr(nm, _BUILT_ATTR, nm._version)
            except Exception:
                pass
        return
    old = getattr(nm, _PACKED_ATTR, None)
    words = old.words if (old is not None and old.words.numel() == nbytes and old.words.device == pos.device) else torch.empty(nbytes, dtype=torch.uint8, device=pos.device)
    ws = workspace(n, cell.shape[0], pos.dtype, pos.device)
    ctx = getattr(nm, _D3CTX_ATTR, None)
    if ctx is None and _PACKED_POLICY == "auto":
        ctx = _D3CTX_BY_SHAPE.get((pos.device.index, n, int(max_neighbors)))
    if ctx is not None and (ctx.numbers.shape[0] != n or ctx.numbers.device != pos.device):
        ctx = None
    _written(nm, nsh, num)
    cn = None
    if ctx is not None:
        cn_bytes = int(C.lib().mi_nl_cn_bytes(n))
        cn = old.cn if (old is not None and old.cn is not None and old.cn.numel() == cn_bytes and old.cn.device == pos.device) else torch.empty(cn_bytes, dtype=torch.uint8, device=pos.device)
        req = C.MiNlCnRequest(numbers=ctx.numbers.data_ptr(), covalent_radii=ctx.rcov.data_ptr(), nz=int(ctx.rcov.shape[0]), k1=ctx.k1)
        rc = C.lib().mi_nl_neighbors_packed_cn(
            C.ptr(pos), n, C.ptr(cell), C.ptr(pbc), C.ptr(batch_idx), cell.shape[0], C.cdouble(cutoff), C.dtype_code(pos.dtype), flags,
            C.ptr(nm), C.ptr(nsh), C.ptr(num), int(max_neighbors), int(fill_value), C.ptr(origin), C.ptr(ws), ctypes.c_size_t(ws.numel()),
            C.ptr(words), ctypes.c_size_t(nbytes), ctypes.byref(req), C.ptr(cn), ctypes.c_size_t(cn_bytes), C.stream_of(pos))
        C.check(rc, "mi_nl_neighbors_packed_cn")
    else:
        rc = C.lib().mi_nl_neighbors_packed(
            C.ptr(pos), n, C.ptr(cell), C.ptr(pbc), C.ptr(batch_idx), cell.shape[0], C.cdouble(cutoff), C.dtype_code(pos.dtype), flags,
            C.ptr(nm), C.ptr(nsh), C.ptr(num), int(max_neighbors), int(fill_value), C.ptr(origin), C.ptr(ws), ctypes.c_size_t(ws.numel()),
            C.ptr(words), ctypes.c_size_t(nbytes), C.stream_of(pos))
        C.check(rc, "mi_nl_neighbors_packed")
    _record_full_list(nm, nsh, num, fill_value, qualifies)
    try:
        setattr(nm, _PACKED_ATTR, PackedCompanion(words, nm, nsh, fill_value, cn=cn))
        setattr(nsh, "_nvalchemiops_owner", weakref.ref(nm))
    except Exception:
        pass


def neighbor_matrix_dual(pos, cell, pbc, batch_idx, cutoff_short, cutoff_long, fill_value, half_fill, short, long_, *, naive=True, want_shifts=True,
                         origin=None):
    flags = (C.NL_HALF_FILL if half_fill else 0) | (C.NL_NAIVE_EXPR if naive else 0)
    if not want_shifts:
        flags |= C.NL_NO_SHIFTS
    n, nsys = pos.shape[0], cell.shape[0]
    (nm1, nsh1, num1), (nm2, nsh2, num2) = short, long_
    if C.tracing():
        torch.ops.nvalchemiops.neighbor_search_dual(pos, cell, pbc, batch_idx, cutoff_short, cutoff_long, flags, fill_value, nm1,
                                                    nsh1 if want_shifts else None, num1, nm2, nsh2 if want_shifts else None, num2, origin)
        return
    ws = workspace(n, nsys, pos.dtype, pos.device)
    _written(nm1, nsh1, num1, nm2, nsh2, num2)
    rc = C.lib().mi_nl_neighbors_dual(
        C.ptr(pos), n, C.ptr(cell), C.ptr(pbc), C.ptr(batch_idx), nsys, C.cdouble(cutoff_short), C.cdouble(cutoff_long), C.dtype_code(pos.dtype), flags,
        C.ptr(nm1), C.ptr(nsh1 if want_shifts else None), C.ptr(num1), int(nm1.shape[1]),
        C.ptr(nm2), C.ptr(nsh2 if want_shifts else None), C.ptr(num2), int(nm2.shape[1]),
        int(fill_value), C.ptr(origin), C.ptr(ws), ctypes.c_size_t(ws.numel()), C.stream_of(pos))
    C.check(rc, "mi_nl_neighbors_dual")


@torch.compiler.disable
def neighbor_csr(pos, cell, pbc, batch_idx, cutoff, half_fill, *, naive=False, want_shifts=True, max_neighbors=None, origin=None):
    n = pos.shape[0]
    dev = pos.device
    flags = (C.NL_HALF_FILL if half_fill else 0) | (C.NL_NAIVE_EXPR if naive else 0)
    num = torch.empty(n, dtype=torch.int32, device=dev)
    ws = run(pos, cell, pbc, batch_idx, cutoff, C.NL_COUNT, flags, num=num, origin=origin)
    nptr = torch.zeros(n + 1, dtype=torch.int32, device=dev)
    torch.cumsum(num, dim=0, out=nptr[1:])
    total, max_count = (int(v) for v in torch.stack([nptr[-1], num.max()]).tolist())
    if max_neighbors is not None and max_count > max_neighbors:
        from nvalchemiops.neighborlist.neighbor_utils import NeighborOverflowError

        raise NeighborOverflowError(max_neighbors, max_count)
    lst = torch.empty((2, total), dtype=torch.int32, device=dev)
    sh = torch.empty((total, 3), dtype=torch.int32, device=dev) if want_shifts else None
    if total > 0:
        run(pos, cell, pbc, batch_idx, cutoff, C.NL_CSR, flags | C.NL_REUSE_GRID, nptr=nptr, list_ij=lst, list_sh=sh, n_pairs=total, ws=ws)
    return lst, nptr, sh, max_count
```

nvalchemi-toolkit-ops_amd/nvalchemiops/neighborlist/buffers.py:

```python
from __future__ import annotations

import statistics

import torch

from nvalchemiops.neighborlist import _engine as E


@torch.compiler.disable
def tuned_neighbor_buffers(positions: torch.Tensor, cutoff: float, cell: torch.Tensor, pbc: torch.Tensor, max_neighbors: int, *,
                           batch_idx: torch.Tensor | None = None, candidates: int = 6, trials: int = 3,
                           for_dftd3: "bool | E.D3SearchContext" = False, release_unused: bool = True, report: dict | None = None):
    from nvalchemiops.neighborlist.batch_cell_list import batch_cell_list
    from nvalchemiops.neighborlist.cell_list import cell_list

    n, m, dev = positions.shape[0], int(max_neighbors), positions.device

    ctx = for_dftd3 if isinstance(for_dftd3, E.D3SearchContext) else None

    def fresh():
        bufs = (torch.empty((n, m), dtype=torch.int32, device=dev), torch.empty((n, m, 3), dtype=torch.int32, device=dev),
                torch.empty((n,), dtype=torch.int32, device=dev))
        if ctx is not None:
            setattr(bufs[0], E._D3CTX_ATTR, ctx)
        return bufs

    def search(bufs):
        if batch_idx is None:
            cell_list(positions, cutoff, cell, pbc, neighbor_matrix=bufs[0], neighbor_matrix_shifts=bufs[1], num_neighbors=bufs[2])
        else:
            batch_cell_list(positions, cutoff, cell, pbc, batch_idx, neighbor_matrix=bufs[0], neighbor_matrix_shifts=bufs[1], num_neighbors=bufs[2])

    if for_dftd3 and E._PACKED_POLICY != "0":
        E.want_packed_companion(dev, n, m)
    if not positions.is_cuda or 16 * n * m < (256 << 20) or candidates <= 1:
        bufs = fresh()
        if report is not None:
            report.update(candidates=1, chosen=0, trial_ms=[])
        return bufs
    try:
        free_bytes, _ = torch.cuda.mem_get_info(dev)
        candidates = max(1, min(int(candidates), int(0.5 * free_bytes // (20 * n * m + 1))))
    except Exception:
        pass
    sets, times = [], []
    for _ in range(int(candidates)):
        bufs = fresh()
        search(bufs)
        search(bufs)
        ms = []
        for _ in range(int(trials)):
            a, b = torch.cuda.Event(enable_timing=True), torch.cuda.Event(enable_timing=True)
            a.record()
            search(bufs)
            b.record()
            b.synchronize()
            ms.append(a.elapsed_time(b))
        sets.append(bufs)
        times.append(statistics.median(ms))
    best = min(range(len(sets)), key=times.__getitem__)
    chosen = sets[best]
    if report is not None:
        report.update(candidates=len(sets), chosen=best, trial_ms=[round(t, 4) for t in times])
    del sets, bufs
    if release_unused:
        torch.cuda.synchronize(dev)
        torch.cuda.empty_cache()
    return chosen


__all__ = ["tuned_neighbor_buffers"]
```

Before: 31.50 million.

## Keep per-row neighbor-matrix padding state to skip redundant pad and shift writes

Adds a persistent per-row state block (span of nonzero-shift prefix and used count) attached to neighbor-matrix buffers. When the host and device agree the buffers are untouched since the last search, the tiled query kernel rewrites only the padding and zero-shift regions that changed, rather than refilling the whole row tail and pre-zeroing shifts. A strided device guard samples rows each call and marks the state dirty if the buffer contents differ from what is expected. This cuts memory writes per search, at the cost of extra bookkeeping, shared memory, and a risk of stale data if invalidation misses a mutation.

After: 31.45 million. Within noise of the previous version (-0.2%).

```diff
diff --git a/include/nvalchemiops_hip.h b/include/nvalchemiops_hip.h
--- a/include/nvalchemiops_hip.h
+++ b/include/nvalchemiops_hip.h
@@ -74,6 +74,14 @@
                               int32_t* num_neighbors, int max_neighbors, int fill_value, const void* bin_origin, void* workspace,
                               size_t workspace_bytes, void* packed_out, size_t packed_bytes, const mi_nl_cn_request* request ,
                               void* cn_out, size_t cn_bytes, void* stream);
+
+size_t mi_nl_row_state_bytes(int n_atoms);
+int mi_nl_neighbors_kept(const void* positions, int n_atoms, const void* cell, const uint8_t* pbc, const int32_t* batch_idx, int n_systems,
+                         double cutoff, int dtype, int flags, int32_t* neighbor_matrix, int32_t* neighbor_matrix_shifts,
+                         int32_t* num_neighbors, int max_neighbors, int fill_value, const void* bin_origin, void* workspace,
+                         size_t workspace_bytes, void* packed_out, size_t packed_bytes, const mi_nl_cn_request* request ,
+                         void* cn_out, size_t cn_bytes, void* row_state, size_t row_state_bytes, int row_state_trusted, int verify_stride,
+                         void* stream);
 
 int mi_nl_neighbors_dual(const void* positions, int n_atoms, const void* cell, const uint8_t* pbc, const int32_t* batch_idx, int n_systems,
                          double cutoff_short, double cutoff_long, int dtype, int flags,
diff --git a/nvalchemi-toolkit-ops_amd/csrc/nlist.hip b/nvalchemi-toolkit-ops_amd/csrc/nlist.hip
--- a/nvalchemi-toolkit-ops_amd/csrc/nlist.hip
+++ b/nvalchemi-toolkit-ops_amd/csrc/nlist.hip
@@ -86,6 +86,58 @@
 __device__ __forceinline__ double4 pack4(double x, double y, double z, int idx) { return make_double4(x, y, z, (double)idx); }
 __device__ __forceinline__ int idx_of(const float4& v) { return __float_as_int(v.w); }
 __device__ __forceinline__ int idx_of(const double4& v) { return (int)v.w; }
+
+#define NL_RS_HEADER_BYTES 256
+#define NL_RS_MAGIC 0x4e4c5253
+struct NlRowHdr {
+  int dirty, calls, clean_calls, raised;
+  int magic, n_atoms, M, fill_value;
+  unsigned long long p_nm, p_nsh, p_words;
+};
+struct NlKeep {
+  NlRowHdr* hdr;
+  int2* span;
+  int trust, stride, M, fill_value;
+  const int* nm; const int* nsh; const unsigned* words;
+};
+__device__ __forceinline__ void nl_keep_finish(NlRowHdr* h) {
+  h->clean_calls += h->dirty == 0 ? 1 : 0;
+  h->calls += 1;
+  h->dirty = 0;
+}
+__device__ __forceinline__ bool nl_wave_differs(const int* __restrict__ p0, long long begin, long long end, int value, int lane) {
+  const long long n = end - begin;
+  if (n <= 0) return false;
+  const int* p = p0 + begin;
+  int head = (int)(((16 - ((uintptr_t)p & 15)) & 15) >> 2);
+  if (head > n) head = (int)n;
+  bool bad = lane < head && p[lane] != value;
+  const long long body = (n - head) >> 2;
+  const int4* p4 = reinterpret_cast<const int4*>(p + head);
+  for (long long t = lane; t < body; t += MI_WAVE) {
+    const int4 w = p4[t];
+    bad |= (w.x != value) | (w.y != value) | (w.z != value) | (w.w != value);
+  }
+  const long long done = head + (body << 2);
+  if (done + lane < n) bad |= p[done + lane] != value;
+  return bad;
+}
+__device__ void nl_keep_guard(const NlKeep& RS, int N, int wave_id, int n_waves, int lane) {
+  NlRowHdr* h = RS.hdr;
+  if (h->dirty || RS.stride <= 0) return;
+  const int off = (int)((unsigned)h->calls % (unsigned)RS.stride);
+  const int M = RS.M;
+  for (long long r = off + (long long)wave_id * RS.stride; r < N; r += (long long)n_waves * RS.stride) {
+    int2 sp = RS.span[r];
+    const int cnt = sp.y < 0 ? 0 : (sp.y > M ? M : sp.y), n0 = sp.x < 0 ? 0 : (sp.x > cnt ? cnt : sp.x);
+    const long long ob = r * M;
+    bool bad = nl_wave_differs(RS.nsh, ob * 3, (ob + n0) * 3, 0, lane);
+    bad |= nl_wave_differs(RS.nsh, (ob + cnt) * 3, (ob + M) * 3, 0, lane);
+    bad |= nl_wave_differs(RS.nm, ob + cnt, ob + M, RS.fill_value, lane);
+    bad |= (sp.x != n0) | (sp.y != cnt);
+    if (__any(bad) && lane == 0) { h->dirty = 1; atomicAdd(&h->raised, 1); }
+  }
+}
 
 __global__ void nl_count_atoms_kernel(const int* __restrict__ batch_idx, int N, int* __restrict__ natoms) {
   const int i = blockIdx.x * blockDim.x + threadIdx.x;
@@ -145,8 +197,17 @@
 __global__ __launch_bounds__(256) void nl_setup_kernel(const T* __restrict__ cell, const uint8_t* __restrict__ pbc, const int* __restrict__ natoms, int N,
                                 int B, T cutoff, const T* __restrict__ origin, NlSys<T>* __restrict__ sys, NlGlobal* __restrict__ glob,
                                 int table_blocks, int4* __restrict__ zero, long long zero_words, int* __restrict__ pk_flag,
-                                int* __restrict__ cn_hdr, float cn_scale) {
+                                int* __restrict__ cn_hdr, float cn_scale, NlKeep RS) {
   constexpr int NE = (NL_PRUNE_R + 1) * (NL_PRUNE_R + 1);
+  if (RS.hdr && blockIdx.x == 0 && threadIdx.x == 0) {
+    NlRowHdr* h = RS.hdr;
+    if (h->magic != NL_RS_MAGIC) { h->calls = 0; h->clean_calls = 0; h->raised = 0; h->dirty = 1; h->magic = NL_RS_MAGIC; }
+    const bool same = h->n_atoms == N && h->M == RS.M && h->fill_value == RS.fill_value && h->p_nm == (unsigned long long)RS.nm &&
+                      h->p_nsh == (unsigned long long)RS.nsh && h->p_words == (unsigned long long)RS.words;
+    if (!RS.trust || !same) h->dirty = 1;
+    h->n_atoms = N; h->M = RS.M; h->fill_value = RS.fill_value;
+    h->p_nm = (unsigned long long)RS.nm; h->p_nsh = (unsigned long long)RS.nsh; h->p_words = (unsigned long long)RS.words;
+  }
   if (pk_flag && blockIdx.x == 0 && threadIdx.x == 0) *pk_flag = 0;
   if (cn_hdr && blockIdx.x == 0) {
     if (threadIdx.x == 0) { cn_hdr[0] = 0; cn_hdr[1] = 0; cn_hdr[2] = __float_as_int((float)cutoff); cn_hdr[3] = __float_as_int(cn_scale); }
@@ -244,11 +305,16 @@
 }
 
 struct NlCnBuild { const int* numbers; const float* rcov; int nz; float K; float* srk; unsigned long long* slots; const void* cell; int n_cell; const int* batch_idx; };
-template <class T>
+template <class T, bool GUARD = false>
 __global__ void nl_rank_gather_kernel(const T* __restrict__ pos, const int* __restrict__ ids, const int* __restrict__ keys,
                                       const int* __restrict__ cell_start, const short4* __restrict__ wrap, int N,
                                       typename Vec4<T>::type* __restrict__ spos, short4* __restrict__ swrap, int* __restrict__ keys_sorted,
-                                      NlCnBuild C) {
+                                      NlCnBuild C, NlKeep RS = NlKeep{}, int main_blocks = 0) {
+  if (GUARD && (int)blockIdx.x >= main_blocks) {
+    nl_keep_guard(RS, N, ((int)blockIdx.x - main_blocks) * (int)(blockDim.x / MI_WAVE) + (int)(threadIdx.x / MI_WAVE),
+                  ((int)gridDim.x - main_blocks) * (int)(blockDim.x / MI_WAVE), threadIdx.x & (MI_WAVE - 1));
+    return;
+  }
   int p = blockIdx.x * blockDim.x + threadIdx.x;
   unsigned long long h = 0;
   if (p < N) {
@@ -366,7 +432,7 @@
   return hit;
 }
 
-template <class T, int MODE, bool FAST, bool DUAL = false, bool CNF = false>
+template <class T, int MODE, bool FAST, bool DUAL = false, bool CNF = false, bool KEEP = false>
 #if NL_TILED_WAVES > 0
 __global__ __launch_bounds__(256) __attribute__((amdgpu_waves_per_eu(NL_TILED_WAVES, NL_TILED_WAVES))) void nl_query_tiled_kernel(
 #else
@@ -375,11 +441,15 @@
     const typename Vec4<T>::type* __restrict__ spos, const short4* __restrict__ swrap, const int* __restrict__ cell_start,
     const NlSys<T>* __restrict__ sys, const NlGlobal* __restrict__ glob, int B, T rc2, int flags, int* __restrict__ nm,
     int* __restrict__ nsh, int* __restrict__ num, int M, int fill_value, const int* __restrict__ ptr, int* __restrict__ list_ij,
-    int* __restrict__ list_sh, long long P, NlSecond<T> D, NlPacked K, NlCn CN = NlCn{nullptr, nullptr, nullptr, 0.0f}) {
+    int* __restrict__ list_sh, long long P, NlSecond<T> D, NlPacked K, NlCn CN = NlCn{nullptr, nullptr, nullptr, 0.0f}, NlKeep RS = NlKeep{}) {
   static_assert(!DUAL || (MODE == MI_NL_MODE_MATRIX && !FAST), "the dual-cutoff sweep is instantiated for the general matrix kernel only");
+  static_assert(!KEEP || (MODE == MI_NL_MODE_MATRIX && FAST && !DUAL), "a row state rides with the plain full-list padded matrix search");
   static_assert(!CNF || (MODE == MI_NL_MODE_MATRIX && FAST && !DUAL), "coordination numbers ride with the plain full-list matrix search");
   constexpr int TILE = sizeof(T) == 8 ? NL_TILE_F64 : NL_TILE;
-  if (!glob->use_tiled) return;
+  if (!glob->use_tiled) {
+    if (KEEP && blockIdx.x == 0 && threadIdx.x == 0) nl_keep_finish(RS.hdr);
+    return;
+  }
   if (!DUAL && FAST != ((flags & (MI_NL_HALF_FILL | MI_NL_NAIVE_EXPR)) == 0)) return;
   __shared__ float trk[CNF ? TILE : 1], cen_rk[CNF ? NL_CCHUNK : 1];
   __shared__ double ccn[CNF ? NL_CCHUNK : 1];
@@ -393,6 +463,9 @@
   __shared__ T cen_x[NL_CCHUNK], cen_y[NL_CCHUNK], cen_z[NL_CCHUNK];
   __shared__ int cen_i[NL_CCHUNK];
   __shared__ short4 cen_w[NL_CCHUNK];
+  __shared__ int2 cen_sp[KEEP ? NL_CCHUNK : 1];
+  __shared__ int cn0[KEEP ? NL_CCHUNK : 1];
+  const bool clean = KEEP && RS.hdr->dirty == 0;
   __shared__ int grp_run[TILE / MI_WAVE];
   __shared__ int grp_shift[TILE / MI_WAVE];
   __shared__ int u_store[CNF ? 1 : 9 * NL_MAXROWS];
@@ -487,6 +560,15 @@
           cen_i[tid] = idx_of(cr);
           cen_w[tid] = anyw ? swrap[c_beg + cbase + tid] : make_short4(0, 0, 0, 0);
           if (CNF) { cen_rk[tid] = CN.rk[c_beg + cbase + tid]; ccn[tid] = 0.0; }
+          if (KEEP) {
+            cn0[tid] = -1;
+            if (clean) {
+              int2 sp = RS.span[idx_of(cr)];
+              sp.y = sp.y < 0 ? 0 : (sp.y > M ? M : sp.y);
+              sp.x = sp.x < 0 ? 0 : (sp.x > sp.y ? sp.y : sp.x);
+              cen_sp[tid] = sp;
+            }
+          }
         }
       }
       for (int tile0 = 0; tile0 < total; tile0 += TILE) {
@@ -527,6 +609,7 @@
         for (int ci0 = cbase + wave; ci0 < cend; ci0 += 4 * NC) {
           T ccx[NC], ccy[NC], ccz[NC];
           int ii[NC], cap_row[NC], cnt[NC], cnt2[NC];
+          int n0[NC];
           float rki[NC], cnp[NC];
           long long out_base[NC];
           short4 wi[NC];
@@ -543,6 +626,7 @@
             else { out_base[u] = (long long)ii[u] * M; cap_row[u] = M; }
             cnt[u] = ccnt[ci - cbase];
             cnt2[u] = DUAL ? ccnt2[ci - cbase] : 0;
+            n0[u] = KEEP ? __builtin_amdgcn_readfirstlane(cn0[ci - cbase]) : 0;
             if (CNF) { rki[u] = nl_uni(cen_rk[ci - cbase]); cnp[u] = 0.0f; }
           }
           const bool ortho = S->prune != 0;
@@ -558,7 +642,7 @@
             else { row_j[u] = nullptr; row_s[u] = nullptr; }
           }
           constexpr bool PREZERO = NL_PREZERO_SHIFTS && MODE == MI_NL_MODE_MATRIX && !DUAL;
-          const bool prezero = PREZERO && nsh && !(flags & MI_NL_NO_PAD);
+          const bool prezero = PREZERO && nsh && !(flags & MI_NL_NO_PAD) && !clean;
           if (PREZERO && prezero && tile0 == 0) {
 #pragma unroll
             for (int u = 0; u < NC; ++u)
@@ -569,9 +653,11 @@
             if (MODE == MI_NL_MODE_COUNT) { cnt[u] += __popcll(mask); return; }
             if (mask) {
               const unsigned slot = __builtin_amdgcn_mbcnt_hi((unsigned)(mask >> 32), __builtin_amdgcn_mbcnt_lo((unsigned)mask, (unsigned)cnt[u]));
+              if (KEEP && !zero_shift && n0[u] < 0) n0[u] = __builtin_amdgcn_readfirstlane(cnt[u]);
+              const bool skip_shift = KEEP ? (zero_shift && n0[u] < 0) : (PREZERO && prezero && zero_shift);
               if (hit && slot < (unsigned)cap_row[u]) {
                 *reinterpret_cast<int*>(reinterpret_cast<char*>(row_j[u]) + slot * 4u) = j;
-                if (row_s[u] && !(PREZERO && prezero && zero_shift))
+                if (row_s[u] && !skip_shift)
                   *reinterpret_cast<NlInt3*>(reinterpret_cast<char*>(row_s[u]) + __umul24(slot, 12u)) = NlInt3{Sx, Sy, Sz};
                 if (MODE == MI_NL_MODE_MATRIX && !DUAL && row_p[u]) *reinterpret_cast<unsigned*>(reinterpret_cast<char*>(row_p[u]) + slot * 4u) = (unsigned)j | code;
               }
@@ -674,7 +760,7 @@
           }
           if (lane == 0) {
 #pragma unroll
-            for (int u = 0; u < NC; ++u) if (u < nc) { ccnt[ci0 + 4 * u - cbase] = cnt[u]; if (DUAL) ccnt2[ci0 + 4 * u - cbase] = cnt2[u]; }
+            for (int u = 0; u < NC; ++u) if (u < nc) { ccnt[ci0 + 4 * u - cbase] = cnt[u]; if (DUAL) ccnt2[ci0 + 4 * u - cbase] = cnt2[u]; if (KEEP) cn0[ci0 + 4 * u - cbase] = n0[u]; }
           }
         }
       }
@@ -692,7 +778,24 @@
           const int room = ptr[i + 1] - ptr[i];
           wave_fill(list_ij, rb, rb + (cnt < room ? cnt : room), i, lane);
         }
-        if (MODE == MI_NL_MODE_MATRIX && !(flags & MI_NL_NO_PAD)) {
+        if (KEEP) {
+          const long long out_base = (long long)i * M;
+          const int used = cnt < M ? cnt : M;
+          int n0n = __builtin_amdgcn_readfirstlane(cn0[ci - cbase]);
+          n0n = (n0n < 0 || n0n > used) ? used : n0n;
+          if (clean) {
+            const int2 so = cen_sp[ci - cbase];
+            const int n0o = __builtin_amdgcn_readfirstlane(so.x), cno = __builtin_amdgcn_readfirstlane(so.y);
+            wave_fill(nm, out_base + used, out_base + cno, fill_value, lane);
+            if (K.words) wave_fill(reinterpret_cast<int*>(K.words), out_base + used, out_base + cno, (int)NL_PK_PAD, lane);
+            wave_fill(nsh, (out_base + n0o) * 3, (out_base + (n0n < cno ? n0n : cno)) * 3, 0, lane);
+            wave_fill(nsh, (out_base + (used > n0o ? used : n0o)) * 3, (out_base + cno) * 3, 0, lane);
+          } else {
+            wave_fill(nm, out_base + used, out_base + M, fill_value, lane);
+            if (K.words) wave_fill(reinterpret_cast<int*>(K.words), out_base + used, out_base + M, (int)NL_PK_PAD, lane);
+          }
+          if (lane == 0) RS.span[i] = make_int2(n0n, used);
+        } else if (MODE == MI_NL_MODE_MATRIX && !(flags & MI_NL_NO_PAD)) {
           const long long out_base = (long long)i * M;
           const int used = cnt < M ? cnt : M;
           wave_fill(nm, out_base + used, out_base + M, fill_value, lane);
@@ -716,17 +819,19 @@
   if (tid == 0 && atomicAdd(&gw->done[MODE], 1) == (int)gridDim.x - 1) {
     gw->work[MODE] = 0;
     gw->done[MODE] = 0;
-  }
-}
-
-template <class T, int MODE, bool DUAL = false, bool CNF = false>
+    if (KEEP) nl_keep_finish(RS.hdr);
+  }
+}
+
+template <class T, int MODE, bool DUAL = false, bool CNF = false, bool KEEP = false>
 __global__ __launch_bounds__(256) void nl_query_kernel(
     const typename Vec4<T>::type* __restrict__ spos, const short4* __restrict__ swrap, const int* __restrict__ keys_sorted,
     const int* __restrict__ cell_start, const int* __restrict__ batch_idx, const NlSys<T>* __restrict__ sys,
     const NlGlobal* __restrict__ glob, int N, T rc2, int flags, int* __restrict__ nm, int* __restrict__ nsh, int* __restrict__ num,
     int M, int fill_value, const int* __restrict__ ptr, int* __restrict__ list_ij, int* __restrict__ list_sh, long long P, NlSecond<T> D,
-    NlPacked K, NlCn CN = NlCn{nullptr, nullptr, nullptr, 0.0f}) {
+    NlPacked K, NlCn CN = NlCn{nullptr, nullptr, nullptr, 0.0f}, NlKeep RS = NlKeep{}) {
   static_assert(!DUAL || MODE == MI_NL_MODE_MATRIX, "the dual-cutoff sweep fills two padded matrices");
+  static_assert(!KEEP || (MODE == MI_NL_MODE_MATRIX && !DUAL), "a row state rides with the plain padded matrix search");
   static_assert(!CNF || (MODE == MI_NL_MODE_MATRIX && !DUAL), "coordination numbers ride with the plain matrix search");
   if (glob->use_tiled) return;
   const int lane = threadIdx.x & (MI_WAVE - 1);
@@ -919,6 +1024,7 @@
     wave_fill(nm, out_base + used, out_base + M, fill_value, lane);
     if (nsh) wave_fill(nsh, (out_base + used) * 3, (out_base + M) * 3, 0, lane);
     if (K.words) wave_fill(reinterpret_cast<int*>(K.words), out_base + used, out_base + M, (int)NL_PK_PAD, lane);
+    if (KEEP && lane == 0) RS.span[i] = make_int2(0, used);
   }
   if (DUAL) {
     if (lane == 0) D.num[i] = cnt2;
@@ -1137,7 +1243,8 @@
 int nl_neighbors_impl(const T* pos, int N, const T* cell, const uint8_t* pbc, const int* batch_idx, int B, double cutoff, int mode, int flags,
                       int* nm, int* nsh, int* num, int M, int fill_value, const int* ptr, int* list_ij, int* list_sh, long long P,
                       const T* origin, char* ws, const NlLayout& L, hipStream_t st, const NlSecond<T>* second = nullptr,
-                      NlPacked K = NlPacked{nullptr, nullptr}, const mi_nl_cn_request* cnreq = nullptr, void* cn_block = nullptr) {
+                      NlPacked K = NlPacked{nullptr, nullptr}, const mi_nl_cn_request* cnreq = nullptr, void* cn_block = nullptr,
+                      NlKeep RS = NlKeep{}) {
   auto* sys = reinterpret_cast<NlSys<T>*>(ws + L.sys);
   auto* glob = reinterpret_cast<NlGlobal*>(ws + L.glob);
   int* natoms = reinterpret_cast<int*>(ws + L.natoms);
@@ -1177,12 +1284,18 @@
     const int table_blocks = mi_blocks((long long)B * (NL_PRUNE_R + 1) * (NL_PRUNE_R + 1), 256);
     nl_setup_kernel<T><<<1 + table_blocks + zero_blocks, 256, 0, st>>>(cell, pbc, nat, N, B, rc, origin, sys, glob, table_blocks,
                                                                        reinterpret_cast<int4*>(bins.count), zero_words, K.words ? K.flag : nullptr,
-                                                                       CN.flag, CN.K);
+                                                                       CN.flag, CN.K, RS);
     MI_LAUNCH_CHECK();
     nl_assign_kernel<T><<<mi_blocks(N, 256), 256, 0, st>>>(pos, batch_idx, N, sys, keys_in, bins.count, wrap, glob);
     MI_LAUNCH_CHECK();
     MI_HIP_CHECK(bs_sort(bins, keys_in, N, &glob->total_cells, vals_out, cell_start, st));
-    nl_rank_gather_kernel<T><<<mi_blocks(CB.srk && 9 * B > N ? 9 * B : N, 256), 256, 0, st>>>(pos, vals_out, keys_in, cell_start, wrap, N, spos, swrap, keys_out, CB);
+    const int gather_blocks = mi_blocks(CB.srk && 9 * B > N ? 9 * B : N, 256);
+    if (RS.hdr && RS.stride > 0) {
+      const long long rows = ((long long)N + RS.stride - 1) / RS.stride;
+      const int guard_blocks = (int)((rows + 3) / 4 > 1024 ? 1024 : (rows + 3) / 4);
+      nl_rank_gather_kernel<T, true><<<gather_blocks + guard_blocks, 256, 0, st>>>(pos, vals_out, keys_in, cell_start, wrap, N, spos, swrap, keys_out, CB, RS, gather_blocks);
+    } else
+      nl_rank_gather_kernel<T><<<gather_blocks, 256, 0, st>>>(pos, vals_out, keys_in, cell_start, wrap, N, spos, swrap, keys_out, CB);
     MI_LAUNCH_CHECK();
     mi_timing_end((void*)st);
   }
@@ -1211,7 +1324,20 @@
       nl_query_tiled_kernel<T, MODE_, false><<<nl_tiled_grid(), 256, 0, st>>>(spos, swrap, cell_start, sys, glob, B, rc2, flags, nm, nsh, num, \
                                                                            M, fill_value, ptr, list_ij, list_sh, P, none, K);            \
   } while (0)
-  if (mode == MI_NL_MODE_MATRIX && CN.cn) {
+  if (RS.hdr) {
+    if (CN.cn)
+      MI_TIMED(sizeof(T) == 4 ? "nl_query_matrix_f32" : "nl_query_matrix_f64", st,
+               (nl_query_kernel<T, MI_NL_MODE_MATRIX, false, true, true><<<blocks, 256, 0, st>>>(spos, swrap, keys_out, cell_start, batch_idx, sys, glob, N, rc2, flags,
+                                                                                                nm, nsh, num, M, fill_value, ptr, list_ij, list_sh, P, none, K, CN, RS),
+                nl_query_tiled_kernel<T, MI_NL_MODE_MATRIX, true, false, true, true><<<nl_tiled_grid(), 256, 0, st>>>(
+                    spos, swrap, cell_start, sys, glob, B, rc2, flags, nm, nsh, num, M, fill_value, ptr, list_ij, list_sh, P, none, K, CN, RS)));
+    else
+      MI_TIMED(sizeof(T) == 4 ? "nl_query_matrix_f32" : "nl_query_matrix_f64", st,
+               (nl_query_kernel<T, MI_NL_MODE_MATRIX, false, false, true><<<blocks, 256, 0, st>>>(spos, swrap, keys_out, cell_start, batch_idx, sys, glob, N, rc2, flags,
+                                                                                                 nm, nsh, num, M, fill_value, ptr, list_ij, list_sh, P, none, K, CN, RS),
+                nl_query_tiled_kernel<T, MI_NL_MODE_MATRIX, true, false, false, true><<<nl_tiled_grid(), 256, 0, st>>>(
+                    spos, swrap, cell_start, sys, glob, B, rc2, flags, nm, nsh, num, M, fill_value, ptr, list_ij, list_sh, P, none, K, CN, RS)));
+  } else if (mode == MI_NL_MODE_MATRIX && CN.cn) {
     MI_TIMED(sizeof(T) == 4 ? "nl_query_matrix_f32" : "nl_query_matrix_f64", st,
              (nl_query_kernel<T, MI_NL_MODE_MATRIX, false, true><<<blocks, 256, 0, st>>>(spos, swrap, keys_out, cell_start, batch_idx, sys, glob, N, rc2, flags, nm,
                                                                                         nsh, num, M, fill_value, ptr, list_ij, list_sh, P, none, K, CN),
@@ -1266,7 +1392,8 @@
                     double cutoff, int dtype, int mode, int flags, int32_t* neighbor_matrix, int32_t* neighbor_matrix_shifts,
                     int32_t* num_neighbors, int max_neighbors, int fill_value, const int32_t* neighbor_ptr, int32_t* list_ij,
                     int32_t* list_shifts, long long n_pairs, const void* bin_origin, void* workspace, size_t workspace_bytes, void* stream, void* packed_out,
-                    const mi_nl_cn_request* cnreq = nullptr, void* cn_block = nullptr) {
+                    const mi_nl_cn_request* cnreq = nullptr, void* cn_block = nullptr, void* row_state = nullptr, int row_state_trusted = 0,
+                    int verify_stride = 0) {
   MI_REQUIRE(dtype == MI_F32 || dtype == MI_F64, "dtype must be MI_F32 or MI_F64");
   MI_REQUIRE(n_atoms >= 0 && n_systems >= 1, "n_atoms >= 0 and n_systems >= 1");
   MI_REQUIRE(cutoff > 0, "cutoff must be positive");
@@ -1287,14 +1414,27 @@
     K.flag = reinterpret_cast<int*>(packed_out);
     K.words = reinterpret_cast<unsigned*>(packed_out) + 64;
   }
+  NlKeep RS{};
+  if (row_state) {
+    MI_REQUIRE(mode == MI_NL_MODE_MATRIX && neighbor_matrix_shifts && max_neighbors > 0 &&
+                   !(flags & (MI_NL_NO_PAD | MI_NL_HALF_FILL | MI_NL_NAIVE_EXPR | MI_NL_REUSE_GRID | MI_NL_NO_SHIFTS)),
+               "row state: full (not half-filled) padded cell-list matrix with shifts, own binning");
+    RS.hdr = reinterpret_cast<NlRowHdr*>(row_state);
+    RS.span = reinterpret_cast<int2*>(reinterpret_cast<char*>(row_state) + NL_RS_HEADER_BYTES);
+    RS.trust = row_state_trusted != 0;
+    RS.stride = verify_stride;
+    RS.M = max_neighbors;
+    RS.fill_value = fill_value;
+    RS.nm = neighbor_matrix; RS.nsh = neighbor_matrix_shifts; RS.words = K.words;
+  }
   if (cnreq) MI_REQUIRE(packed_out && cn_block && cnreq->numbers && cnreq->covalent_radii && cnreq->nz >= 2, "coordination numbers: companion, output block, numbers and radii");
   if (dtype == MI_F32)
     return nl_neighbors_impl<float>((const float*)positions, n_atoms, (const float*)cell, pbc, batch_idx, n_systems, cutoff, mode, flags,
                                     neighbor_matrix, neighbor_matrix_shifts, num_neighbors, max_neighbors, fill_value, neighbor_ptr, list_ij,
-                                    list_shifts, n_pairs, (const float*)bin_origin, (char*)workspace, L, st, nullptr, K, cnreq, cn_block);
+                                    list_shifts, n_pairs, (const float*)bin_origin, (char*)workspace, L, st, nullptr, K, cnreq, cn_block, RS);
   return nl_neighbors_impl<double>((const double*)positions, n_atoms, (const double*)cell, pbc, batch_idx, n_systems, cutoff, mode, flags,
                                    neighbor_matrix, neighbor_matrix_shifts, num_neighbors, max_neighbors, fill_value, neighbor_ptr, list_ij,
-                                   list_shifts, n_pairs, (const double*)bin_origin, (char*)workspace, L, st, nullptr, K, cnreq, cn_block);
+                                   list_shifts, n_pairs, (const double*)bin_origin, (char*)workspace, L, st, nullptr, K, cnreq, cn_block, RS);
 }
 
 extern "C" {
@@ -1336,6 +1476,22 @@
   return nl_neighbors_entry(positions, n_atoms, cell, pbc, batch_idx, n_systems, cutoff, dtype, MI_NL_MODE_MATRIX, flags, neighbor_matrix,
                             neighbor_matrix_shifts, num_neighbors, max_neighbors, fill_value, nullptr, nullptr, nullptr, 0, bin_origin, workspace,
                             workspace_bytes, stream, packed_out, request, cn_out);
+}
+
+size_t mi_nl_row_state_bytes(int n_atoms) { return n_atoms > 0 ? NL_RS_HEADER_BYTES + sizeof(int2) * (size_t)n_atoms : 0; }
+
+int mi_nl_neighbors_kept(const void* positions, int n_atoms, const void* cell, const uint8_t* pbc, const int32_t* batch_idx, int n_systems,
+                         double cutoff, int dtype, int flags, int32_t* neighbor_matrix, int32_t* neighbor_matrix_shifts,
+                         int32_t* num_neighbors, int max_neighbors, int fill_value, const void* bin_origin, void* workspace,
+                         size_t workspace_bytes, void* packed_out, size_t packed_bytes, const mi_nl_cn_request* request, void* cn_out,
+                         size_t cn_bytes, void* row_state, size_t row_state_bytes, int row_state_trusted, int verify_stride, void* stream) {
+  MI_REQUIRE(row_state != nullptr && row_state_bytes >= mi_nl_row_state_bytes(n_atoms) && verify_stride >= 0, "row_state: mi_nl_row_state_bytes(n_atoms) bytes");
+  MI_REQUIRE(!packed_out || (packed_bytes >= mi_nl_packed_bytes(n_atoms, max_neighbors) && mi_nl_packed_bytes(n_atoms, max_neighbors) > 0),
+             "packed_out: mi_nl_packed_bytes(n_atoms, max_neighbors) bytes");
+  MI_REQUIRE(!request || (cn_out != nullptr && cn_bytes >= mi_nl_cn_bytes(n_atoms)), "cn_out: mi_nl_cn_bytes(n_atoms) bytes");
+  return nl_neighbors_entry(positions, n_atoms, cell, pbc, batch_idx, n_systems, cutoff, dtype, MI_NL_MODE_MATRIX, flags, neighbor_matrix,
+                            neighbor_matrix_shifts, num_neighbors, max_neighbors, fill_value, nullptr, nullptr, nullptr, 0, bin_origin, workspace,
+                            workspace_bytes, stream, packed_out, request, request ? cn_out : nullptr, row_state, row_state_trusted, verify_stride);
 }
 
 int mi_nl_neighbors_dual(const void* positions, int n_atoms, const void* cell, const uint8_t* pbc, const int32_t* batch_idx, int n_systems,
diff --git a/nvalchemi-toolkit-ops_amd/nvalchemiops/_capi.py b/nvalchemi-toolkit-ops_amd/nvalchemiops/_capi.py
--- a/nvalchemi-toolkit-ops_amd/nvalchemiops/_capi.py
+++ b/nvalchemi-toolkit-ops_amd/nvalchemiops/_capi.py
@@ -65,6 +65,8 @@
         L.mi_nl_packed_bytes.argtypes = [ctypes.c_int, ctypes.c_int]
         L.mi_nl_cn_bytes.restype = ctypes.c_size_t
         L.mi_nl_cn_bytes.argtypes = [ctypes.c_int]
+        L.mi_nl_row_state_bytes.restype = ctypes.c_size_t
+        L.mi_nl_row_state_bytes.argtypes = [ctypes.c_int]
         if hasattr(L, "mi_d3_workspace_bytes"):
             L.mi_d3_workspace_bytes.restype = ctypes.c_size_t
             L.mi_d3_workspace_bytes.argtypes = [ctypes.c_int, ctypes.c_int, ctypes.c_int]
diff --git a/nvalchemi-toolkit-ops_amd/nvalchemiops/neighborlist/_engine.py b/nvalchemi-toolkit-ops_amd/nvalchemiops/neighborlist/_engine.py
--- a/nvalchemi-toolkit-ops_amd/nvalchemiops/neighborlist/_engine.py
+++ b/nvalchemi-toolkit-ops_amd/nvalchemiops/neighborlist/_engine.py
@@ -19,6 +19,8 @@
 _D3CTX_BY_SHAPE: dict = {}
 _VERIFY_STRIDE = max(0, int(os.environ.get("NVALCHEMIOPS_NL_PACKED_VERIFY", "64") or 0))
 _verify_calls = 0
+_KEEP_POLICY = os.environ.get("NVALCHEMIOPS_NL_KEEP", "1")
+_KEEP_ATTR = "_nvalchemiops_row_state"
 
 
 def verify_args() -> tuple[int, int]:
@@ -69,6 +71,61 @@
         pass
 
 
+class RowStateRecord:
+    __slots__ = ("block", "nm_version", "nsh_ref", "nsh_version", "num_ref", "num_version", "n_atoms", "row_width", "fill_value", "words_ptr",
+                 "searches", "trusted_searches")
+
+    def __init__(self, block: torch.Tensor, nm: torch.Tensor):
+        self.block = block
+        self.n_atoms, self.row_width = int(nm.shape[0]), int(nm.shape[1])
+        self.searches = self.trusted_searches = 0
+        self.forget()
+
+    def forget(self) -> None:
+        self.nm_version = self.nsh_ref = self.nsh_version = self.num_ref = self.num_version = self.fill_value = self.words_ptr = None
+
+    def remember(self, nm, nsh, num, fill_value, words) -> None:
+        self.nm_version = nm._version
+        self.nsh_ref, self.nsh_version = weakref.ref(nsh), nsh._version
+        self.num_ref, self.num_version = weakref.ref(num), num._version
+        self.fill_value = int(fill_value)
+        self.words_ptr = 0 if words is None else words.data_ptr()
+
+    def usable(self, nm, nsh, num) -> bool:
+        return (nsh is not None and num is not None and tuple(nm.shape) == (self.n_atoms, self.row_width) and self.row_width > 0
+                and tuple(nsh.shape) == (self.n_atoms, self.row_width, 3) and tuple(num.shape) == (self.n_atoms,)
+                and nm.dtype == torch.int32 and nsh.dtype == torch.int32 and num.dtype == torch.int32
+                and nm.is_contiguous() and nsh.is_contiguous() and num.is_contiguous()
+                and nm.device == self.block.device and nsh.device == nm.device and num.device == nm.device)
+
+    def trusted(self, nm, nsh, num, fill_value, words) -> bool:
+        return (self.nm_version is not None and self.usable(nm, nsh, num) and self.nsh_ref() is nsh and self.num_ref() is num
+                and nm._version == self.nm_version and nsh._version == self.nsh_version and num._version == self.num_version
+                and int(fill_value) == self.fill_value and (0 if words is None else words.data_ptr()) == self.words_ptr)
+
+
+def attach_row_state(nm: torch.Tensor) -> None:
+    if _KEEP_POLICY == "0" or not nm.is_cuda or nm.shape[0] == 0 or nm.shape[1] == 0:
+        return
+    nbytes = int(C.lib().mi_nl_row_state_bytes(int(nm.shape[0])))
+    setattr(nm, _KEEP_ATTR, RowStateRecord(torch.zeros(nbytes, dtype=torch.uint8, device=nm.device), nm))
+
+
+def row_state_info(nm: torch.Tensor) -> dict | None:
+    rec = getattr(nm, _KEEP_ATTR, None)
+    if rec is None:
+        return None
+    dirty, calls, clean, raised = (int(v) for v in rec.block[:16].view(torch.int32).tolist())
+    return {"searches": rec.searches, "host_trusted": rec.trusted_searches, "device_calls": calls, "clean_searches": clean,
+            "guard_raised": raised, "dirty": dirty}
+
+
+def _forget_row_state(t) -> None:
+    rec = getattr(t, _KEEP_ATTR, None)
+    if rec is not None:
+        rec.forget()
+
+
 def invalidate(*tensors: torch.Tensor) -> None:
     for t in tensors:
         if t is None:
@@ -76,12 +133,14 @@
         for attr in (_PACKED_ATTR, _BUILT_ATTR, _FULL_ATTR):
             if hasattr(t, attr):
                 delattr(t, attr)
+        _forget_row_state(t)
         owner = getattr(t, "_nvalchemiops_owner", None)
         nm = owner() if owner is not None else None
         if nm is not None and nm is not t:
             for attr in (_PACKED_ATTR, _BUILT_ATTR, _FULL_ATTR):
                 if hasattr(nm, attr):
                     delattr(nm, attr)
+            _forget_row_state(nm)
 
 
 class PackedCompanion:
@@ -154,6 +213,7 @@
         for attr in (_PACKED_ATTR, _BUILT_ATTR, _FULL_ATTR):
             if hasattr(t, attr):
                 delattr(t, attr)
+        _forget_row_state(t)
         try:
             torch.autograd.graph.increment_version(t)
         except Exception:
@@ -263,6 +323,11 @@
                  and int(max_neighbors) > 0)
     emit = qualifies and (_PACKED_POLICY == "1" or (_PACKED_POLICY == "auto" and (pos.device.index, n, int(max_neighbors)) in _PACKED_WANTED))
     nbytes = int(C.lib().mi_nl_packed_bytes(n, int(max_neighbors))) if emit else 0
+    rec = getattr(nm, _KEEP_ATTR, None) if _KEEP_POLICY != "0" else None
+    if (rec is not None and want_shifts and pad and not half_fill and not naive and n > 0 and int(max_neighbors) == rec.row_width
+            and rec.usable(nm, nsh, num)):
+        _neighbor_matrix_kept(rec, pos, cell, pbc, batch_idx, cutoff, max_neighbors, fill_value, flags, nm, nsh, num, origin, qualifies, nbytes)
+        return
     if nbytes == 0:
         run(pos, cell, pbc, batch_idx, cutoff, C.NL_MATRIX, flags, nm=nm, nsh=nsh if want_shifts else None, num=num,
             max_neighbors=max_neighbors, fill_value=fill_value, origin=origin)
@@ -306,6 +371,49 @@
         pass
 
 
+def _neighbor_matrix_kept(rec, pos, cell, pbc, batch_idx, cutoff, max_neighbors, fill_value, flags, nm, nsh, num, origin, qualifies, nbytes):
+    n = pos.shape[0]
+    old = getattr(nm, _PACKED_ATTR, None)
+    words = cn = req = None
+    cn_bytes = 0
+    if nbytes:
+        words = old.words if (old is not None and old.words.numel() == nbytes and old.words.device == pos.device) else torch.empty(nbytes, dtype=torch.uint8, device=pos.device)
+        ctx = getattr(nm, _D3CTX_ATTR, None)
+        if ctx is None and _PACKED_POLICY == "auto":
+            ctx = _D3CTX_BY_SHAPE.get((pos.device.index, n, int(max_neighbors)))
+        if ctx is not None and (ctx.numbers.shape[0] != n or ctx.numbers.device != pos.device):
+            ctx = None
+        if ctx is not None:
+            cn_bytes = int(C.lib().mi_nl_cn_bytes(n))
+            cn = old.cn if (old is not None and old.cn is not None and old.cn.numel() == cn_bytes and old.cn.device == pos.device) else torch.empty(cn_bytes, dtype=torch.uint8, device=pos.device)
+            req = C.MiNlCnRequest(numbers=ctx.numbers.data_ptr(), covalent_radii=ctx.rcov.data_ptr(), nz=int(ctx.rcov.shape[0]), k1=ctx.k1)
+    try:
+        trusted = rec.trusted(nm, nsh, num, fill_value, words)
+    except Exception:
+        trusted = False
+    ws = workspace(n, cell.shape[0], pos.dtype, pos.device)
+    _written(nm, nsh, num)
+    stride = 1 if _KEEP_POLICY == "verify_all" else _VERIFY_STRIDE
+    rc = C.lib().mi_nl_neighbors_kept(
+        C.ptr(pos), n, C.ptr(cell), C.ptr(pbc), C.ptr(batch_idx), cell.shape[0], C.cdouble(cutoff), C.dtype_code(pos.dtype), flags,
+        C.ptr(nm), C.ptr(nsh), C.ptr(num), int(max_neighbors), int(fill_value), C.ptr(origin), C.ptr(ws), ctypes.c_size_t(ws.numel()),
+        C.ptr(words), ctypes.c_size_t(nbytes), ctypes.byref(req) if req is not None else None, C.ptr(cn), ctypes.c_size_t(cn_bytes),
+        C.ptr(rec.block), ctypes.c_size_t(rec.block.numel()), int(trusted), int(stride), C.stream_of(pos))
+    C.check(rc, "mi_nl_neighbors_kept")
+    rec.searches += 1
+    rec.trusted_searches += int(trusted)
+    _record_full_list(nm, nsh, num, fill_value, qualifies)
+    try:
+        if words is not None:
+            setattr(nm, _PACKED_ATTR, PackedCompanion(words, nm, nsh, fill_value, cn=cn))
+        elif qualifies and _PACKED_POLICY == "auto":
+            setattr(nm, _BUILT_ATTR, nm._version)
+        setattr(nsh, "_nvalchemiops_owner", weakref.ref(nm))
+        rec.remember(nm, nsh, num, fill_value, words)
+    except Exception:
+        pass
+
+
 def neighbor_matrix_dual(pos, cell, pbc, batch_idx, cutoff_short, cutoff_long, fill_value, half_fill, short, long_, *, naive=True, want_shifts=True,
                          origin=None):
     flags = (C.NL_HALF_FILL if half_fill else 0) | (C.NL_NAIVE_EXPR if naive else 0)
diff --git a/nvalchemi-toolkit-ops_amd/nvalchemiops/neighborlist/buffers.py b/nvalchemi-toolkit-ops_amd/nvalchemiops/neighborlist/buffers.py
--- a/nvalchemi-toolkit-ops_amd/nvalchemiops/neighborlist/buffers.py
+++ b/nvalchemi-toolkit-ops_amd/nvalchemiops/neighborlist/buffers.py
@@ -23,6 +23,7 @@
                 torch.empty((n,), dtype=torch.int32, device=dev))
         if ctx is not None:
             setattr(bufs[0], E._D3CTX_ATTR, ctx)
+        E.attach_row_state(bufs[0])
         return bufs
 
     def search(bufs):
```
